# quickwit-oss/tantivy

Measured on AMD Instinct MI355X. Metric: queries_per_sec_2term_AND_bm25_top10, higher is better.
Workload: dtype u32+f32; 1 GPU; and2: 10000 queries/batch, k=10, one 10M-doc Zipf segment per GPU (256 terms, df_r=0.5N/r, WithFreqs); term ranks ~ Zipf(1); distinct_queries=3877, mode=block-max pruned (block_wand_intersection semantics), exchange=single rank: no exchange, segments_per_gpu=1, index_bytes=40381332

## Files before the change

include/tantivy_amd.h:

```cpp
#ifndef TANTIVY_AMD_H
#define TANTIVY_AMD_H

#include <stddef.h>
#include <stdint.h>

#ifdef __cplusplus
extern "C" {
#endif

#define TQ_TERMINATED 0x7FFFFFFFu
#define TQ_MAX_TERMS 16u
#define TQ_MAX_K 1024u

enum tq_status {
  TQ_OK = 0,
  TQ_ERR_INVALID = 1,
  TQ_ERR_HIP = 2,
  TQ_ERR_FORMAT = 3,
  TQ_ERR_UNSUPPORTED = 4,
  TQ_ERR_NO_DEVICE = 5
};

enum tq_record_option { TQ_BASIC = 0, TQ_WITH_FREQS = 1, TQ_WITH_FREQS_AND_POSITIONS = 2 };

// ... 34 lines not shown
int tq_all_query_form(const tq_query *q, tq_all_form *out);

int tq_init(const int *device_ids, int n_devices, tq_ctx **out);
void tq_shutdown(tq_ctx *ctx);
const char *tq_last_error(void);

int tq_segment_upload(tq_ctx *ctx, int device, uint32_t max_doc, const uint8_t *idx,
                      size_t idx_len, const uint8_t *pos, size_t pos_len,
                      const uint8_t *fieldnorm, size_t fn_len, uint8_t record_option,
                      tq_segment **out);
int tq_segment_upload_device(tq_ctx *ctx, int device, uint32_t max_doc, const uint8_t *d_idx,
                             size_t idx_len, const uint8_t *d_pos, size_t pos_len,
                             const uint8_t *d_fieldnorm, size_t fn_len, uint8_t record_option,
                             tq_segment **out);
void tq_segment_free(tq_segment *seg);

int tq_term_prepare(tq_segment *seg, uint64_t postings_off, uint32_t postings_len,
                    uint64_t positions_off, uint32_t positions_len, uint32_t doc_freq,
                    tq_term_handle *out);
typedef struct tq_term_info {
  uint64_t postings_off;
  uint64_t positions_off;
  uint32_t postings_len, positions_len;
  uint32_t doc_freq;
  uint32_t pad_;
} tq_term_info;
int tq_term_prepare_batch(tq_segment *seg, const tq_term_info *infos, uint32_t n, tq_term_handle *out);
int tq_segment_reserve_columns(tq_segment *seg, const uint64_t *postings_offs, uint32_t n);

int tq_term_set_prepare(tq_segment *seg, const tq_term_handle *members, uint32_t n, tq_term_handle *out);
int tq_term_set_info(tq_segment *seg, tq_term_handle set, uint32_t *n_docs, uint64_t *bytes);
int tq_term_set_release(tq_segment *seg, tq_term_handle set);

int tq_search_batch(tq_segment *seg, const tq_query *queries, uint32_t n_queries,
                    uint32_t out_stride, float *out_scores, uint32_t *out_docs,
                    uint32_t *out_counts);

int tq_search_batch_device(tq_segment *seg, const tq_query *queries, uint32_t n_queries,
                           uint32_t out_stride, float *d_out_scores, uint32_t *d_out_docs,
                           uint32_t *d_out_counts, void *hip_stream);

#define TQ_OPT_DEFAULT 0xFFFFFFFFu
typedef struct tq_search_opts {
  int32_t exhaustive;
  uint32_t bound_slack_ppm;
} tq_search_opts;
int tq_search_batch_opts(tq_segment *seg, const tq_query *queries, uint32_t n_queries,
                         uint32_t out_stride, float *out_scores, uint32_t *out_docs,
                         uint32_t *out_counts, const tq_search_opts *opts);
int tq_search_batch_device_opts(tq_segment *seg, const tq_query *queries, uint32_t n_queries,
                                uint32_t out_stride, float *d_out_scores, uint32_t *d_out_docs,
                                uint32_t *d_out_counts, const tq_search_opts *opts,
                                void *hip_stream);

typedef struct tq_ticket tq_ticket;
int tq_submit(tq_segment *seg, const tq_query *query, const tq_search_opts *opts, float *out_scores,
              uint32_t *out_docs, uint32_t *out_count, tq_ticket **out);
int tq_wait(tq_ticket *ticket);
int tq_search_one(tq_segment *seg, const tq_query *query, const tq_search_opts *opts,
                  float *out_scores, uint32_t *out_docs, uint32_t *out_count);
typedef struct tq_submit_stats {
  uint64_t batches;
  uint64_t queries;
  uint64_t max_batch;
} tq_submit_stats;
int tq_get_submit_stats(tq_segment *seg, tq_submit_stats *out, int reset);

int tq_merge_topk(const float *scores, const uint32_t *docs, const uint32_t *counts,
                  uint32_t n_segments, uint32_t n_queries, uint32_t stride, uint32_t offset,
                  uint32_t limit, float *out_scores, uint32_t *out_segment_ords,
                  uint32_t *out_docs, uint32_t *out_counts);
int tq_merge_topk_device(tq_ctx *ctx, int device, const float *d_scores, const uint32_t *d_docs,
                         const uint32_t *d_counts, const uint32_t *segment_ords,
                         uint32_t n_segments, uint32_t n_queries, uint32_t stride,
                         uint32_t offset, uint32_t limit, float *d_out_scores,
                         uint32_t *d_out_segment_ords, uint32_t *d_out_docs,
                         uint32_t *d_out_counts, void *hip_stream);
int tq_copy_to_host_async(tq_ctx *ctx, int device, void *dst_pinned_host, const void *src_device, size_t bytes,
                          void *hip_stream);

#define TQ_COMM_ID_BYTES 128
typedef struct tq_comm tq_comm;
int tq_comm_unique_id(uint8_t *id_out );
int tq_comm_init(tq_ctx *ctx, int device, const uint8_t *id, int rank, int world, tq_comm **out);
void tq_comm_free(tq_comm *comm);
int tq_comm_info(const tq_comm *comm, int *rank, int *world, const char **library);
int tq_allgather_topk(tq_comm *comm, const float *d_scores, const uint32_t *d_docs,
                      const uint32_t *d_counts, uint32_t n_rows, uint32_t stride,
                      float *d_all_scores, uint32_t *d_all_docs, uint32_t *d_all_counts,
                      void *hip_stream);

int tq_decode_postings(tq_segment *seg, tq_term_handle term, uint32_t *docs, uint32_t *tfs);
int tq_decode_position_deltas(tq_segment *seg, tq_term_handle term, uint32_t *out, uint64_t cap,
                              uint64_t *n_out);

typedef struct tq_encoder tq_encoder;
int tq_encoder_create(tq_ctx *ctx, int device, tq_encoder **out);
void tq_encoder_free(tq_encoder *enc);
int tq_encode_postings(tq_encoder *enc, uint32_t n_terms, const uint64_t *term_starts,
                       const uint32_t *docs, const uint32_t *tfs, const uint8_t *fieldnorm_ids,
                       uint32_t num_docs, float avg_fieldnorm, uint8_t record_option, uint8_t *out,
                       uint64_t out_cap, uint64_t *out_term_starts, uint64_t *out_len);
int tq_encode_positions(tq_encoder *enc, uint32_t n_terms, const uint64_t *term_starts,
                        const uint32_t *position_deltas, uint8_t *out, uint64_t out_cap,
                        uint64_t *out_term_starts, uint64_t *out_len);
int tq_encode_postings_device(tq_encoder *enc, uint32_t n_terms, const uint64_t *term_starts,
// ... 76 lines not shown
```

include/tantivy_amd_host.h:

```cpp
#ifndef TANTIVY_AMD_HOST_H
#define TANTIVY_AMD_HOST_H
#include "tantivy_amd.h"
#ifdef __cplusplus
extern "C" {
#endif

typedef struct tqh_searcher tqh_searcher;

typedef struct tqh_term_info {
  uint32_t term_id;
  uint32_t doc_freq;
  uint64_t postings_start, postings_end, positions_start, positions_end;
} tqh_term_info;

#define TQH_MODE_TERM 4
typedef struct tqh_query {
  uint8_t mode;
  uint32_t n_terms;
  const uint32_t *terms;
  const uint32_t *phrase_offsets;
  const uint8_t *occurs;
  const uint8_t *clause_of;
  uint32_t min_should_match;
  const float *boosts;
  const uint8_t *nested_occurs;
  const uint8_t *clause_min_should;
  const uint8_t *atom_of;
  const uint32_t *set_terms;
  const uint32_t *set_starts;
} tqh_query;
#define TQH_TERM_SET_BASE 0xFFFFFF00u

const char *tqh_last_error(void);
int tqh_searcher_new(tq_ctx *ctx, tqh_searcher **out);
void tqh_searcher_free(tqh_searcher *s);
int tqh_searcher_add_segment(tqh_searcher *s, int device, uint32_t max_doc, uint8_t record_option,
                             const uint8_t *idx, size_t idx_len, const uint8_t *pos,
                             size_t pos_len, const uint8_t *fieldnorm, size_t fn_len,
                             const tqh_term_info *terms, uint32_t n_terms);
int tqh_searcher_add_remote_stats(tqh_searcher *s, uint64_t max_doc, uint64_t total_num_tokens,
                                  const uint32_t *term_ids, const uint32_t *doc_freqs,
                                  uint32_t n_terms);
int tqh_prepare_batch(tqh_searcher *s, const tqh_query *queries, uint32_t n);
int tqh_prepare_batch_next(tqh_searcher *s, const tqh_query *queries, uint32_t n);
int tqh_commit_next(tqh_searcher *s);
int tqh_search_prepared(tqh_searcher *s, uint32_t offset, uint32_t limit, float *scores,
                        uint32_t *segment_ords, uint32_t *docs, uint32_t *counts);
int tqh_search_concurrent(tqh_searcher *s, const tqh_query *queries, uint32_t n, uint32_t offset,
                          uint32_t limit, uint32_t n_threads, float *scores, uint32_t *segment_ords,
                          uint32_t *docs, uint32_t *counts, float *latency_ms, double *wall_ms);
int tqh_count_prepared(tqh_searcher *s, uint64_t *counts);
int tqh_docset_prepared(tqh_searcher *s, uint32_t *out_segment_ords, uint32_t *out_docs, uint64_t out_cap,
                        uint64_t *out_starts);
int tqh_docset_scored_prepared(tqh_searcher *s, uint32_t *out_segment_ords, uint32_t *out_docs, float *out_scores,
                               uint64_t out_cap, uint64_t *out_starts);
int tqh_collect_segment_prepared(tqh_searcher *s, uint32_t segment_ord, uint32_t k, float *scores,
                                 uint32_t *docs, uint32_t *counts);
int tqh_collect_segment_prepared_device(tqh_searcher *s, uint32_t segment_ord, uint32_t k,
                                        float *d_scores, uint32_t *d_docs, uint32_t *d_counts,
                                        void *hip_stream);
int tqh_bm25_for_terms(const uint64_t *term_doc_freqs, uint32_t n_terms, uint64_t total_num_docs,
                       uint64_t total_num_tokens, float boost, float *weight_out,
                       float *cache_out);
tq_segment *tqh_segment_raw(tqh_searcher *s, uint32_t segment_ord);
uint32_t tqh_term_handle(tqh_searcher *s, uint32_t segment_ord, uint32_t term_id);

typedef struct tqh_term_info_store tqh_term_info_store;
int tqh_term_dictionary_values(const uint8_t *file, size_t len, uint64_t *store_off,
                               uint64_t *store_len);
int tqh_term_info_store_open(const uint8_t *bytes, size_t len, tqh_term_info_store **out);
void tqh_term_info_store_free(tqh_term_info_store *s);
uint64_t tqh_term_info_store_num_terms(const tqh_term_info_store *s);
int tqh_term_info_store_get(const tqh_term_info_store *s, const uint64_t *term_ords, uint32_t n,
                            tqh_term_info *out);
int tqh_term_info_store_write(const tqh_term_info *infos, uint32_t n, uint8_t *out,
                              uint64_t out_cap, uint64_t *out_len);
int tqh_searcher_add_segment_with_store(tqh_searcher *s, int device, uint32_t max_doc,
                                        uint8_t record_option, const uint8_t *idx, size_t idx_len,
                                        const uint8_t *pos, size_t pos_len,
                                        const uint8_t *fieldnorm, size_t fn_len,
                                        const uint8_t *store, size_t store_len);

int tqh_searcher_add_segment_device_with_store(tqh_searcher *s, int device, uint32_t max_doc,
                                               uint8_t record_option, const uint8_t *d_idx,
                                               size_t idx_len, const uint8_t *d_pos, size_t pos_len,
                                               const uint8_t *d_fieldnorm, size_t fn_len,
                                               uint64_t total_num_tokens, const uint8_t *store,
                                               size_t store_len);

#ifdef __cplusplus
}
#endif
#endif
```

tantivy_amd/binding.py:

```python
import ctypes as C
import os

import numpy as np

_HERE = os.path.dirname(os.path.abspath(__file__))
LIB_PATH = os.path.join(_HERE, "lib", "libtantivy_amd.so")
if os.environ.get("TQ_LIB_PATH"):
    LIB_PATH = os.environ["TQ_LIB_PATH"]

TERMINATED = 0x7FFFFFFF
TERM_ABSENT = 0xFFFFFFFF
TERM_ALL = 0xFFFFFFFE
ALL_EMPTY, ALL_PLAIN, ALL_BASED = 0, 1, 2
MODE_AND, MODE_OR, MODE_PHRASE, MODE_BOOL, MODE_TERM = 0, 1, 2, 3, 4
SHOULD, MUST, MUST_NOT = 0, 1, 2
BASIC, WITH_FREQS, WITH_FREQS_AND_POSITIONS = 0, 1, 2


class TantivyAmdError(RuntimeError):
    def __init__(self, code, msg):
        super().__init__("tantivy_amd error %d: %s" % (code, msg))
        self.code = code


# ... 42 lines not shown
    return [n for b, n in sorted(KERNEL_NAMES.items()) if mask & b]


class TqAllForm(C.Structure):
    _fields_ = [("kind", C.c_uint32), ("base", C.c_float), ("min_should", C.c_uint32), ("keep_mask", C.c_uint32)]


class TqSubmitStats(C.Structure):
    _fields_ = [("batches", C.c_uint64), ("queries", C.c_uint64), ("max_batch", C.c_uint64)]


class TqSegmentStats(C.Structure):
    _fields_ = [(n, C.c_uint64) for n in (
        "index_bytes", "positions_bytes", "fieldnorm_bytes", "alive_bytes", "term_table_bytes",
        "bitmap_bytes", "docmat_bytes", "posdir_bytes", "scratch_bytes", "dense_budget_bytes")] + [
        (n, C.c_uint32) for n in ("n_terms", "n_dense_lists", "n_docmat_columns", "probe_evictions")] + [
        ("device_scratch_bytes", C.c_uint64)]


class TqTermInfo(C.Structure):
    _fields_ = [("postings_off", C.c_uint64), ("positions_off", C.c_uint64), ("postings_len", C.c_uint32),
                ("positions_len", C.c_uint32), ("doc_freq", C.c_uint32), ("pad_", C.c_uint32)]


class TqhTermInfo(C.Structure):
    _fields_ = [("term_id", C.c_uint32), ("doc_freq", C.c_uint32), ("postings_start", C.c_uint64),
                ("postings_end", C.c_uint64), ("positions_start", C.c_uint64),
                ("positions_end", C.c_uint64)]


class TqhQuery(C.Structure):
    _fields_ = [("mode", C.c_uint8), ("n_terms", C.c_uint32), ("terms", C.POINTER(C.c_uint32)),
                ("phrase_offsets", C.POINTER(C.c_uint32)), ("occurs", C.POINTER(C.c_uint8)),
                ("clause_of", C.POINTER(C.c_uint8)), ("min_should_match", C.c_uint32),
                ("boosts", C.POINTER(C.c_float)), ("nested_occurs", C.POINTER(C.c_uint8)),
                ("clause_min_should", C.POINTER(C.c_uint8)), ("atom_of", C.POINTER(C.c_uint8)),
                ("set_terms", C.POINTER(C.c_uint32)), ("set_starts", C.POINTER(C.c_uint32))]


TERM_SET_BASE = 0xFFFFFF00


class RawHandle(int):
    """A tq_term_handle as the C ABI returned it (DeviceIndex.term_set_prepare): DeviceIndex.term_handle passes it
    through untouched where a plain int is a term id of the dictionary."""


_lib = None

EXPORTS = [
    "tq_init", "tq_shutdown", "tq_last_error", "tq_segment_upload", "tq_segment_upload_device",
    "tq_segment_free",
    "tq_term_prepare", "tq_term_prepare_batch", "tq_search_batch", "tq_search_batch_device", "tq_search_batch_opts",
    "tq_search_batch_device_opts", "tq_merge_topk",
    "tq_merge_topk_device", "tq_copy_to_host_async", "tq_decode_postings", "tq_decode_position_deltas",
    "tq_last_batch_stats", "tq_segment_get_stats", "tq_segment_reserve_columns", "tq_set_option", "tq_segment_set_alive_bitset", "tq_count_batch",
    "tq_last_batch_match_counts", "tq_last_batch_query_kernels", "tq_encoder_create", "tq_encoder_free", "tq_encode_postings",
    "tq_encode_positions", "tq_encode_postings_device", "tq_encode_positions_device",
    "tq_encoder_last_kernel_ms", "tq_comm_unique_id", "tq_comm_init", "tq_comm_free",
    "tq_comm_info", "tq_allgather_topk",
    "tqh_last_error", "tqh_searcher_new", "tqh_searcher_free", "tqh_searcher_add_segment",
    "tqh_prepare_batch", "tqh_prepare_batch_next", "tqh_commit_next", "tqh_search_prepared", "tqh_collect_segment_prepared",
    "tqh_collect_segment_prepared_device", "tqh_searcher_add_remote_stats",
    "tqh_bm25_for_terms", "tqh_segment_raw", "tqh_term_handle", "tqh_term_dictionary_values",
    "tqh_term_info_store_open", "tqh_term_info_store_free", "tqh_term_info_store_num_terms",
    "tqh_term_info_store_get", "tqh_term_info_store_write", "tqh_searcher_add_segment_with_store",
    "tqh_count_prepared", "tqh_searcher_add_segment_device_with_store",
    "tq_docset_batch", "tq_docset_batch_device", "tqh_docset_prepared",
    "tq_docset_scored_batch", "tq_docset_scored_batch_device", "tqh_docset_scored_prepared",
    "tq_all_query_form",
    "tq_term_set_prepare", "tq_term_set_info", "tq_term_set_release",
]


def lib():
    global _lib
    if _lib is not None:
        return _lib
    if not os.path.exists(LIB_PATH):
        raise TantivyAmdError(-1, "%s not built (run `python -m tantivy_amd.build` or "
                                  "__graft_entry__.build())" % LIB_PATH)
    L = C.CDLL(LIB_PATH)
    vp, u8p, u32p, f32p = C.c_void_p, C.POINTER(C.c_uint8), C.POINTER(C.c_uint32), C.POINTER(C.c_float)
    L.tq_last_error.restype = C.c_char_p
    L.tqh_last_error.restype = C.c_char_p
    L.tq_init.argtypes = [C.POINTER(C.c_int), C.c_int, C.POINTER(vp)]
    L.tq_shutdown.argtypes = [vp]
    L.tq_segment_upload.argtypes = [vp, C.c_int, C.c_uint32, vp, C.c_size_t, vp, C.c_size_t, vp,
                                    C.c_size_t, C.c_uint8, C.POINTER(vp)]
    L.tq_segment_upload_device.argtypes = [vp, C.c_int, C.c_uint32, vp, C.c_size_t, vp, C.c_size_t, vp,
                                           C.c_size_t, C.c_uint8, C.POINTER(vp)]
    L.tq_segment_free.argtypes = [vp]
    L.tq_term_prepare.argtypes = [vp, C.c_uint64, C.c_uint32, C.c_uint64, C.c_uint32, C.c_uint32,
                                  u32p]
    L.tq_term_prepare_batch.argtypes = [vp, C.POINTER(TqTermInfo), C.c_uint32, u32p]
    L.tq_search_batch.argtypes = [vp, C.POINTER(TqQuery), C.c_uint32, C.c_uint32, f32p, u32p, u32p]
    L.tq_search_batch_device.argtypes = [vp, C.POINTER(TqQuery), C.c_uint32, C.c_uint32, vp, vp,
                                         vp, vp]
    L.tq_search_batch_opts.argtypes = [vp, C.POINTER(TqQuery), C.c_uint32, C.c_uint32, f32p, u32p,
                                       u32p, C.POINTER(TqSearchOpts)]
    L.tq_search_batch_device_opts.argtypes = [vp, C.POINTER(TqQuery), C.c_uint32, C.c_uint32, vp,
                                              vp, vp, C.POINTER(TqSearchOpts), vp]
    L.tq_merge_topk.argtypes = [f32p, u32p, u32p, C.c_uint32, C.c_uint32, C.c_uint32, C.c_uint32,
                                C.c_uint32, f32p, u32p, u32p, u32p]
    L.tq_copy_to_host_async.argtypes = [vp, C.c_int, vp, vp, C.c_size_t, vp]
    L.tq_merge_topk_device.argtypes = [vp, C.c_int, vp, vp, vp, vp, C.c_uint32, C.c_uint32,
                                       C.c_uint32, C.c_uint32, C.c_uint32, vp, vp, vp, vp, vp]
    L.tq_decode_postings.argtypes = [vp, C.c_uint32, u32p, u32p]
    L.tq_decode_position_deltas.argtypes = [vp, C.c_uint32, u32p, C.c_uint64,
                                            C.POINTER(C.c_uint64)]
    L.tq_last_batch_stats.argtypes = [vp, C.POINTER(TqBatchStats)]
    L.tq_segment_get_stats.argtypes = [vp, C.POINTER(TqSegmentStats)]
    L.tq_segment_reserve_columns.argtypes = [vp, C.POINTER(C.c_uint64), C.c_uint32]
    L.tq_set_option.argtypes = [vp, C.c_char_p, C.c_int64]
    L.tq_segment_set_alive_bitset.argtypes = [vp, vp, C.c_size_t]
    L.tq_count_batch.argtypes = [vp, C.POINTER(TqQuery), C.c_uint32, u32p]
    L.tq_last_batch_match_counts.argtypes = [vp, u32p, C.c_uint32]
    L.tq_docset_batch.argtypes = [vp, C.POINTER(TqQuery), C.c_uint32, u32p, C.c_uint64, C.POINTER(C.c_uint64)]
    L.tq_docset_batch_device.argtypes = [vp, C.POINTER(TqQuery), C.c_uint32, vp, C.c_uint64, vp, vp]
    L.tqh_docset_prepared.argtypes = [vp, u32p, u32p, C.c_uint64, C.POINTER(C.c_uint64)]
    L.tq_docset_scored_batch.argtypes = [vp, C.POINTER(TqQuery), C.c_uint32, u32p, f32p, C.c_uint64, C.POINTER(C.c_uint64)]
    L.tq_docset_scored_batch_device.argtypes = [vp, C.POINTER(TqQuery), C.c_uint32, vp, vp, C.c_uint64, vp, vp]
    L.tqh_docset_scored_prepared.argtypes = [vp, u32p, u32p, f32p, C.c_uint64, C.POINTER(C.c_uint64)]
    L.tq_last_batch_query_kernels.argtypes = [vp, u32p, C.c_uint32]
    L.tq_all_query_form.argtypes = [C.POINTER(TqQuery), C.POINTER(TqAllForm)]
    L.tq_term_set_prepare.argtypes = [vp, u32p, C.c_uint32, u32p]
    L.tq_term_set_info.argtypes = [vp, C.c_uint32, u32p, C.POINTER(C.c_uint64)]
    L.tq_term_set_release.argtypes = [vp, C.c_uint32]
    u64p = C.POINTER(C.c_uint64)
    L.tq_encoder_create.argtypes = [vp, C.c_int, C.POINTER(vp)]
    L.tq_encoder_free.argtypes = [vp]
    L.tq_encoder_free.restype = None
    L.tq_encode_postings.argtypes = [vp, C.c_uint32, vp, vp, vp, vp, C.c_uint32, C.c_float,
                                     C.c_uint8, vp, C.c_uint64, vp, u64p]
    L.tq_encode_positions.argtypes = [vp, C.c_uint32, vp, vp, vp, C.c_uint64, vp, u64p]
    L.tq_encode_postings_device.argtypes = [vp, C.c_uint32, vp, vp, vp, vp, vp, C.c_uint32,
                                            C.c_float, C.c_uint8, vp, C.c_uint64, vp, u64p, vp]
    L.tq_encode_positions_device.argtypes = [vp, C.c_uint32, vp, vp, vp, vp, C.c_uint64, vp, u64p,
                                             vp]
    L.tq_encoder_last_kernel_ms.argtypes = [vp, C.POINTER(C.c_float)]
    L.tq_comm_unique_id.argtypes = [vp]
    L.tq_comm_init.argtypes = [vp, C.c_int, vp, C.c_int, C.c_int, C.POINTER(vp)]
    L.tq_comm_free.argtypes = [vp]
    L.tq_comm_free.restype = None
    L.tq_comm_info.argtypes = [vp, C.POINTER(C.c_int), C.POINTER(C.c_int), C.POINTER(C.c_char_p)]
    L.tq_allgather_topk.argtypes = [vp, vp, vp, vp, C.c_uint32, C.c_uint32, vp, vp, vp, vp]
    L.tqh_searcher_new.argtypes = [vp, C.POINTER(vp)]
    L.tqh_searcher_free.argtypes = [vp]
    L.tqh_searcher_add_segment.argtypes = [vp, C.c_int, C.c_uint32, C.c_uint8, vp, C.c_size_t, vp,
                                           C.c_size_t, vp, C.c_size_t, C.POINTER(TqhTermInfo),
                                           C.c_uint32]
    L.tqh_prepare_batch.argtypes = [vp, C.POINTER(TqhQuery), C.c_uint32]
    L.tqh_prepare_batch_next.argtypes = [vp, C.POINTER(TqhQuery), C.c_uint32]
    L.tqh_commit_next.argtypes = [vp]
    L.tqh_search_prepared.argtypes = [vp, C.c_uint32, C.c_uint32, f32p, u32p, u32p, u32p]
    L.tqh_search_concurrent.argtypes = [vp, C.POINTER(TqhQuery), C.c_uint32, C.c_uint32, C.c_uint32, C.c_uint32,
                                        f32p, u32p, u32p, u32p, f32p, C.POINTER(C.c_double)]
    L.tq_get_submit_stats.argtypes = [vp, C.POINTER(TqSubmitStats), C.c_int]
    L.tq_search_one.argtypes = [vp, C.POINTER(TqQuery), C.POINTER(TqSearchOpts), f32p, u32p, u32p]
    L.tq_submit.argtypes = [vp, C.POINTER(TqQuery), C.POINTER(TqSearchOpts), f32p, u32p, u32p, C.POINTER(vp)]
    L.tq_wait.argtypes = [vp]
    L.tqh_collect_segment_prepared.argtypes = [vp, C.c_uint32, C.c_uint32, f32p, u32p, u32p]
    L.tqh_collect_segment_prepared_device.argtypes = [vp, C.c_uint32, C.c_uint32, vp, vp, vp, vp]
    L.tqh_searcher_add_remote_stats.argtypes = [vp, C.c_uint64, C.c_uint64, u32p, u32p, C.c_uint32]
    L.tqh_bm25_for_terms.argtypes = [C.POINTER(C.c_uint64), C.c_uint32, C.c_uint64, C.c_uint64,
                                     C.c_float, f32p, f32p]
    L.tqh_segment_raw.restype = vp
    L.tqh_segment_raw.argtypes = [vp, C.c_uint32]
    L.tqh_term_handle.restype = C.c_uint32
    L.tqh_term_handle.argtypes = [vp, C.c_uint32, C.c_uint32]
    L.tqh_term_dictionary_values.argtypes = [vp, C.c_size_t, u64p, u64p]
    L.tqh_count_prepared.argtypes = [vp, u64p]
    L.tqh_term_info_store_open.argtypes = [vp, C.c_size_t, C.POINTER(vp)]
    L.tqh_term_info_store_free.argtypes = [vp]
    L.tqh_term_info_store_free.restype = None
    L.tqh_term_info_store_num_terms.argtypes = [vp]
    L.tqh_term_info_store_num_terms.restype = C.c_uint64
    L.tqh_term_info_store_get.argtypes = [vp, vp, C.c_uint32, C.POINTER(TqhTermInfo)]
    L.tqh_term_info_store_write.argtypes = [C.POINTER(TqhTermInfo), C.c_uint32, vp, C.c_uint64, u64p]
    L.tqh_searcher_add_segment_with_store.argtypes = [vp, C.c_int, C.c_uint32, C.c_uint8, vp,
                                                      C.c_size_t, vp, C.c_size_t, vp, C.c_size_t,
                                                      vp, C.c_size_t]
    L.tqh_searcher_add_segment_device_with_store.argtypes = [
        vp, C.c_int, C.c_uint32, C.c_uint8, vp, C.c_size_t, vp, C.c_size_t, vp, C.c_size_t,
        C.c_uint64, vp, C.c_size_t]
    _lib = L
    return L


def _check(rc, host=False):
    if rc != 0:
        L = lib()
        msg = (L.tqh_last_error() if host else L.tq_last_error()) or b""
        if host and not msg:
            msg = L.tq_last_error() or b""
        raise TantivyAmdError(rc, msg.decode("utf-8", "replace"))


def _f32(a):
    return a.ctypes.data_as(C.POINTER(C.c_float))


def _u32(a):
    return a.ctypes.data_as(C.POINTER(C.c_uint32))


def bm25_for_terms(doc_freqs, total_num_docs, total_num_tokens, boost=1.0):
    dfs = (C.c_uint64 * len(doc_freqs))(*[int(d) for d in doc_freqs])
    w = C.c_float()
    cache = np.zeros(256, np.float32)
    _check(lib().tqh_bm25_for_terms(dfs, len(doc_freqs), int(total_num_docs), int(total_num_tokens),
                                    C.c_float(boost), C.byref(w), _f32(cache)), host=True)
    return float(w.value), cache


def all_query_form(handles, weights=None, mode=MODE_BOOL, occurs=None, clause_of=None, min_should_match=0):
# ... 328 lines not shown

    def commit_next(self):
        fut, n, _ = self._prep_next
        secs = fut.result()
        self._prep_next = None
        _check(lib().tqh_commit_next(self._s), host=True)
        self._n_prepared = n
        return secs

    def search_concurrent(self, queries, limit, n_threads, offset=0):
        qs, keep = self._host_queries(queries)
        n = len(queries)
        scores = np.zeros((n, limit), np.float32)
        ords = np.zeros((n, limit), np.uint32)
        docs = np.zeros((n, limit), np.uint32)
        counts = np.zeros(n, np.uint32)
        lat = np.zeros(max(1, n), np.float32)
        wall = C.c_double()
        _check(lib().tqh_search_concurrent(self._s, qs, n, int(offset), int(limit), int(n_threads),
                                           _f32(scores), _u32(ords), _u32(docs), _u32(counts), _f32(lat),
                                           C.byref(wall)), host=True)
        return scores, ords, docs, counts, lat[:n], float(wall.value)

    def submit_stats(self, segment_ord=0, reset=False):
        st = TqSubmitStats()
        _check(lib().tq_get_submit_stats(self.segment_raw(segment_ord), C.byref(st), 1 if reset else 0))
        return {"batches": int(st.batches), "queries": int(st.queries), "max_batch": int(st.max_batch)}

    def search_prepared(self, limit, offset=0):
        n = self._n_prepared
        scores = np.zeros((n, limit), np.float32)
        ords = np.zeros((n, limit), np.uint32)
        docs = np.zeros((n, limit), np.uint32)
        counts = np.zeros(n, np.uint32)
        _check(lib().tqh_search_prepared(self._s, int(offset), int(limit), _f32(scores),
                                         _u32(ords), _u32(docs), _u32(counts)), host=True)
        return scores, ords, docs, counts

    def collect_segment_prepared(self, segment_ord, k):
        n = self._n_prepared
        scores = np.zeros((n, k), np.float32)
        docs = np.zeros((n, k), np.uint32)
        counts = np.zeros(n, np.uint32)
        _check(lib().tqh_collect_segment_prepared(self._s, int(segment_ord), int(k), _f32(scores),
                                                  _u32(docs), _u32(counts)), host=True)
        return scores, docs, counts

    def collect_segment_prepared_device(self, segment_ord, k, d_scores, d_docs, d_counts,
                                        stream=None):
        _check(lib().tqh_collect_segment_prepared_device(
            self._s, int(segment_ord), int(k), d_scores.data_ptr(), d_docs.data_ptr(),
            d_counts.data_ptr(), C.c_void_p(stream) if stream else None), host=True)

    @property
    def ctx(self):
        return self._ctx

    def search(self, queries, limit, offset=0):
        self.prepare(queries)
        return self.search_prepared(limit, offset)

    def count(self, queries):
        self.prepare(queries)
        out = np.zeros(max(1, len(queries)), np.uint64)
        _check(lib().tqh_count_prepared(self._s, out.ctypes.data_as(C.POINTER(C.c_uint64))), host=True)
        return out[: len(queries)]

    def docset(self, queries):
        self.prepare(queries)
        n = len(queries)
        starts = np.zeros(n + 1, np.uint64)
        ords = np.zeros(1, np.uint32)
        docs = np.zeros(1, np.uint32)
        u64p = C.POINTER(C.c_uint64)
        rc = lib().tqh_docset_prepared(self._s, _u32(ords), _u32(docs), 0, starts.ctypes.data_as(u64p))
        if rc != 0 and int(starts[n]) > 0:
            ords = np.zeros(int(starts[n]), np.uint32)
            docs = np.zeros(int(starts[n]), np.uint32)
            rc = lib().tqh_docset_prepared(self._s, _u32(ords), _u32(docs), docs.size, starts.ctypes.data_as(u64p))
        _check(rc, host=True)
        pairs = np.stack([ords, docs], axis=1)
        return [pairs[int(starts[q]): int(starts[q + 1])] for q in range(n)]

    def docset_scored(self, queries):
        self.prepare(queries)
        n = len(queries)
        starts = np.zeros(n + 1, np.uint64)
        ords = np.zeros(1, np.uint32)
        docs = np.zeros(1, np.uint32)
        scores = np.zeros(1, np.float32)
        u64p = C.POINTER(C.c_uint64)
        rc = lib().tqh_docset_scored_prepared(self._s, _u32(ords), _u32(docs), _f32(scores), 0, starts.ctypes.data_as(u64p))
        if rc != 0 and int(starts[n]) > 0:
            ords = np.zeros(int(starts[n]), np.uint32)
            docs = np.zeros(int(starts[n]), np.uint32)
            scores = np.zeros(int(starts[n]), np.float32)
            rc = lib().tqh_docset_scored_prepared(self._s, _u32(ords), _u32(docs), _f32(scores), docs.size,
                                                  starts.ctypes.data_as(u64p))
        _check(rc, host=True)
        pairs = np.stack([ords, docs], axis=1)
        return [(pairs[int(starts[q]): int(starts[q + 1])], scores[int(starts[q]): int(starts[q + 1])]) for q in range(n)]

    def segment_raw(self, segment_ord=0):
        return C.c_void_p(lib().tqh_segment_raw(self._s, segment_ord))

    def term_handle(self, term_id, segment_ord=0):
# ... 279 lines not shown
```

tantivy_amd/csrc/tq_api.cpp:

```cpp
#include "tq_internal.hpp"
#include "../host/bm25.hpp"

namespace tqi {

thread_local std::string g_last_error;

int fail(int code, const char *fmt, ...) {
  char buf[512];
  va_list ap;
  va_start(ap, fmt);
  vsnprintf(buf, sizeof buf, fmt, ap);
  va_end(ap);
  g_last_error = buf;
  return code;
}
}

int tq_internal_fail(int code, const char *where, const char *what) {
  return fail(code, "%s: %s", where, what);
}
bool tq_internal_ctx_has_device(const tq_ctx *ctx, int device) {
  return std::find(ctx->devices.begin(), ctx->devices.end(), device) != ctx->devices.end();
}

// ... 409 lines not shown
    r.device_scratch_bytes = s->dscratch->partials.cap + s->dscratch->share_stage.cap + s->dscratch->ashare_stage.cap +
                             s->dscratch->bshare_stage.cap;
  }
  r.n_terms = (uint32_t)s->terms.size();
  r.n_dense_lists = s->n_dense_lists;
  r.n_docmat_columns = s->n_mat_slots;
  r.probe_evictions = (uint32_t)std::min<uint64_t>(s->probe_evictions, 0xFFFFFFFFull);
  r.dense_budget_bytes = s->dense_budget();
  *out = r;
  return TQ_OK;
}

int tq_set_option(tq_segment *s, const char *name, int64_t value) {
  if (!s || !name) return fail(TQ_ERR_INVALID, "tq_set_option: null argument");
  TQ_SEGMENT_LOCK(s);
  if (!strcmp(name, "exhaustive"))
    __atomic_store_n(&s->opt.exhaustive, value != 0 ? 1 : 0, __ATOMIC_RELAXED);
  else if (!strcmp(name, "timing"))
    s->opt.timing = value != 0;
  else if (!strcmp(name, "use_dpp"))
    s->opt.use_dpp = value != 0;
  else if (!strcmp(name, "use_dense"))
    s->opt.use_dense = value != 0;
  else if (!strcmp(name, "or_windows"))
    s->opt.or_windows = value < 0 ? -1 : (value != 0);
  else if (!strcmp(name, "dense_ratio") && value >= 1)
    s->opt.dense_ratio = (int)value;
  else if (!strcmp(name, "rdir_budget_x") && value >= 0 && value <= 0x7FFFFFFF)
    s->opt.rdir_budget_x = (int)value;
  else if (!strcmp(name, "probe_budget_x") && value >= 0 && value <= 0x7FFFFFFF)
    s->opt.probe_budget_x = (int)value, s->probe_full = false;
  else if (!strcmp(name, "dense_budget_x") && value >= 0)
    s->opt.dense_budget_x = (int)value;
  else if (!strcmp(name, "bound_slack_ppm") && value >= 0 && value <= 1000000000)
    __atomic_store_n(&s->opt.bound_slack_ppm, (int)value, __ATOMIC_RELAXED);
  else if (!strcmp(name, "dense"))
    s->opt.dense = value != 0;
  else if (!strcmp(name, "docmat"))
    s->opt.docmat = value != 0;
  else if (!strcmp(name, "docsig"))
    s->opt.docsig = value != 0;
  else if (!strcmp(name, "device_prepare"))
    s->opt.device_prepare = value != 0;
  else if (!strcmp(name, "xunion_ratio") && value >= 0 && value <= 0x7FFFFFFF)
    s->opt.xunion_ratio = (int)value;
  else if (!strcmp(name, "count_bitmap_ratio") && value >= 0 && value <= 0x7FFFFFFF)
    s->opt.count_bitmap_ratio = (int)value;
  else if (!strcmp(name, "docset_temp_lists") && value >= 0 && value <= 0x7FFFFFFF)
    s->opt.docset_temp_lists = (int)value;
  else if (!strcmp(name, "docset_trees") && (value == 0 || value == 1))
    s->opt.docset_trees = (int)value;
  else if (!strcmp(name, "docset_score_trees") && (value == 0 || value == 1))
    s->opt.docset_score_trees = (int)value;
  else if (!strcmp(name, "ashare_min_batch") && value >= 0 && value <= 0x7FFFFFFF)
    s->opt.ashare_min_batch = (int)value;
  else if (!strcmp(name, "xunion_min_queries") && value >= 1 && value <= 0x7FFFFFFF)
    s->opt.xunion_min_queries = (int)value;
  else if (!strcmp(name, "record_query_kernels"))
    s->opt.record_query_kernels = value != 0;
  else if (!strcmp(name, "debug") && value >= -1 && value <= 0x7FFFFFFF)
    s->opt.debug = (int)value;
  else if (!strcmp(name, "submit_window_us") && value >= 0 && value <= 1000000)
    s->opt.submit_window_us = (int)value;
  else
    return fail(TQ_ERR_INVALID, "unknown option '%s'", name);
  return TQ_OK;
}

int tq_decode_postings(tq_segment *s, tq_term_handle term, uint32_t *docs, uint32_t *tfs) {
  if (!s || !docs || !tfs) return fail(TQ_ERR_INVALID, "tq_decode_postings: null argument");
  TQ_SEGMENT_LOCK(s);
  if (term >= s->terms.size()) return fail(TQ_ERR_INVALID, "unknown term handle %u", term);
  if (s->terms[term].set_kind != TermHost::kNoSet) return fail(TQ_ERR_INVALID, "tq_decode_postings: handle %u is a term set: it has no postings", term);
  HIP_TRY(hipSetDevice(s->device));
  int rc = sync_terms(s, s->stream);
  if (rc != TQ_OK) return rc;
  const TermHost &t = s->terms[term];
  const size_t bytes = (size_t)t.doc_freq * sizeof(uint32_t);
  rc = s->d_misc.ensure(2 * bytes + 64);
  if (rc != TQ_OK) return rc;
  uint32_t *dd = (uint32_t *)s->d_misc.p, *dt = dd + t.doc_freq;
  hipError_t e = tqk_launch_decode_list(s->dseg, s->d_terms, term, t.n_blocks, dd, dt,
                                        s->opt.use_dpp != 0, s->stream);
  if (e != hipSuccess) return fail(TQ_ERR_HIP, "decode launch: %s", hipGetErrorString(e));
  HIP_TRY(hipMemcpyAsync(docs, dd, bytes, hipMemcpyDeviceToHost, s->stream));
  HIP_TRY(hipMemcpyAsync(tfs, dt, bytes, hipMemcpyDeviceToHost, s->stream));
  HIP_TRY(hipStreamSynchronize(s->stream));
  return TQ_OK;
}

int tq_decode_position_deltas(tq_segment *s, tq_term_handle term, uint32_t *out, uint64_t cap,
                              uint64_t *n_out) {
  if (!s || !n_out) return fail(TQ_ERR_INVALID, "tq_decode_position_deltas: null argument");
  TQ_SEGMENT_LOCK(s);
  if (term >= s->terms.size()) return fail(TQ_ERR_INVALID, "unknown term handle %u", term);
  const TermHost &t = s->terms[term];
  if (t.set_kind != TermHost::kNoSet) return fail(TQ_ERR_INVALID, "tq_decode_position_deltas: handle %u is a term set: it has no positions", term);
  if (t.positions_len == 0) return fail(TQ_ERR_UNSUPPORTED, "term has no positions on the device");
  *n_out = t.n_positions;
  const uint64_t n = std::min<uint64_t>(cap, t.n_positions);
  if (n == 0 || !out) return TQ_OK;
  HIP_TRY(hipSetDevice(s->device));
  int rc = sync_terms(s, s->stream);
  if (rc != TQ_OK) return rc;
  rc = s->d_misc.ensure(n * sizeof(uint32_t));
  if (rc != TQ_OK) return rc;
// ... 98 lines not shown
```

tantivy_amd/csrc/tq_common.hpp:

```cpp
#pragma once
#include <hip/hip_runtime.h>
#include <stdint.h>

#include "tq_device.h"
#include "tq_launch.h"

namespace {

constexpr int WAVE = 64;

__device__ __forceinline__ uint32_t uni(uint32_t x) {
  return (uint32_t)__builtin_amdgcn_readfirstlane((int)x);
}
__device__ __forceinline__ float uni_f(float x) { return __uint_as_float(uni(__float_as_uint(x))); }
__device__ uint32_t uni(float) = delete;
__device__ uint32_t uni(double) = delete;
__device__ __forceinline__ uint64_t uni64(uint64_t x) {
  uint32_t lo = uni((uint32_t)x), hi = uni((uint32_t)(x >> 32));
  return ((uint64_t)hi << 32) | lo;
}
template <typename T>
__device__ __forceinline__ const T *uni_ptr(const T *p) {
  return (const T *)uni64((uint64_t)p);
}
// ... 328 lines not shown
      m &= m - 1;
      const uint64_t nk = readlane64(key, src);
      if (nk <= thr) continue;
      uint32_t pos = 0;
#pragma unroll
      for (int r = 0; r < KPL; ++r) pos += (uint32_t)__popcll(__ballot(v[r] > nk));
#pragma unroll
      for (int r = KPL - 1; r >= 0; --r) {
        uint64_t up = __shfl_up(v[r], 1, WAVE);
        if (r > 0) {
          const uint64_t carry = readlane64(v[r - 1], 63);
          if (lane == 0) up = carry;
        }
        const uint32_t rank = (uint32_t)r * 64u + (uint32_t)lane;
        if (rank > pos)
          v[r] = up;
        else if (rank == pos)
          v[r] = nk;
      }
      refresh_thr();
    }
  }
};

__device__ __forceinline__ void wave_mem_fence() {
  __builtin_amdgcn_fence(__ATOMIC_ACQ_REL, "wavefront");
  __builtin_amdgcn_wave_barrier();
}

__device__ __forceinline__ uint32_t find_query(const uint32_t *tile_starts, uint32_t n_queries,
                                               uint32_t t) {
  uint32_t lo = 0, hi = n_queries;
  while (hi - lo > 1u) {
    const uint32_t mid = (lo + hi) >> 1;
    if (sload(tile_starts + mid) <= t)
      lo = mid;
    else
      hi = mid;
  }
  return lo;
}

template <int KPL>
__device__ __forceinline__ void flush_partial(const TopK<KPL> &tk, uint64_t *partials,
                                              uint32_t part, int lane) {
  uint64_t *dst = partials + (uint64_t)part * (uint64_t)(KPL * 64);
#pragma unroll
  for (int r = 0; r < KPL; ++r) {
    const uint32_t rank = (uint32_t)r * 64u + (uint32_t)lane;
    dst[rank] = rank < tk.k ? tk.v[r] : 0ull;
  }
}

__device__ __forceinline__ uint32_t sortable(float x) {
  uint32_t fb = __float_as_uint(x);
  return fb ^ ((uint32_t)((int32_t)fb >> 31) | 0x80000000u);
}
__device__ __forceinline__ float block_max_score(uint32_t meta, float w, const float *cache,
                                                 uint32_t has_freq, float slack) {
  const uint32_t tfc = meta >> 24;
  if (meta == META_TAIL || !has_freq || tfc == 0u) return w;
  const uint32_t tf = tfc == 255u ? 0xFFFFFFFFu : tfc;
  return bm25(w, cache[(meta >> 16) & 0xFFu], tf) * slack;
}
__device__ __forceinline__ float block_max_bound(uint32_t meta, float w, const float *cache,
                                                 uint32_t has_freq, float slack) {
  const uint32_t tfc = meta >> 24;
  if (meta == META_TAIL || !has_freq || tfc == 0u) return w;
  const uint32_t tf = tfc == 255u ? 0xFFFFFFFFu : tfc;
  return bm25_bound(w, cache[(meta >> 16) & 0xFFu], tf) * slack;
}
template <int S>
__device__ __forceinline__ uint32_t kth_largest_multi(const uint32_t (&v)[S], uint32_t k) {
  uint32_t ans = 0;
  for (int bit = 31; bit >= 0; --bit) {
    const uint32_t trial = ans | (1u << bit);
    uint32_t c = 0;
#pragma unroll
    for (int r = 0; r < S; ++r) c += (uint32_t)__popcll(__ballot(v[r] >= trial));
    if (c >= k) ans = trial;
  }
  return ans;
}
#ifndef TQ_KTH_LOW_BIT
#define TQ_KTH_LOW_BIT 8
#endif
template <int S>
__device__ __forceinline__ uint32_t kth_largest_hi16(const uint32_t (&v)[4], uint32_t k) {
  uint32_t ans = 0;
  for (int bit = 31; bit >= TQ_KTH_LOW_BIT; --bit) {
    const uint32_t trial = ans | (1u << bit);
    uint32_t c = 0;
#pragma unroll
    for (int r = 0; r < S; ++r) c += (uint32_t)__popcll(__ballot(v[r] >= trial));
    if (c >= k) ans = trial;
  }
  return ans;
}
__device__ __forceinline__ uint32_t kth_largest64(uint32_t v, uint32_t k) {
  const uint32_t a[1] = {v};
  return kth_largest_multi<1>(a, k);
}
__device__ __forceinline__ uint32_t mbcnt64(uint64_t m) {
  return __builtin_amdgcn_mbcnt_hi((uint32_t)(m >> 32), __builtin_amdgcn_mbcnt_lo((uint32_t)m, 0u));
}
constexpr uint32_t NOT_FOUND = 0xFFFFFFFFu;
// ... 199 lines not shown
```

tantivy_amd/csrc/tq_internal.hpp:

```cpp
#pragma once
#include <hip/hip_runtime.h>

#include <algorithm>
#include <array>
#include <atomic>
#include <chrono>
#include <condition_variable>
#include <deque>
#include <map>
#include <mutex>
#include <new>
#include <cstdlib>
#include <cmath>
#include <cstdarg>
#include <cstdio>
#include <cstring>
#include <string>
#include <unordered_map>
#include <unordered_set>
#include <thread>
#include <vector>

#include "../../include/tantivy_amd.h"
#include "tq_device.h"
// ... 87 lines not shown
inline uint32_t rd32(const uint8_t *p) {
  return (uint32_t)p[0] | ((uint32_t)p[1] << 8) | ((uint32_t)p[2] << 16) | ((uint32_t)p[3] << 24);
}
inline bool read_vint(const uint8_t *d, size_t len, size_t &at, uint64_t &out) {
  uint64_t r = 0;
  unsigned shift = 0;
  while (at < len) {
    uint8_t b = d[at++];
    r |= (uint64_t)(b & 127u) << shift;
    if (b & 128u) {
      out = r;
      return true;
    }
    shift += 7;
    if (shift > 63) return false;
  }
  return false;
}
inline bool read_vint32_block(const uint8_t *d, size_t len, size_t &at, uint32_t &out) {
  uint32_t r = 0, shift = 0;
  while (at < len) {
    uint8_t b = d[at++];
    r += (uint32_t)(b & 127u) << shift;
    if (b & 128u) {
      out = r;
      return true;
    }
    shift += 7;
  }
  return false;
}

struct Options {
  int exhaustive = 0;
  int timing = 0;
  int use_dpp = 1;
  int dense = 1;
  int dense_ratio = TQD_DENSE_RATIO;
  int dense_budget_x = 8;
  int use_dense = 1;
  int docmat = 1;
  int docsig = 1;
  int device_prepare = 0;
  int or_windows = -1;
  int bound_slack_ppm = 0;
  int xunion_ratio = 64;
  int xunion_min_queries = 64;
  int rdir_budget_x = 4;
  int probe_budget_x = 16;
  int count_bitmap_ratio = 128;
  int docset_temp_lists = 0;
  int docset_trees = 0;
  int docset_score_trees = 0;
  int ashare_min_batch = 16;
  int submit_window_us = 100;
  int record_query_kernels = 0;
  int debug = -1;
};


inline uint32_t tune_u32(const char *name, uint32_t dflt) {
  const char *v = getenv(name);
  return v && *v ? (uint32_t)strtoul(v, nullptr, 10) : dflt;
}

}
using namespace tqi;

struct DeviceScratch {
  std::mutex m;
  DevBuf partials, share_stage, ashare_stage, bshare_stage;
  hipEvent_t ev_last = nullptr;
  hipStream_t last_stream = nullptr;
  bool in_flight = false;
};
struct tq_ctx {
  std::vector<int> devices;
  std::mutex m;
  std::map<int, DeviceScratch *> scratch;
  DeviceScratch *scratch_for(int device) {
    std::lock_guard<std::mutex> lk(m);
    DeviceScratch *&p = scratch[device];
    if (!p) p = new DeviceScratch();
    return p;
  }
  ~tq_ctx() {
    for (auto &kv : scratch) {
      (void)hipSetDevice(kv.first);
      if (kv.second->ev_last) (void)hipEventDestroy(kv.second->ev_last);
      kv.second->partials.release();
      kv.second->share_stage.release();
      kv.second->ashare_stage.release();
      kv.second->bshare_stage.release();
      delete kv.second;
    }
  }
};

struct tq_segment {
  tq_ctx *ctx = nullptr;
  int device = 0;
  hipStream_t stream = nullptr;
  uint32_t max_doc = 0;
  uint8_t record_option = 0;
  std::vector<uint8_t> h_idx, h_pos;
  size_t idx_len = 0, pos_len = 0;
// ... 253 lines not shown
    {TQ_MODE_OR, false, TQ_KERNEL_ALL}};
inline uint32_t group_kernel_bit(int gi, bool or_windows) {
  return gi == kGUnion && or_windows ? TQ_KERNEL_OR_WINDOWS : kGroupTraits[gi].kernel;
}
struct RouteTotals {
  uint32_t n_thr_rows = 0;
  uint32_t n_ashare_ext = 0;
  uint64_t algo_bytes = 0;
  bool phrase_all_dense = true;
};
struct QuerySlab {
  Group groups[kNGroups];
  RouteTotals t;
  int rc = 0;
  std::string err;
};
struct PlanScratch {
  Group groups[kNGroups];
  std::vector<uint32_t> q_cache;
  std::vector<QuerySlab> q_slabs;
  std::vector<TqkDenseRow> xrows;
  std::vector<TqkDenseQuery> xqueries;
  std::vector<uint64_t> xrow_term;
  std::unordered_map<uint64_t, uint32_t> xrow_of;
  uint32_t xcache = 0xFFFFFFFFu;
  uint32_t xgrid = 0, x_bitmap_rows = 0, x_tiles_per_task = 1, x_list_stride = 0, x_max_terms = 1;
  std::vector<ShareKey> share_keys, share_keys2;
  std::vector<uint64_t> sort_keys, sort_keys2;
  std::vector<uint32_t> term_rank, term_distinct;
  std::vector<TqdLead> leads;
  std::vector<uint4> tasks;
  std::vector<uint32_t> share_pairs;
  struct ASharePlan {
    std::vector<TqdALead> aleads, aleads_unsorted;
    std::vector<ALeadKey> alead_keys, alead_keys2;
    std::vector<uint32_t> alead_first, alead_bucket, alead_bucket_at, alead_bucket_starts;
    std::vector<uint8_t> alead_same;
    std::vector<uint64_t> aq_sig;
    std::vector<uint64_t> aq_slot;
    struct QKey {
      uint32_t t0, t1, w0, w1, k, shape;
    };
    std::vector<QKey> aq_key;
    std::vector<uint32_t> aowner;
    std::vector<uint4> atasks;
    std::vector<uint2> alists;
    std::vector<uint32_t> apairs, atask_hist, atask_slab_run;
    struct ARun {
      uint32_t r0, r1, term, cache, n_blocks, n_groups, per_group, bpt, nb_warm, n_runs;
      size_t task0;
    };
    std::vector<ARun> aruns;
    uint32_t a_warm_tasks = 0;
    bool over_budget = false;
    bool any_rdir = false;
  };
  ASharePlan ap[2];
  std::vector<uint32_t> q_leader;
  std::vector<uint32_t> and_lead_count;
  std::vector<uint32_t> term_stamp;
  uint32_t batch_stamp = 0;
  uint32_t share_phase_first[TQD_US_MAX_TERMS + 1];
  uint64_t share_table_base = 0;
  std::vector<uint32_t> lead_cost, sort_start;
  std::vector<PlanSlab> slabs;
  std::vector<std::pair<uint64_t, uint32_t>> keyed;
  PodVec<TqdQuery> q_tmp;
  std::vector<uint32_t> o_tmp, c_tmp, hist;
  std::vector<uint4> sorted_recs;
};

namespace tqi {

uint32_t plan_threads();
class PlanPool {
 public:
  static PlanPool &get() {
    static PlanPool *pool = new PlanPool();
    return *pool;
  }
  void run(uint32_t n, void (*fn)(void *, uint32_t), void *ctx) {
    std::unique_lock<std::mutex> job_lock(job_mutex_, std::try_to_lock);
    if (!job_lock.owns_lock() || !ensure_workers(std::min<uint32_t>(n, plan_threads()) - 1u)) {
      for (uint32_t i = 0; i < n; ++i) fn(ctx, i);
      return;
    }
    uint64_t gen;
    {
      std::lock_guard<std::mutex> lk(m_);
      fn_ = fn;
      ctx_ = ctx;
      n_ = n;
      gen = generation_.load(std::memory_order_relaxed) + 1;
      done_.store(0, std::memory_order_relaxed);
      ticket_.store(gen << 32, std::memory_order_release);
      generation_.store(gen, std::memory_order_release);
    }
    cv_.notify_all();
    work(gen, fn, ctx, n);
    while (done_.load(std::memory_order_acquire) < n) std::this_thread::yield();
  }

 private:
  void work(uint64_t gen, void (*fn)(void *, uint32_t), void *ctx, uint32_t n) {
    for (;;) {
      uint64_t cur = ticket_.load(std::memory_order_acquire);
// ... 167 lines not shown
  uint32_t min_should = 0, keep_mask = 0;
  bool boost_mixed = false;
};
int all_query_form(const tq_query &q, AllForm &f, const char **why);
struct AllView {
  tq_query q;
  tq_term_handle terms[TQ_MAX_TERMS];
  float weights[TQ_MAX_TERMS];
  uint8_t occurs[TQ_MAX_TERMS], clause_of[TQ_MAX_TERMS];
  uint32_t pos[TQ_MAX_TERMS];
};
void all_strip_view(const tq_query &q, const AllForm &f, AllView &v);
inline bool is_term_set(const tq_segment *s, uint32_t h) { return h < s->terms.size() && s->terms[h].set_kind == TermHost::kSet; }
inline const void *expression_bitmap(const tq_segment *s, const TermHost &th) {
  return th.dense_blob && (s->opt.use_dense || th.set_kind == TermHost::kSet) ? th.dense_blob : nullptr;
}
inline bool query_names_set(const tq_segment *s, const tq_query &q) {
  if (!q.terms || q.n_terms > TQ_MAX_TERMS) return false;
  for (uint32_t i = 0; i < q.n_terms; ++i)
    if (is_term_set(s, q.terms[i])) return true;
  return false;
}
int check_set_query(const tq_segment *s, const tq_query &q, uint32_t qi, const char *fn, bool *has);
int count_batch(tq_segment *s, const tq_query *queries, uint32_t n_queries, uint32_t *out_counts);
bool count_expression(tq_segment *s, const tq_query &q, TqkCountQuery &cq, bool &known, uint64_t &driver_postings,
                      std::unordered_map<uint32_t, uint32_t> &temp_slot, uint32_t max_temp);
struct FlatClauses {
  struct Clause {
    uint32_t id, occur, n = 0, terms[TQ_MAX_TERMS];
    uint32_t pos[TQ_MAX_TERMS];
    uint64_t cost = 0;
  };
  Clause cl[TQ_MAX_TERMS];
  uint32_t n_cl = 0, n_must = 0, n_should = 0;
  bool empty = false;
  uint32_t msm = 0;
  bool all_based = false, all_boost_mixed = false;
  float all_base = 0.0f;
};
enum { FLAT_OK = 0, FLAT_UNSUPPORTED, FLAT_INVALID };
int parse_flat_clauses(tq_segment *s, const tq_query &q, FlatClauses &fc, const char **why);
int docset_expression(tq_segment *s, const tq_query &q, TqkDocsetQuery &dq, const char **why, FlatClauses *fc_out = nullptr);
void score_expression(tq_segment *s, const tq_query &q, const FlatClauses &fc, TqkScoreQuery &sq);
int docset_batch(tq_segment *s, const tq_query *queries, uint32_t n_queries, uint32_t *out_docs, float *out_scores,
                 uint64_t out_cap, uint64_t *out_starts, bool scored, bool device_out, void *hip_stream, bool count_only = false);
struct TreeView {
  tq_query q;
  uint8_t occurs[TQ_MAX_TERMS], clause_of[TQ_MAX_TERMS], atom_of[TQ_MAX_TERMS], nested_occurs[TQ_MAX_TERMS];
  float weights[TQ_MAX_TERMS];
};
void docset_tree_view(const tq_query &q, TreeView &v, bool scored = false);
int build_group_chunks(Group &g, bool or_windows, PlanScratch &ps, bool boolean_group = false);
int build_share_plan(tq_segment *s, Group &g, PlanScratch &ps);
int build_ashare_plan(tq_segment *s, Group &g, PlanScratch &ps, bool boolean = false);
int build_dense_plan(tq_segment *s, Group &g, PlanScratch &ps, uint32_t cus);
int plan_bool_query(tq_segment *s, const tq_query &q, uint32_t qi, TqdQuery &dq, uint64_t &qbytes,
                    uint32_t &n_tiles, uint32_t &tile_cost, uint32_t &n_thr_rows, bool exhaustive);
bool bool_query_is_tree(const tq_query &q);
int plan_tree_query(tq_segment *s, const tq_query &q, uint32_t qi, TqdTreeQuery &tq, uint64_t &qbytes, uint64_t table_base);
int resolve_opts(const tq_segment *s, const tq_search_opts *o, CallOpts &co);
void update_table_span(tq_segment *s);
int build_tree_query_probe_tables(tq_segment *s, const tq_query &q, bool *built, bool flat_too = false);
int fail_tree_tables(const tq_segment *s, uint32_t qi);
int search_batch_impl(tq_segment *s, const tq_query *queries, uint32_t n_queries, uint32_t out_stride,
                      float *d_out_scores, uint32_t *d_out_docs, uint32_t *d_out_counts, void *hip_stream,
                      const CallOpts &co);
int search_batch_host(tq_segment *s, const tq_query *queries, uint32_t n_queries, uint32_t out_stride,
                      float *out_scores, uint32_t *out_docs, uint32_t *out_counts, const CallOpts &co);
struct HostBatchSlot {
  PinnedBuf out;
  hipEvent_t done = nullptr, done_blocking = nullptr;
  bool blocking = false;
  size_t o_docs = 0, o_counts = 0;
  uint32_t n = 0, stride = 0;
};
int search_batch_host_begin(tq_segment *s, const tq_query *queries, uint32_t n_queries, uint32_t out_stride,
                            const CallOpts &co, HostBatchSlot &slot);
int search_batch_host_end(tq_segment *s, HostBatchSlot &slot);

}
```

tantivy_amd/csrc/tq_launch.h:

```cpp
#pragma once
#include <hip/hip_runtime.h>
#include <stdint.h>

#include "tq_device.h"

struct TqkSinks {
  uint64_t *partials;
  unsigned long long *match_counter;
  uint32_t *query_matches;
  const uint32_t *out_index;
};

struct TqkScanParams {
  TqdSegment seg;
  const TqdTerm *terms;
  const TqdQuery *queries;
  const uint32_t *tile_starts;
  const uint4 *chunk_recs;
  const float *caches;
  const TqkSinks *sinks;
  uint32_t *thr_slots;
  uint32_t n_queries;
  uint32_t total_tiles;
  uint32_t n_chunks;
// ... 62 lines not shown
constexpr uint32_t TQK_XU_TILE = 128;
constexpr uint32_t TQK_XU_MAX_ROWS = 256;
constexpr uint32_t TQK_XU_MAX_QUERIES = 8192;
#ifndef TQK_XU_WAVES_N
#define TQK_XU_WAVES_N 16
#endif
constexpr uint32_t TQK_XU_WAVES = TQK_XU_WAVES_N;
struct TqkDenseRow {
  const uint2 *dense;
  const uint8_t *tf8;
  const uint32_t *flat_docs;
  uint32_t handle;
  uint32_t doc_freq;
  float w;
  uint32_t pad;
};
struct TqkDenseQuery {
  uint32_t rows_lo, rows_hi;
  uint32_t nt_k;
  uint32_t thr_row;
};
struct TqkDenseParams {
  TqdSegment seg;
  const TqdTerm *terms;
  const TqkDenseRow *rows;
  const TqkDenseQuery *queries;
  const float *cache;
  const TqkSinks *sinks;
  uint32_t *thr_slots;
  uint32_t *thr_val;
  uint32_t *list_count;
  uint32_t *task_counter;
  uint64_t *stage;
  uint64_t *lists;
  uint32_t n_rows, n_bitmap_rows;
  uint32_t n_queries;
  uint32_t max_terms;
  uint32_t n_tasks, tiles_per_task;
  uint32_t list_stride;
  uint32_t grid;
  uint32_t debug;
};

struct TqkMergeParams {
  const TqdQuery *queries;
  const uint64_t *partials;
  const uint32_t *out_index;
  float *out_scores;
  uint32_t *out_docs;
  uint32_t *out_counts;
  uint32_t n_queries;
  uint32_t out_stride;
  uint32_t pre_slices;
};
constexpr uint32_t TQK_MERGE_PRE_MIN = 96;
inline __host__ __device__ uint32_t tqk_merge_slice_lists(uint32_t n_parts, uint32_t pre_slices) {
  return (pre_slices == 0u || n_parts < TQK_MERGE_PRE_MIN) ? 1u : (n_parts + pre_slices - 1u) / pre_slices;
}

struct TqkSegMergeParams {
  const float *scores;
  const uint32_t *docs;
  const uint32_t *counts;
  const uint32_t *segment_ords;
  float *out_scores;
  uint32_t *out_segment_ords;
  uint32_t *out_docs;
  uint32_t *out_counts;
  uint32_t n_segments, n_queries, stride, offset, limit;
};

constexpr uint32_t TQK_TREE_TILE_WORDS = 4096;
constexpr uint32_t TQK_TREE_MAX_TERMS = 16;
constexpr uint32_t TQK_TREE_PHRASE_TERMS = 8;
struct TqdTreeQuery {
  uint32_t n_terms, n_clauses;
  uint32_t k, cache_idx;
  uint32_t part_start;
  uint32_t top_has_must;
  uint32_t top_need;
  uint32_t has_phrase;
  uint32_t dense_off[TQK_TREE_MAX_TERMS];
  uint32_t tf8_off[TQK_TREE_MAX_TERMS];
  uint32_t weight_bits[TQK_TREE_MAX_TERMS];
  uint32_t handle[TQK_TREE_MAX_TERMS];
  uint32_t inner[TQK_TREE_MAX_TERMS];
  uint32_t atom_end[TQK_TREE_MAX_TERMS];
  uint32_t dir_off[TQK_TREE_MAX_TERMS];
  uint32_t phrase_off[TQK_TREE_MAX_TERMS];
  uint32_t outer[TQK_TREE_MAX_TERMS];
  uint32_t inner_need[TQK_TREE_MAX_TERMS];
  uint32_t first_term[TQK_TREE_MAX_TERMS + 1];
};
struct TqkTreeParams {
  TqdSegment seg;
  const TqdTerm *terms;
  const TqdTreeQuery *queries;
  const float *caches;
  const TqkSinks *sinks;
  const uint8_t *table_base;
  uint32_t n_queries, n_words;
  uint32_t any_phrase;
};
hipError_t tqk_launch_tree(const TqkTreeParams &p, int kpl, hipStream_t st);
uint32_t tqk_tree_tiles(uint32_t n_words);
struct TqkDocsetTreeParams {
// ... 190 lines not shown
```

tantivy_amd/csrc/tq_misc.hip:

```cpp
#include "tq_common.hpp"

namespace {

template <int KPL, bool PRE>
__global__ __launch_bounds__(64) void merge_kernel(TqkMergeParams p) {
  const int lane = (int)__lane_id();
  const uint32_t q = PRE ? blockIdx.x % p.n_queries : blockIdx.x;
  if (q >= p.n_queries) return;
  const TqdQuery *Q = uni_ptr(p.queries + q);
  const uint32_t k = uni(Q->k);
  uint32_t part_start = uni(Q->part_start), n_parts = uni(Q->n_parts);
  const uint32_t per = tqk_merge_slice_lists(n_parts, p.pre_slices);
  uint32_t stride = 1u;
  if constexpr (PRE) {
    if (per == 1u) return;
    const uint32_t sl = blockIdx.x / p.n_queries;
    if (sl * per >= n_parts) return;
    part_start += sl * per;
    n_parts = n_parts - sl * per < per ? n_parts - sl * per : per;
    if (n_parts == 1u) return;
  } else {
    stride = per;
    n_parts = (n_parts + per - 1u) / per;
  }
  TopK<KPL> tk;
  tk.reset(k);
  uint64_t floor_key = 0;
  for (uint32_t pi = (uint32_t)lane; pi < n_parts; pi += WAVE) {
    const uint64_t kth = p.partials[(uint64_t)(part_start + pi * stride) * (uint64_t)(KPL * 64) + (k - 1u)];
    floor_key = kth > floor_key ? kth : floor_key;
  }
  for (int o = 32; o; o >>= 1) {
    const uint64_t other = ((uint64_t)(uint32_t)__shfl_xor((int)(floor_key >> 32), o, WAVE) << 32) |
                           (uint32_t)__shfl_xor((int)(uint32_t)floor_key, o, WAVE);
    floor_key = other > floor_key ? other : floor_key;
  }
  constexpr uint32_t GROUP = KPL <= 2 ? 8u : (KPL <= 4 ? 4u : 1u);
  for (uint32_t pi0 = 0; pi0 < n_parts; pi0 += GROUP) {
    uint64_t keys[GROUP][KPL];
#pragma unroll
    for (uint32_t g = 0; g < GROUP; ++g) {
      const uint32_t pi = pi0 + g < n_parts ? pi0 + g : n_parts - 1u;
      const uint64_t *src = p.partials + (uint64_t)(part_start + pi * stride) * (uint64_t)(KPL * 64);
#pragma unroll
      for (int r = 0; r < KPL; ++r) keys[g][r] = src[(uint32_t)r * 64u + (uint32_t)lane];
    }
#pragma unroll
    for (uint32_t g = 0; g < GROUP; ++g) {
      if (pi0 + g >= n_parts) break;
#pragma unroll
      for (int r = 0; r < KPL; ++r)
        tk.offer(keys[g][r] != 0ull && keys[g][r] >= floor_key, keys[g][r], lane);
    }
  }
  if constexpr (PRE) {
    flush_partial<KPL>(tk, const_cast<uint64_t *>(p.partials), part_start, lane);
    return;
  }
  const uint32_t out_q = p.out_index ? p.out_index[q] : q;
  uint32_t count = 0;
#pragma unroll
  for (int r = 0; r < KPL; ++r) {
    const uint32_t rank = (uint32_t)r * 64u + (uint32_t)lane;
    const bool real = rank < k && tk.v[r] != 0ull;
    count += (uint32_t)__popcll(__ballot(real));
    if (rank < p.out_stride) {
      p.out_scores[(uint64_t)out_q * p.out_stride + rank] = real ? key_score(tk.v[r]) : 0.0f;
      p.out_docs[(uint64_t)out_q * p.out_stride + rank] = real ? key_doc(tk.v[r]) : TQD_TERMINATED;
    }
  }
  for (uint32_t rank = (uint32_t)(KPL * 64) + (uint32_t)lane; rank < p.out_stride; rank += 64u) {
    p.out_scores[(uint64_t)out_q * p.out_stride + rank] = 0.0f;
    p.out_docs[(uint64_t)out_q * p.out_stride + rank] = TQD_TERMINATED;
  }
  if (lane == 0) p.out_counts[out_q] = count;
}

__global__ __launch_bounds__(256) void zero_regions_kernel(TqkZeroParams p) {
  const uint32_t r = blockIdx.y;
  uint32_t *dst = p.ptr[r];
  const uint32_t n = p.words[r];
  const uint32_t head = (uint32_t)((16u - ((uintptr_t)dst & 15u)) & 15u) >> 2;
  const uint32_t h = head < n ? head : n;
  const uint32_t tid = blockIdx.x * 256u + threadIdx.x, stride = gridDim.x * 256u;
  if (tid < h) dst[tid] = 0u;
  const uint32_t n4 = (n - h) >> 2;
  uint4 *d4 = reinterpret_cast<uint4 *>(dst + h);
  for (uint32_t i = tid; i < n4; i += stride) d4[i] = make_uint4(0u, 0u, 0u, 0u);
  const uint32_t tail0 = h + (n4 << 2);
  if (tid < n - tail0) dst[tail0 + tid] = 0u;
}

template <bool USE_DPP>
__global__ __launch_bounds__(256) void decode_list_kernel(TqdSegment seg, const TqdTerm *terms,
                                                          uint32_t handle, uint32_t *docs,
                                                          uint32_t *tfs) {
  const int lane = (int)__lane_id();
  const uint32_t wave = uni(threadIdx.x >> 6);
  const TermRef t = load_term(terms, handle);
  const uint32_t j = blockIdx.x * 4u + wave;
  if (j >= t.n_blocks) return;
  const Dec d = decode_block<USE_DPP, false>(uni_ptr(seg.idx), t, j, lane);
  const uint32_t i0 = j * 128u + 2u * (uint32_t)lane;
  const uint32_t df = uni(terms[handle].doc_freq);
  if (i0 < df) {
    docs[i0] = d.d0;
    tfs[i0] = d.t0;
  }
  if (i0 + 1u < df) {
    docs[i0 + 1u] = d.d1;
    tfs[i0 + 1u] = d.t1;
  }
}

__global__ void decode_positions_kernel(TqdSegment seg, const TqdTerm *terms, uint32_t handle,
                                        uint32_t *out, uint64_t n) {
  const uint64_t i = (uint64_t)blockIdx.x * blockDim.x + threadIdx.x;
  if (i >= n) return;
  out[i] = position_delta(seg.pos, terms + handle, i);
}

__global__ __launch_bounds__(64) void merge_segments_kernel(TqkSegMergeParams p) {
  const int lane = (int)__lane_id();
  const uint32_t q = blockIdx.x;
  if (q >= p.n_queries) return;
  const uint32_t total = p.n_segments * p.stride;
  const uint32_t want = p.offset + p.limit;
  uint32_t n_valid = 0;
// ... 248 lines not shown
```

tantivy_amd/csrc/tq_plan_share.cpp:

```cpp
#include "tq_internal.hpp"

namespace tqi {

int build_share_plan(tq_segment *s, Group &g, PlanScratch &ps) {
  static const uint32_t kTaskCost = std::max<uint32_t>(64u, tune_u32("TQ_US_TASK_COST", 2048));
  static const uint32_t kTaskBlocksMax = std::max<uint32_t>(1u, tune_u32("TQ_US_TASK_BLOCKS", 64));
  static const uint32_t kGroupMax = std::min<uint32_t>(TQD_US_GROUP, std::max<uint32_t>(1u, tune_u32("TQ_US_GROUP", TQD_US_GROUP)));
  const size_t nq = g.queries.size();
  g.kpl = kpl_for(g.max_k);
  static const bool ptrace = getenv("TQ_PLAN_TRACE") != nullptr;
  auto pt_last = std::chrono::steady_clock::now();
  auto pt = [&](const char *what) {
    if (!ptrace) return;
    const auto now = std::chrono::steady_clock::now();
    fprintf(stderr, "[tq share plan] %-12s %7.2f ms\n", what, std::chrono::duration<double, std::milli>(now - pt_last).count());
    pt_last = now;
  };
  std::vector<ShareKey> &keys = ps.share_keys;
  {
    std::vector<uint32_t> &rank = ps.term_rank, &distinct = ps.term_distinct;
    if (rank.size() < s->terms.size()) rank.resize(s->terms.size(), 0u);
    distinct.clear();
    size_t n_pairs = 0;
    for (size_t q = 0; q < nq; ++q) {
// ... 132 lines not shown
  for (size_t r0 = 0; r0 < keys.size();) {
    size_t r1 = r0;
    while (r1 < keys.size() && keys[r1].key == keys[r0].key && keys[r1].term == keys[r0].term) ++r1;
    const uint32_t li = (uint32_t)(keys[r0].key >> 56);
    const uint32_t task_cost = (uint32_t)std::min<uint64_t>(kTaskCost, std::max<uint64_t>(36u, phase_cost[li] / kPhaseTasks));
    while (phase < li) ps.share_phase_first[++phase] = (uint32_t)tasks.size();
    const uint32_t term = keys[r0].term, cache = (uint32_t)keys[r0].key & 0xFFu;
    const uint32_t n_blocks = s->terms[term].n_blocks;
    const uint32_t n_run = (uint32_t)(r1 - r0);
    const uint32_t n_groups = (n_run + kGroupMax - 1) / kGroupMax;
    const uint32_t per_group = (n_run + n_groups - 1) / n_groups;
    uint32_t bpt = task_cost / (4u + per_group);
    bpt = std::min<uint32_t>(kTaskBlocksMax, std::max<uint32_t>(1u, bpt));
    bpt = (uint32_t)std::min<uint64_t>(0xFFFFu, (uint64_t)bpt * stretch);
    for (uint32_t j0 = 0; j0 < n_blocks; j0 += bpt) {
      const uint32_t nb = std::min<uint32_t>(bpt, n_blocks - j0);
      for (uint32_t gr = 0; gr < n_groups; ++gr) {
        const uint32_t l0 = gr * per_group, l1 = std::min<uint32_t>(n_run, l0 + per_group);
        if (l0 >= l1) continue;
        tasks.push_back(make_uint4(term, j0, nb | ((l1 - l0) << 16) | (cache << 24), (uint32_t)r0 + l0));
      }
    }
    const uint32_t n_runs = (n_blocks + bpt - 1) / bpt;
    for (size_t a = r0; a < r1; ++a) pairs[keys[a].q] += n_runs;
    r0 = r1;
  }
  while (phase < TQD_US_MAX_TERMS) ps.share_phase_first[++phase] = (uint32_t)tasks.size();
  pt("tasks");
  if (tasks.size() > 0x7FFFFFFFull) return fail(TQ_ERR_UNSUPPORTED, "batch too large (tasks)");
  {
    uint64_t total = 0;
    for (size_t q = 0; q < nq; ++q) total += (uint64_t)pairs[q] * g.queries[q].k;
    if ((total * sizeof(uint64_t) > kListBudget || total > 0xFFFFFFFFull) && stretch < 65536u) {
      stretch *= 2u;
      goto retry_tasks;
    }
  }
  uint64_t entries = 0;
  for (size_t q = 0; q < nq; ++q) {
    TqdQuery &dq = g.queries[q];
    const uint64_t cap = (uint64_t)pairs[q] * dq.k;
    if (entries + cap > 0xFFFFFFFFull) return fail(TQ_ERR_UNSUPPORTED, "batch too large (result lists)");
    dq.part_start = (uint32_t)entries;
    dq.n_parts = (uint32_t)cap;
    dq.chunk_first = (uint32_t)q;
    entries += cap;
  }
  g.list_entries = entries;
  g.total_tiles = (uint32_t)tasks.size();
  g.n_chunks = (uint32_t)tasks.size();
  return TQ_OK;
}

int build_ashare_plan(tq_segment *s, Group &g, PlanScratch &ps, bool boolean) {
  PlanScratch::ASharePlan &A = ps.ap[boolean ? 1 : 0];
  static const uint32_t kTaskPairsEnv = tune_u32("TQ_AS_TASK_PAIRS", 0);
  static const uint32_t kTargetTasks = std::max<uint32_t>(1u, tune_u32("TQ_AS_TARGET_TASKS", 24576));
  static const uint32_t kTaskBlocksMax = std::min<uint32_t>(0xFFFFu, std::max<uint32_t>(1u, tune_u32("TQ_AS_TASK_BLOCKS", 64)));
  static const uint32_t kGroupMax = std::min<uint32_t>(TQD_AS_GROUP, std::max<uint32_t>(1u, tune_u32("TQ_AS_GROUP", TQD_AS_GROUP)));
  static const uint64_t kListBudget = (uint64_t)std::max<uint32_t>(1u, tune_u32("TQ_AS_LIST_MB", 1024)) << 20;
  static const bool ptrace = getenv("TQ_PLAN_TRACE") != nullptr;
  auto pt_last = std::chrono::steady_clock::now();
  auto pt = [&](const char *what) {
    if (!ptrace) return;
    const auto now = std::chrono::steady_clock::now();
    fprintf(stderr, "[tq ashare plan] %-12s %7.2f ms\n", what, std::chrono::duration<double, std::milli>(now - pt_last).count());
    pt_last = now;
  };
  static const bool kUseRanges = tune_u32("TQ_AS_BOUND", 3) != 0;
  const size_t nq = g.queries.size();
  A.over_budget = false;
  g.kpl = g.max_k <= 64 ? 1 : 2;
  auto column_of = [&](uint32_t handle) -> uint32_t {
    const uint32_t slot1 = (s->h_dterms[handle].has_freq >> 8) & 0xFFu;
    return slot1 ? 8u + (slot1 - 1u) : 0u;
  };
  ps.share_table_base = s->share_table_lo;
  auto off_of = [&](const void *ptr) -> uint32_t {
    return ptr ? (uint32_t)(((uint64_t)ptr - ps.share_table_base) >> 3) : 0u;
  };
  std::vector<TqdALead> &leads = A.aleads, &unsorted = A.aleads_unsorted;
  std::vector<ALeadKey> &keys = A.alead_keys;
  std::vector<uint32_t> &lead0 = A.alead_first;
  static const bool kDedupe = tune_u32("TQ_AS_DEDUPE", 1) != 0;
  std::vector<uint32_t> &owner = A.aowner;
  std::vector<uint64_t> &sigs = A.aq_sig;
  owner.resize(nq);
  sigs.resize(nq);
  std::vector<PlanScratch::ASharePlan::QKey> &qk = A.aq_key;
  qk.resize(nq);
  for (size_t q = 0; q < nq; ++q) {
    const TqdQuery &dq = g.queries[q];
    uint64_t sig = 0x9E3779B97F4A7C15ull * (uint64_t)(dq.n_terms | (dq.k << 8));
    for (uint32_t m = 0; m < dq.n_terms; ++m) {
      uint32_t wb;
      memcpy(&wb, &dq.weight[m], sizeof wb);
      sig = (sig ^ (((uint64_t)dq.term[m] << 32) | wb)) * 0xFF51AFD7ED558CCDull;
      sig ^= sig >> 29;
    }
    if (boolean) {
      sig = (sig ^ (((uint64_t)dq.roles << 32) | dq.clause_end)) * 0xFF51AFD7ED558CCDull;
      sig = (sig ^ (((uint64_t)dq.n_lead << 40) | ((uint64_t)dq.n_opt_lead << 20) | dq.min_should)) * 0xFF51AFD7ED558CCDull;
    }
    sigs[q] = sig;
    owner[q] = (uint32_t)q;
    PlanScratch::ASharePlan::QKey &key = qk[q];
    key.t0 = dq.term[0];
// ... 289 lines not shown
    uint64_t total_pairs = 0;
    for (size_t r0 = 0; r0 < nl;) {
      size_t r1 = r0;
      while (r1 < nl && keys[r1].k1 == keys[r0].k1) ++r1;
      total_pairs += (uint64_t)(r1 - r0) * s->terms[(size_t)(keys[r0].k1 >> 8)].n_blocks;
      r0 = r1;
    }
    static const uint32_t kTaskPairsMin = std::max<uint32_t>(4u, tune_u32("TQ_AS_TASK_PAIRS_MIN", 64));
    task_pairs = (uint32_t)std::min<uint64_t>(512u, std::max<uint64_t>(kTaskPairsMin, total_pairs / kTargetTasks));
  }
  task_pairs = std::max<uint32_t>(4u, task_pairs);
  const uint32_t kStretchedBlocksMax = std::max<uint32_t>(kTaskBlocksMax, 511u);
  uint32_t stretch = 1;
  size_t n_tasks = 0;
  for (;;) {
    runs.clear();
    n_tasks = 0;
    uint64_t entries = 0;
    bool can_stretch = false;
    for (size_t r0 = 0; r0 < nl;) {
      size_t r1 = r0;
      uint64_t k_sum = 0;
      while (r1 < nl && keys[r1].k1 == keys[r0].k1) k_sum += leads[r1++].k;
      PlanScratch::ASharePlan::ARun R;
      R.r0 = (uint32_t)r0;
      R.r1 = (uint32_t)r1;
      R.term = (uint32_t)(keys[r0].k1 >> 8);
      R.cache = (uint32_t)keys[r0].k1 & 0xFFu;
      R.n_blocks = s->terms[R.term].n_blocks;
      const uint32_t n_run = (uint32_t)(r1 - r0);
      const uint32_t n_groups = (n_run + kGroupMax - 1) / kGroupMax;
      R.per_group = (n_run + n_groups - 1) / n_groups;
      R.n_groups = (n_run + R.per_group - 1) / R.per_group;
      R.bpt = (uint32_t)std::min<uint64_t>(kStretchedBlocksMax, (uint64_t)std::min<uint32_t>(kTaskBlocksMax, std::max<uint32_t>(1u, task_pairs / R.per_group)) * stretch);
      R.nb_warm = (uint32_t)((uint64_t)R.n_blocks * kWarmPermille / 1000u);
      R.n_runs = (R.nb_warm + kWarmBlocks - 1) / kWarmBlocks + (R.n_blocks - R.nb_warm + R.bpt - 1) / R.bpt;
      can_stretch = can_stretch || (R.bpt < kStretchedBlocksMax && R.bpt < R.n_blocks);
      R.task0 = n_tasks;
      n_tasks += (size_t)R.n_runs * R.n_groups;
      entries += (uint64_t)R.n_runs * k_sum;
      runs.push_back(R);
      r0 = r1;
    }
    if (entries * sizeof(uint64_t) <= kListBudget && entries <= 0xFFFFFFFFull) break;
    if (!can_stretch) {
      A.over_budget = true;
      return fail(TQ_ERR_UNSUPPORTED, "batch too large (result lists of the shared launch: %llu entries over the %llu MB budget)",
                  (unsigned long long)entries, (unsigned long long)(kListBudget >> 20));
    }
    stretch *= 2u;
  }
  if (n_tasks > 0x7FFFFFFFull) return fail(TQ_ERR_UNSUPPORTED, "batch too large (tasks)");
  tasks.resize(n_tasks);
  constexpr uint32_t kSl = 4098;
  const uint32_t t_slabs = n_tasks >= 16384 ? std::min<uint32_t>(plan_threads(), (uint32_t)runs.size()) : 1u;
  std::vector<uint32_t> &hist = A.atask_hist;
  hist.assign((size_t)t_slabs * kSl, 0u);
  std::vector<uint32_t> &slab_run = A.atask_slab_run;
  slab_run.assign(t_slabs + 1, (uint32_t)runs.size());
  {
    uint32_t sb = 0;
    slab_run[0] = 0;
    for (uint32_t r = 0; r < runs.size() && sb + 1 < t_slabs; ++r)
      if (runs[r].task0 >= n_tasks * (sb + 1) / t_slabs) slab_run[++sb] = r;
    for (uint32_t x = sb + 1; x < t_slabs; ++x) slab_run[x] = (uint32_t)runs.size();
  }
  auto walk_run = [&](const PlanScratch::ASharePlan::ARun &R, auto &&emit) {
    const uint64_t slice_mul = ((uint64_t)1 << 44) / R.n_blocks;
    for (uint32_t j0 = 0; j0 < R.n_blocks;) {
      const bool warm = j0 < R.nb_warm;
      const uint32_t nb = warm ? std::min<uint32_t>(kWarmBlocks, R.nb_warm - j0) : std::min<uint32_t>(R.bpt, R.n_blocks - j0);
      emit(j0, nb, warm ? 0u : 1u + std::min<uint32_t>(4095u, (uint32_t)((j0 * slice_mul) >> 32)));
      j0 += nb;
    }
  };
  parallel_slabs(t_slabs, [&](uint32_t sb) {
    uint32_t *h = hist.data() + (size_t)sb * kSl;
    for (uint32_t r = slab_run[sb]; r < slab_run[sb + 1]; ++r) {
      const PlanScratch::ASharePlan::ARun &R = runs[r];
      for (uint32_t a = R.r0; a < R.r1; ++a) {
        const bool twin = (a - R.r0) % R.per_group != 0 && same_as_prev[a];
        leads[a].info = (leads[a].info & ~0x200u) | (twin ? 0x200u : 0u);
      }
      walk_run(R, [&](uint32_t, uint32_t, uint32_t slice) { h[slice] += R.n_groups; });
    }
  });
  {
    uint32_t run = 0;
    for (uint32_t sl = 0; sl < kSl; ++sl)
      for (uint32_t sb = 0; sb < t_slabs; ++sb) {
        const uint32_t n = hist[(size_t)sb * kSl + sl];
        hist[(size_t)sb * kSl + sl] = run;
        run += n;
        if (sl == 0 && sb + 1 == t_slabs) A.a_warm_tasks = run;
      }
  }
  parallel_slabs(t_slabs, [&](uint32_t sb) {
    uint32_t *h = hist.data() + (size_t)sb * kSl;
    for (uint32_t r = slab_run[sb]; r < slab_run[sb + 1]; ++r) {
      const PlanScratch::ASharePlan::ARun &R = runs[r];
      const uint32_t n_run = R.r1 - R.r0;
      walk_run(R, [&](uint32_t j0, uint32_t nb, uint32_t slice) {
        uint4 *out = tasks.data() + h[slice];
        h[slice] += R.n_groups;
        for (uint32_t gr = 0; gr < R.n_groups; ++gr) {
          const uint32_t l0 = gr * R.per_group, l1 = std::min<uint32_t>(n_run, l0 + R.per_group);
          out[gr] = make_uint4(R.term, j0, nb | ((l1 - l0) << 16) | (R.cache << 24), R.r0 + l0);
        }
      });
    }
  });
  pt("tasks");
  std::fill(pairs.begin(), pairs.end(), 0u);
  for (const PlanScratch::ASharePlan::ARun &R : runs)
    for (uint32_t a = R.r0; a < R.r1; ++a) pairs[leads[a].query] += R.n_runs;
  uint64_t entries = 0;
  for (size_t q = 0; q < nq; ++q) {
    TqdQuery &dq = g.queries[q];
    if (owner[q] != q) {
      dq.part_start = g.queries[owner[q]].part_start;
      dq.n_parts = g.queries[owner[q]].n_parts;
      dq.chunk_first = owner[q];
      continue;
    }
    const uint64_t cap = (uint64_t)pairs[q] * dq.k;
    if (entries + cap > 0xFFFFFFFFull) return fail(TQ_ERR_UNSUPPORTED, "batch too large (result lists)");
    dq.part_start = (uint32_t)entries;
    dq.n_parts = (uint32_t)cap;
    dq.chunk_first = (uint32_t)q;
    entries += cap;
  }
  g.list_entries = entries;
  g.total_tiles = (uint32_t)tasks.size();
  g.n_chunks = (uint32_t)tasks.size();
  return TQ_OK;
}

}
```

tantivy_amd/csrc/tq_search.cpp:

```cpp
#include "tq_internal.hpp"

namespace tqi {
namespace {

using Clock = std::chrono::steady_clock;

struct Knobs {
  bool use_bshare = tune_u32("TQ_BSHARE", 1) != 0, bs_rdir = tune_u32("TQ_BS_RDIR", 1) != 0;
  bool use_ashare = tune_u32("TQ_ASHARE", 1) != 0;
  uint32_t ashare_min = std::max<uint32_t>(1u, tune_u32("TQ_AS_MIN_LEADS", 1));
  bool use_ushare = tune_u32("TQ_USHARE", 1) != 0;
  uint32_t debug = tune_u32("TQ_DEBUG", 0);
};
const Knobs &knobs() {
  static const Knobs k;
  return k;
}

struct Batch {
  tq_segment *s;
  const tq_query *queries;
  uint32_t n_queries, out_stride;
  float *out_scores;
  uint32_t *out_docs, *out_counts;
  void *hip_stream;
  CallOpts co;
  bool replan = false;
  hipStream_t st = nullptr;
  bool exhaustive = false, or_windows = false;
  Clock::time_point t0, t_route, t_routed, t_laid, t_waited, t_filled;
  size_t terms_from = 0, terms_to = 0;
  std::vector<const float *> caches;
  uint32_t n_union_queries = 0, n_bool_queries = 0, n_sparse2 = 0;
  uint32_t n_all_queries = 0;
  const uint8_t *set_q = nullptr;
  bool and_probe = false, ashare_on = false, ashare_and = false;
  uint32_t and_tile_cap = TQD_AND_TILE, dense_min_queries = 1;
  uint64_t unique_bytes = 0, dense_ratio = 0;
  PlanScratch *ps = nullptr;
  Group *groups = nullptr;
  RouteTotals t;
  int cus = 256;
  size_t part_off_bytes[kNGroups] = {}, partial_bytes = 0;
  struct Copy { size_t off; const void *src; size_t bytes; };
  std::vector<Copy> copies;
  size_t stage = 0, o_caches = 0, o_terms = 0;
  int bx = 0;
  const uint8_t *ds = nullptr;
  DeviceScratch *sc = nullptr;
  int slot = 0;
  uint32_t grid[kNGroups] = {};
};

}

void update_table_span(tq_segment *s) {
  if (s->share_span_terms == s->terms.size()) return;
  uint64_t lo = ~0ull, hi = 0;
  for (const TermHost &th : s->terms)
    for (const void *ptr : {th.dense_blob, th.tf8_blob, th.probe_dense_blob, th.probe_tf8_blob, th.rmax_blob, th.posdir_blob, th.probe_posdir_blob, th.lnorm_blob})
      if (ptr) {
        lo = std::min<uint64_t>(lo, (uint64_t)ptr);
        hi = std::max<uint64_t>(hi, (uint64_t)ptr);
      }
  if (lo == ~0ull) lo = hi = 8;
  {
    uint64_t lo2 = lo, hi2 = hi;
    for (const auto &ch : s->rdir_chunks) {
      lo2 = std::min<uint64_t>(lo2, (uint64_t)ch.first);
      hi2 = std::max<uint64_t>(hi2, (uint64_t)ch.first + ch.second);
    }
    s->rdir_span_ok = !s->rdir_chunks.empty() && hi2 - (lo2 - 8) < (8ull << 32);
    if (s->rdir_span_ok) {
      lo = lo2;
      hi = hi2;
    }
  }
  s->share_table_lo = (lo - 8) & ~255ull;
  s->share_span_ok = hi - s->share_table_lo < (8ull << 32);
// ... 653 lines not shown
      const size_t at = g_base[gi][sb], n = src.queries.size();
      for (size_t i = 0; i < n; ++i) {
        g.queries[at + i] = src.queries[i];
        if (g.queries[at + i].thr_index != 0xFFFFFFFFu) g.queries[at + i].thr_index += thr_base[sb];
      }
      if (n) {
        memcpy(g.tile_cost.data() + at, src.tile_cost.data(), n * sizeof(uint32_t));
        memcpy(g.out_index.data() + at, src.out_index.data(), n * sizeof(uint32_t));
      }
    }
  });
  return TQ_OK;
}

int route_queries(Batch &b) {
  PlanScratch &ps = *b.ps;
  static const uint32_t kDenseRatioEnv = tune_u32("TQ_XU_RATIO", 0xFFFFFFFFu);
  static const uint32_t kDenseMinEnv = tune_u32("TQ_XU_MIN_QUERIES", 0xFFFFFFFFu);
  b.dense_ratio = kDenseRatioEnv != 0xFFFFFFFFu ? kDenseRatioEnv : (uint32_t)b.s->opt.xunion_ratio;
  b.dense_min_queries = std::max<uint32_t>(1u, kDenseMinEnv != 0xFFFFFFFFu ? kDenseMinEnv : (uint32_t)b.s->opt.xunion_min_queries);
  b.groups = ps.groups;
  for (int gi = 0; gi < kNGroups; ++gi) {
    b.groups[gi].reset();
    b.groups[gi].mode = kGroupTraits[gi].mode;
  }
  ps.xrow_term.clear();
  ps.xrow_of.clear();
  ps.xcache = 0xFFFFFFFFu;
  b.t_route = Clock::now();
  static const uint32_t kQuerySlabMin = tune_u32("TQ_PLAN_QUERY_PAR_MIN", 4096);
  const uint32_t q_slabs = (!b.exhaustive && b.n_queries >= kQuerySlabMin) ? std::min<uint32_t>(plan_threads(), 8u) : 1u;
  if (q_slabs > 1) {
    const int rc = route_in_slabs(b, q_slabs);
    if (rc != TQ_OK) return rc;
  } else {
    for (uint32_t qi = 0; qi < b.n_queries; ++qi) {
      const int rc = plan_query(b, qi, b.groups, b.t);
      if (rc != TQ_OK) return rc;
    }
  }
  b.t_routed = Clock::now();
  Group &d = b.groups[kGXUnion], &o = b.groups[kGUnion];
  if (!d.queries.empty() && d.queries.size() < b.dense_min_queries) {
    o.queries.append(d.queries.begin(), d.queries.end());
    o.tile_cost.insert(o.tile_cost.end(), d.tile_cost.begin(), d.tile_cost.end());
    o.out_index.insert(o.out_index.end(), d.out_index.begin(), d.out_index.end());
    o.max_k = std::max(o.max_k, d.max_k);
    d.reset();
    d.mode = kGroupTraits[kGXUnion].mode;
  }
  return TQ_OK;
}

int plan_group_tasks(Batch &b) {
  PlanScratch &ps = *b.ps;
  (void)hipDeviceGetAttribute(&b.cus, hipDeviceAttributeMultiprocessorCount, b.s->device);
  for (int gi = 0; gi < kNGroups; ++gi) {
    Group &g = b.groups[gi];
    if (g.queries.empty()) continue;
    if (gi == kGTree) {
      const uint32_t tiles = tqk_tree_tiles((b.s->max_doc + 31u) / 32u);
      g.kpl = kpl_for(g.max_k);
      for (TqdQuery &dq : g.queries) dq.n_parts = tiles;
      g.n_chunks = g.total_tiles = (uint32_t)g.queries.size() * tiles;
      continue;
    }
    if (gi == kGAll) {
      g.kpl = kpl_for(g.max_k);
      for (const TqdQuery &dq : g.queries) g.total_tiles += dq.n_parts;
      g.n_chunks = g.total_tiles;
      continue;
    }
    const int rc = gi == kGUShare   ? build_share_plan(b.s, g, ps)
                   : gi == kGAShare ? build_ashare_plan(b.s, g, ps, false)
                   : gi == kGBShare ? build_ashare_plan(b.s, g, ps, true)
                   : gi == kGXUnion ? build_dense_plan(b.s, g, ps, (uint32_t)std::max(1, b.cus))
                                    : build_group_chunks(g, b.or_windows && gi != kGBool, ps, gi == kGBool);
    if (rc == TQ_ERR_UNSUPPORTED && (gi == kGAShare || gi == kGBShare) && ps.ap[gi == kGBShare ? 1 : 0].over_budget) {
      (gi == kGBShare ? b.co.no_bshare : b.co.no_ashare) = true;
      b.replan = true;
    }
    if (rc != TQ_OK) return rc;
  }
  for (int gi = 0; gi < kNGroups; ++gi) {
    Group &g = b.groups[gi];
    b.part_off_bytes[gi] = b.partial_bytes;
    if (kGroupTraits[gi].result_lists) {
      if (!g.queries.empty())
        b.partial_bytes += std::max<size_t>((size_t)g.list_entries, (size_t)g.queries.back().part_start + g.queries.back().n_parts) * sizeof(uint64_t);
      continue;
    }
    uint32_t parts = 0;
    for (TqdQuery &dq : g.queries) {
      dq.part_start = parts;
      parts += dq.n_parts;
    }
    b.partial_bytes += (size_t)parts * (size_t)g.kpl * 64u * sizeof(uint64_t);
  }
  Group &tree = b.groups[kGTree];
  for (size_t i = 0; i < tree.tree.size(); ++i) tree.tree[i].part_start = tree.queries[i].part_start;
  Group &all = b.groups[kGAll];
  for (size_t i = 0; i < all.all.size(); ++i) all.all[i].part_start = all.queries[i].part_start;
  return TQ_OK;
}

int plan_batch(Batch &b) {
  b.t0 = Clock::now();
  b.exhaustive = b.co.exhaustive;
  int rc = sync_term_records(b);
  if (rc != TQ_OK) return rc;
  look_at_queries(b);
  b.or_windows = b.s->opt.or_windows < 0 ? b.exhaustive : b.s->opt.or_windows != 0;
  if ((rc = build_flat_probe_tables(b)) != TQ_OK || (rc = build_tree_probe_tables(b)) != TQ_OK || (rc = build_all_probe_tables(b)) != TQ_OK) return rc;
  count_leaders(b);
  build_leader_norms(b);
  if ((rc = route_queries(b)) != TQ_OK) return rc;
  return plan_group_tasks(b);
}

int lay_out_stage(Batch &b) {
  if (!b.sc->ev_last) HIP_TRY(hipEventCreateWithFlags(&b.sc->ev_last, hipEventDisableTiming));
  int rc = b.sc->partials.ensure(b.partial_bytes + 256);
  if (rc == TQ_OK) rc = b.s->d_qmatches.ensure((size_t)b.n_queries * sizeof(uint32_t));
  if (rc != TQ_OK) return rc;
  const PlanScratch &ps = *b.ps;
  b.copies.reserve(8 * kNGroups + b.caches.size());
  auto put = [&](size_t align, const void *src, size_t bytes) {
// ... 160 lines not shown
    const Group &g = b.groups[gi];
    const size_t n = g.queries.size();
    if (!n) continue;
    const uint32_t per_cu = gi == kGXUnion ? 0u : gi == kGUShare ? kGridMul : kAGridMul ? kAGridMul
                            : gi == kGBShare ? tqk_bshare_waves_per_cu() : tqk_ashare_waves_per_cu();
    b.grid[gi] = gi == kGXUnion ? b.ps->xgrid : (uint32_t)std::min<uint64_t>(g.n_chunks, cus * per_cu);
    const size_t stage_lists = (size_t)b.grid[gi] * (gi == kGXUnion ? n : gi == kGUShare ? TQD_US_GROUP : TQD_AS_GROUP);
    const size_t words = 2 * n + 16;
    rc = list_words(b.s, gi).ensure(words * sizeof(uint32_t));
    if (rc == TQ_OK) rc = list_stage(*b.sc, gi).ensure(stage_lists * tqk_share_capl(g.kpl) * sizeof(uint64_t));
    if (rc == TQ_OK) rc = zero_later(list_words(b.s, gi).p, words * sizeof(uint32_t));
    if (rc != TQ_OK) return rc;
  }
  return launched(tqk_launch_zero(zp, b.st), "zero");
}

template <typename P>
void common_params(P &p, const Batch &b, const Group &g) {
  p.seg = b.s->dseg;
  p.terms = b.s->d_terms;
  p.queries = (const TqdQuery *)(b.ds + g.o_queries);
  p.caches = (const float *)(b.ds + b.o_caches);
  p.sinks = (const TqkSinks *)(b.ds + g.o_sinks);
  p.thr_slots = (uint32_t *)b.s->d_thr.p;
  p.debug = b.s->opt.debug >= 0 ? (uint32_t)b.s->opt.debug : knobs().debug;
  p.bound_slack = b.co.bound_slack;
}

int launch_ashare(const Batch &b, int gi, hipStream_t gst) {
  const Group &g = b.groups[gi];
  const int ai = gi == kGBShare ? 1 : 0;
  const size_t n_a = g.queries.size();
  TqkAShareParams ap{};
  common_params(ap, b, g);
  if (gi == kGAShare) {
    ap.queries = nullptr;
    ap.aqueries = (const TqdAQuery *)(b.ds + g.o_queries);
    ap.xqueries = (const TqdQuery *)(b.ds + g.o_xqueries);
  }
  ap.leads = (const TqdALead *)(b.ds + g.o_leads);
  ap.tasks = (const uint4 *)(b.ds + g.o_tasks);
  ap.qlists = (const uint2 *)(b.ds + g.o_lists);
  ap.thr_val = (uint32_t *)list_words(b.s, gi).p;
  ap.list_count = ap.thr_val + n_a;
  ap.table_base = (const uint8_t *)b.ps->share_table_base;
  ap.stage = (uint64_t *)list_stage(*b.sc, gi).p;
  ap.lists = (uint64_t *)((uint8_t *)b.sc->partials.p + b.part_off_bytes[gi]);
  ap.n_queries = (uint32_t)n_a;
  ap.boolean = (uint32_t)ai;
  ap.rdir_lists = ai && b.ps->ap[ai].any_rdir ? 1u : 0u;
  static const uint32_t kBoundMode = tune_u32("TQ_AS_BOUND", 3);
  ap.bound_mode = kBoundMode;
  ap.n_queues = 1;
  const uint32_t bounds[3] = {0u, b.ps->ap[ai].a_warm_tasks, g.n_chunks};
  for (int ph = 0; ph < 2; ++ph) {
    ap.task_begin = bounds[ph];
    ap.n_tasks = bounds[ph + 1];
    if (ap.n_tasks <= ap.task_begin) continue;
    ap.task_counter = ap.thr_val + 2 * n_a + 8 * ph;
    ap.grid = std::min<uint32_t>(b.grid[gi], ap.n_tasks - ap.task_begin);
    const int rc = launched(tqk_launch_ashare(ap, g.kpl, gst), "shared-intersection");
    if (rc != TQ_OK) return rc;
  }
  return TQ_OK;
}

int launch_ushare(const Batch &b, hipStream_t gst) {
  const Group &g = b.groups[kGUShare];
  const size_t n_share = g.queries.size();
  TqkShareParams sp{};
  common_params(sp, b, g);
  sp.leads = (const TqdLead *)(b.ds + g.o_leads);
  sp.tasks = (const uint4 *)(b.ds + g.o_tasks);
  sp.thr_val = (uint32_t *)b.s->d_share_words.p;
  sp.list_count = sp.thr_val + n_share;
  uint32_t *const counters = sp.thr_val + 2 * n_share;
  sp.stage = (uint64_t *)b.sc->share_stage.p;
  sp.lists = (uint64_t *)((uint8_t *)b.sc->partials.p + b.part_off_bytes[kGUShare]);
  sp.n_queries = (uint32_t)n_share;
  sp.table_base = (const uint8_t *)b.ps->share_table_base;
  static const uint32_t kPhases = tune_u32("TQ_US_PHASES", 0);
  for (uint32_t ph = 0; ph < TQD_US_MAX_TERMS; ++ph) {
    sp.task_begin = b.ps->share_phase_first[ph];
    sp.n_tasks = b.ps->share_phase_first[ph + 1];
    if (!kPhases) {
      if (ph) break;
      sp.n_tasks = g.n_chunks;
    }
    if (sp.n_tasks <= sp.task_begin) continue;
    sp.task_counter = counters + ph;
    sp.grid = std::min<uint32_t>(b.grid[kGUShare], sp.n_tasks - sp.task_begin);
    const int rc = launched(tqk_launch_share(sp, g.kpl, gst), "shared-union");
    if (rc != TQ_OK) return rc;
  }
  return TQ_OK;
}

int launch_tree(const Batch &b, hipStream_t gst) {
  const Group &g = b.groups[kGTree];
  TqkTreeParams tp{};
  tp.seg = b.s->dseg;
  tp.terms = b.s->d_terms;
  tp.queries = (const TqdTreeQuery *)(b.ds + g.o_leads);
  tp.caches = (const float *)(b.ds + b.o_caches);
  tp.sinks = (const TqkSinks *)(b.ds + g.o_sinks);
  tp.table_base = (const uint8_t *)b.s->share_table_lo;
  tp.n_queries = (uint32_t)g.queries.size();
// ... 64 lines not shown
  p.small_k = g.max_k <= 16u ? 1u : 0u;
  p.max_terms = 0;
  for (const TqdQuery &dq : g.queries) p.max_terms = std::max(p.max_terms, dq.n_terms);
  const bool dpp = b.s->opt.use_dpp != 0;
  return launched(g.mode == TQ_MODE_AND  ? tqk_launch_and(p, g.kpl, dpp, gst)
                  : g.mode == TQ_MODE_OR ? tqk_launch_or(p, g.kpl, dpp, gst)
                                         : tqk_launch_phrase(p, g.kpl, dpp, gst),
                  "scan kernel");
}

int launch_groups(Batch &b) {
  const Group *groups = b.groups;
  if (b.s->opt.timing) HIP_TRY(hipEventRecord(b.s->ev_k0[b.slot], b.st));
  const bool fork = std::count_if(groups, groups + kNGroups, [](const Group &g) { return !g.queries.empty(); }) > 1;
  if (fork) {
    HIP_TRY(hipEventRecord(b.s->ev_fork, b.st));
    HIP_TRY(hipStreamWaitEvent(b.s->side_stream, b.s->ev_fork, 0));
  }
  int main_group = -1;
  for (int gi : {kGAShare, kGAndDense, kGPhSweep})
    if (main_group < 0 && !groups[gi].queries.empty()) main_group = gi;
  for (int gi = 0; main_group < 0 && gi < kNGroups; ++gi)
    if (!groups[gi].queries.empty()) main_group = gi;
  for (const int gi : {kGAnd, kGBool, kGBShare, kGUShare, kGXUnion, kGTree, kGAll, kGUnion, kGPhrase, kGPhSweep, kGAndDense, kGAShare}) {
    if (groups[gi].queries.empty()) continue;
    const hipStream_t gst = (fork && gi != main_group) ? b.s->side_stream : b.st;
    const int rc = gi == kGAShare || gi == kGBShare ? launch_ashare(b, gi, gst)
                   : gi == kGUShare                ? launch_ushare(b, gst)
                   : gi == kGTree                  ? launch_tree(b, gst)
                   : gi == kGAll                   ? launch_all(b, gst)
                   : gi == kGXUnion                ? launch_xunion(b, gst)
                                                   : launch_scan(b, gi, gst);
    if (rc != TQ_OK) return rc;
  }
  if (fork) {
    HIP_TRY(hipEventRecord(b.s->ev_join, b.s->side_stream));
    HIP_TRY(hipStreamWaitEvent(b.st, b.s->ev_join, 0));
  }
  if (b.s->opt.timing) HIP_TRY(hipEventRecord(b.s->ev_k1[b.slot], b.st));
  return TQ_OK;
}

int launch_merges(const Batch &b) {
  for (int gi = 0; gi < kNGroups; ++gi) {
    const Group &g = b.groups[gi];
    if (g.queries.empty()) continue;
    TqkMergeParams m{};
    m.queries = (const TqdQuery *)(b.ds + g.o_queries);
    m.partials = (const uint64_t *)((const uint8_t *)b.sc->partials.p + b.part_off_bytes[gi]);
    m.out_index = (const uint32_t *)(b.ds + g.o_outidx);
    m.out_scores = b.out_scores;
    m.out_docs = b.out_docs;
    m.out_counts = b.out_counts;
    m.n_queries = (uint32_t)g.queries.size();
    m.out_stride = b.out_stride;
    if (!kGroupTraits[gi].result_lists) {
      uint32_t max_parts = 0;
      for (const TqdQuery &dq : g.queries) max_parts = std::max(max_parts, dq.n_parts);
      if (max_parts >= TQK_MERGE_PRE_MIN && m.n_queries <= 4096u)
        m.pre_slices = std::min<uint32_t>(32u, std::max<uint32_t>(2u, (uint32_t)std::sqrt((double)max_parts)));
    }
    const int rc = launched(kGroupTraits[gi].result_lists
                                ? tqk_launch_merge_lists(m, (const uint32_t *)list_words(b.s, gi).p + g.queries.size(), g.kpl, gi == kGAShare, b.st)
                                : tqk_launch_merge(m, g.kpl, b.st),
                            "merge kernel");
    if (rc != TQ_OK) return rc;
  }
  return TQ_OK;
}

int finish_batch(const Batch &b) {
  DeviceScratch &sc = *b.sc;
  if (b.s->opt.timing) {
    HIP_TRY(hipEventRecord(b.s->ev_t1[b.slot], b.st));
    ++b.s->batches_timed;
  }
  HIP_TRY(hipEventRecord(b.s->ev_batch_done, b.st));
  HIP_TRY(hipEventRecord(sc.ev_last, b.st));
  sc.last_stream = b.st;
  sc.in_flight = true;
  HIP_TRY(hipEventRecord(b.s->ev_buf_free[b.bx], b.st));
  b.s->buf_used[b.bx] = true;
  ++b.s->batches_enqueued;
  b.s->last_stream = b.st;
  b.s->batch_in_flight = true;
  uint32_t kernel_mask = 0, tiles_total = 0, chunks_total = 0;
  if (b.s->opt.record_query_kernels) b.s->last_query_kernel.assign(b.n_queries, 0u);
  for (int gi = 0; gi < kNGroups; ++gi) {
    const Group &g = b.groups[gi];
    if (g.queries.empty()) continue;
    const uint32_t bit = group_kernel_bit(gi, b.or_windows);
    kernel_mask |= bit;
    tiles_total += g.total_tiles;
    chunks_total += g.n_chunks;
    if (b.s->opt.record_query_kernels)
      for (uint32_t qi : g.out_index) b.s->last_query_kernel[qi] = bit;
  }
  static const bool trace = getenv("TQ_TRACE") != nullptr;
  if (trace) {
    const auto t_enqueued = Clock::now();
    auto us = [](auto x, auto y) { return (long)std::chrono::duration_cast<std::chrono::microseconds>(y - x).count(); };
    for (int gi = 0; gi < kNGroups; ++gi)
      if (!b.groups[gi].queries.empty())
        fprintf(stderr, "[tq] group %d: %zu queries, %u tasks\n", gi, b.groups[gi].queries.size(), b.groups[gi].n_chunks);
    fprintf(stderr, "[tq] plan %ld us (pre-pass %ld us, queries %ld us, chunks %ld us), wait for the staging buffer %ld us, stage fill %ld us, enqueue %ld us, stage bytes %zu\n",
            us(b.t0, b.t_laid), us(b.t0, b.t_route), us(b.t_route, b.t_routed), us(b.t_routed, b.t_laid), us(b.t_laid, b.t_waited),
// ... 44 lines not shown
    if (query_has_all(queries[qi])) {
      AllForm f;
      const char *why = "";
      const int rc = all_query_form(queries[qi], f, &why);
      if (rc != TQ_OK) return fail(rc, "query %u: %s", qi, why);
      if (f.boost_mixed)
        return fail(TQ_ERR_UNSUPPORTED, "query %u has a boosted match-all clause beside another scoring clause or a second match-all clause: its scores stay on the CPU", qi);
      all_based = f.kind == TQ_ALL_BASED;
      if (all_based) {
        ++st.n_all_based;
      } else {
        if (st.eff.empty()) st.eff.assign(queries, queries + n_queries);
        st.views.emplace_back();
        all_strip_view(queries[qi], f, st.views.back());
        st.eff[qi] = st.views.back().q;
      }
    }
    if (!names_set) continue;
    const tq_query &q = st.eff.empty() ? queries[qi] : st.eff[qi];
    if (all_based) {
      for (uint32_t i = 0; i < q.n_terms; ++i)
        if (is_term_set(s, q.terms[i]) && !(q.mode == TQ_MODE_BOOL && q.occurs && q.occurs[i] == TQ_MUST_NOT))
          return fail(TQ_ERR_UNSUPPORTED, "tq_search_batch: query %u: a term set as a Should clause beside a match-all clause stays on the CPU (its counts and doc sets are taken)", qi);
      continue;
    }
    if (!query_names_set(s, q)) continue;
    if (st.set_q.empty()) st.set_q.assign(n_queries, 0);
    st.set_q[qi] = 1;
    ++st.n_set;
    if (q.mode == TQ_MODE_BOOL) continue;
    if (st.eff.empty()) st.eff.assign(queries, queries + n_queries);
    st.set_occurs.emplace_back();
    st.set_occurs.back().fill(q.mode == TQ_MODE_AND ? (uint8_t)TQ_MUST : (uint8_t)TQ_SHOULD);
    tq_query &v = st.eff[qi];
    v.mode = TQ_MODE_BOOL;
    v.occurs = st.set_occurs.back().data();
    v.clause_of = v.nested_occurs = v.clause_min_should = v.atom_of = nullptr;
    v.min_should_match = 0;
  }
  return TQ_OK;
}

size_t host_rows_layout(uint32_t n_queries, uint32_t out_stride, size_t &o_docs, size_t &o_counts) {
  const size_t n = (size_t)n_queries * out_stride;
  o_docs = (n * sizeof(float) + 255) & ~(size_t)255;
  o_counts = (o_docs + n * sizeof(uint32_t) + 255) & ~(size_t)255;
  return o_counts + (size_t)n_queries * sizeof(uint32_t);
}

}

int search_batch_impl(tq_segment *s, const tq_query *queries, uint32_t n_queries,
                      uint32_t out_stride, float *d_out_scores, uint32_t *d_out_docs,
                      uint32_t *d_out_counts, void *hip_stream, const CallOpts &co) {
  if (!s || (!queries && n_queries) || !d_out_scores || !d_out_docs || !d_out_counts)
    return fail(TQ_ERR_INVALID, "tq_search_batch: null argument");
  if (n_queries == 0) return TQ_OK;
  AllStrip strip;
  int rc = strip_all_clauses(s, queries, n_queries, strip);
  if (rc != TQ_OK) return rc;
  if (!strip.eff.empty()) queries = strip.eff.data();
  Batch b{s, queries, n_queries, out_stride, d_out_scores, d_out_docs, d_out_counts, hip_stream, co};
  b.n_all_queries = strip.n_all_based;
  b.set_q = strip.n_set ? strip.set_q.data() : nullptr;
  rc = plan_batch(b);
  while (rc != TQ_OK && b.replan) {
    b = Batch{s, queries, n_queries, out_stride, d_out_scores, d_out_docs, d_out_counts, hip_stream, b.co};
    b.n_all_queries = strip.n_all_based;
    b.set_q = strip.n_set ? strip.set_q.data() : nullptr;
    rc = plan_batch(b);
  }
  if (rc != TQ_OK) return rc;
  b.sc = s->dscratch;
  std::unique_lock<std::mutex> scratch_lock(b.sc->m);
  if ((rc = lay_out_stage(b)) != TQ_OK || (rc = fill_stage(b)) != TQ_OK || (rc = order_batch(b)) != TQ_OK) return rc;
  DrainOnError drain_on_error{s, b.st};
  if ((rc = enqueue_copy(b)) != TQ_OK || (rc = zero_batch_buffers(b)) != TQ_OK || (rc = launch_groups(b)) != TQ_OK ||
      (rc = launch_merges(b)) != TQ_OK || (rc = finish_batch(b)) != TQ_OK)
    return rc;
  drain_on_error.armed = false;
  s->host_ms_sum += std::chrono::duration<double, std::milli>((Clock::now() - b.t0) - (b.t_waited - b.t_laid)).count();
  ++s->host_ms_n;
  return TQ_OK;
}

int resolve_opts(const tq_segment *s, const tq_search_opts *o, CallOpts &co) {
  co.exhaustive = __atomic_load_n(&s->opt.exhaustive, __ATOMIC_RELAXED) != 0;
  uint32_t ppm = (uint32_t)__atomic_load_n(&s->opt.bound_slack_ppm, __ATOMIC_RELAXED);
  if (o) {
    if (o->exhaustive == 0 || o->exhaustive == 1)
      co.exhaustive = o->exhaustive != 0;
    else if (o->exhaustive != -1)
      return fail(TQ_ERR_INVALID, "tq_search_opts.exhaustive must be -1, 0 or 1");
    if (o->bound_slack_ppm != TQ_OPT_DEFAULT) ppm = o->bound_slack_ppm;
    if (ppm > 1000000000u) return fail(TQ_ERR_INVALID, "bound_slack_ppm above 1e9");
  }
  co.bound_slack = 1.0f + (float)ppm * 1e-6f;
  return TQ_OK;
}

int search_batch_host(tq_segment *s, const tq_query *queries, uint32_t n_queries,
                      uint32_t out_stride, float *out_scores, uint32_t *out_docs,
                      uint32_t *out_counts, const CallOpts &co) {
  if (!s || !out_scores || !out_docs || !out_counts)
    return fail(TQ_ERR_INVALID, "tq_search_batch: null argument");
  if (n_queries == 0) return TQ_OK;
  HIP_TRY(hipSetDevice(s->device));
  const size_t n = (size_t)n_queries * out_stride;
  size_t o_docs, o_counts;
  int rc = s->h_out.ensure(host_rows_layout(n_queries, out_stride, o_docs, o_counts));
  if (rc != TQ_OK) return rc;
  uint8_t *h = (uint8_t *)s->h_out.p;
  rc = search_batch_impl(s, queries, n_queries, out_stride, (float *)h, (uint32_t *)(h + o_docs),
                         (uint32_t *)(h + o_counts), nullptr, co);
  if (rc != TQ_OK) return rc;
  HIP_TRY(hipStreamSynchronize(s->stream));
  memcpy(out_scores, h, n * sizeof(float));
  memcpy(out_docs, h + o_docs, n * sizeof(uint32_t));
  memcpy(out_counts, h + o_counts, (size_t)n_queries * sizeof(uint32_t));
  return TQ_OK;
// ... 2 lines not shown
                            const CallOpts &co, HostBatchSlot &slot) {
  if (!s || !n_queries) return fail(TQ_ERR_INVALID, "tq_submit: empty batch");
  HIP_TRY(hipSetDevice(s->device));
  slot.n = n_queries;
  slot.stride = out_stride;
  int rc = slot.out.ensure(host_rows_layout(n_queries, out_stride, slot.o_docs, slot.o_counts));
  if (rc != TQ_OK) return rc;
  if (!slot.done) HIP_TRY(hipEventCreateWithFlags(&slot.done, hipEventDisableTiming));
  if (!slot.done_blocking) HIP_TRY(hipEventCreateWithFlags(&slot.done_blocking, hipEventDisableTiming | hipEventBlockingSync));
  uint8_t *h = (uint8_t *)slot.out.p;
  rc = search_batch_impl(s, queries, n_queries, out_stride, (float *)h, (uint32_t *)(h + slot.o_docs),
                         (uint32_t *)(h + slot.o_counts), nullptr, co);
  if (rc != TQ_OK) return rc;
  static const uint32_t kBlockMin = tune_u32("TQ_SUBMIT_BLOCK_MIN", 128);
  slot.blocking = n_queries >= kBlockMin;
  HIP_TRY(hipEventRecord(slot.blocking ? slot.done_blocking : slot.done, s->stream));
  return TQ_OK;
}
int search_batch_host_end(tq_segment *s, HostBatchSlot &slot) {
  (void)s;
  HIP_TRY(hipEventSynchronize(slot.blocking ? slot.done_blocking : slot.done));
  return TQ_OK;
}
}

extern "C" {

int tq_search_batch_device(tq_segment *s, const tq_query *queries, uint32_t n_queries,
                           uint32_t out_stride, float *d_out_scores, uint32_t *d_out_docs,
                           uint32_t *d_out_counts, void *hip_stream) {
  return tq_search_batch_device_opts(s, queries, n_queries, out_stride, d_out_scores, d_out_docs,
                                     d_out_counts, nullptr, hip_stream);
}

int tq_search_batch_device_opts(tq_segment *s, const tq_query *queries, uint32_t n_queries,
                                uint32_t out_stride, float *d_out_scores, uint32_t *d_out_docs,
                                uint32_t *d_out_counts, const tq_search_opts *opts,
                                void *hip_stream) {
  if (!s) return fail(TQ_ERR_INVALID, "tq_search_batch: null segment");
  try {
    TQ_SEGMENT_LOCK(s);
    CallOpts co;
    const int rc = resolve_opts(s, opts, co);
    if (rc != TQ_OK) return rc;
    return search_batch_impl(s, queries, n_queries, out_stride, d_out_scores, d_out_docs,
                             d_out_counts, hip_stream, co);
  } catch (const std::exception &e) {
    return fail(TQ_ERR_HIP, "tq_search_batch_device: %s", e.what());
  } catch (...) {
    return fail(TQ_ERR_HIP, "tq_search_batch_device: unknown exception");
  }
}

int tq_search_batch(tq_segment *s, const tq_query *queries, uint32_t n_queries,
                    uint32_t out_stride, float *out_scores, uint32_t *out_docs,
                    uint32_t *out_counts) {
  return tq_search_batch_opts(s, queries, n_queries, out_stride, out_scores, out_docs, out_counts,
                              nullptr);
}

int tq_search_batch_opts(tq_segment *s, const tq_query *queries, uint32_t n_queries,
                         uint32_t out_stride, float *out_scores, uint32_t *out_docs,
                         uint32_t *out_counts, const tq_search_opts *opts) {
  if (!s) return fail(TQ_ERR_INVALID, "tq_search_batch: null segment");
  try {
    TQ_SEGMENT_LOCK(s);
    CallOpts co;
    const int rc = resolve_opts(s, opts, co);
    if (rc != TQ_OK) return rc;
    return search_batch_host(s, queries, n_queries, out_stride, out_scores, out_docs, out_counts, co);
  } catch (const std::exception &e) {
    return fail(TQ_ERR_HIP, "tq_search_batch: %s", e.what());
  } catch (...) {
    return fail(TQ_ERR_HIP, "tq_search_batch: unknown exception");
  }
}

}
```

tantivy_amd/csrc/tq_ushare.hip:

```cpp
#include "tq_common.hpp"

#ifndef TQ_US_REFRESH
#define TQ_US_REFRESH 8u
#endif
#ifndef TQ_US_TIMERS
#define TQ_US_TIMERS 0
#endif
#ifndef TQ_US_CHUNK
#define TQ_US_CHUNK 2
#endif
#ifndef TQ_US_WAVES
#define TQ_US_WAVES 4
#endif
#ifndef TQ_US_FWIDE
#define TQ_US_FWIDE 1
#endif

namespace {

constexpr uint32_t US_GROUP = TQD_US_GROUP;
constexpr uint32_t CH = TQ_US_CHUNK;

struct alignas(16) ShareLds {
  TqdLead lead[US_GROUP];
// ... 695 lines not shown
      }
    }
    tb(5u);
    while (qn) stageC(qn < 64u ? qn : 64u);
    te(5u);
    tb(11u);

    wave_mem_fence();
    const uint32_t cw = (uint32_t)lane < US_GROUP ? L.cnt[lane] : 0u;
    const uint32_t cn = cw & 0xFFFFu, sc = cw >> 16;
    if (sc) atomicAdd(sload(&p.sinks->query_matches) + sload(&p.sinks->out_index)[L.lead[lane].query], sc);
    uint64_t have = __ballot(cn != 0u);
    while (have) {
      const uint32_t gs = (uint32_t)__builtin_ctzll(have);
      have &= have - 1ull;
      uint32_t ns = (uint32_t)__builtin_amdgcn_readlane((int)cn, (int)gs);
      const uint32_t ks = uni(L.lk[gs]) & 0xFFu;
      const uint32_t qs = uni(L.lead[gs].query);
      if (ns > ks) {
        (void)compact_slot(gs, ns, ks);
        ns = ks;
      }
      const uint32_t thr_now = __hip_atomic_load(p.thr_val + qs, __ATOMIC_RELAXED, __HIP_MEMORY_SCOPE_AGENT);
      const uint64_t *sl = my_stage + (size_t)gs * CAPL;
      uint64_t v[R];
      uint32_t keep_n = 0;
#pragma unroll
      for (int r = 0; r < R; ++r) {
        const uint32_t i = (uint32_t)r * 64u + (uint32_t)lane;
        v[r] = i < ns ? sl[i] : 0ull;
        if ((uint32_t)(v[r] >> 32) < thr_now) v[r] = 0ull;
        keep_n += (uint32_t)__popcll(__ballot(v[r] != 0ull));
      }
      if (!keep_n) continue;
      uint32_t at = 0;
      if (lane == 0) at = atomicAdd(p.list_count + qs, keep_n);
      at = uni(at);
      uint64_t *dst = p.lists + (size_t)sload(&p.queries[qs].part_start) + at;
      uint32_t base = 0;
#pragma unroll
      for (int r = 0; r < R; ++r) {
        const uint64_t m = __ballot(v[r] != 0ull);
        if (v[r] != 0ull) dst[base + mbcnt64(m)] = v[r];
        base += (uint32_t)__popcll(m);
      }
    }
    te(11u);
  }
  te(1u);
  if (tphase) n_scored = (uint32_t)(tacc >> 6);
  if (lane == 0 && n_scored) atomicAdd(sload(&p.sinks->match_counter), (unsigned long long)n_scored);
}

template <int KPL, typename QT>
__global__ __launch_bounds__(64) void merge_lists_kernel(TqkMergeParams p, const uint32_t *list_count) {
  const int lane = (int)__lane_id();
  const uint32_t q = blockIdx.x;
  if (q >= p.n_queries) return;
  const QT *Q = uni_ptr(reinterpret_cast<const QT *>(p.queries) + q);
  const uint32_t k = uni(Q->k);
  const uint32_t n = uni(list_count[uni(Q->chunk_first)]);
  const uint64_t *src = p.partials + (size_t)uni(Q->part_start);
  TopK<KPL> tk;
  tk.reset(k);
  for (uint32_t i0 = 0; i0 < n; i0 += 256u) {
    uint64_t keys[4];
#pragma unroll
    for (uint32_t u = 0; u < 4u; ++u) {
      const uint32_t i = i0 + 64u * u + (uint32_t)lane;
      keys[u] = i < n ? src[i] : 0ull;
    }
#pragma unroll
    for (uint32_t u = 0; u < 4u; ++u) tk.offer(keys[u] != 0ull, keys[u], lane);
  }
  const uint32_t out_q = p.out_index ? p.out_index[q] : q;
  uint32_t count = 0;
#pragma unroll
  for (int r = 0; r < KPL; ++r) {
    const uint32_t rank = (uint32_t)r * 64u + (uint32_t)lane;
    const bool real = rank < k && tk.v[r] != 0ull;
    count += (uint32_t)__popcll(__ballot(real));
    if (rank < p.out_stride) {
      p.out_scores[(uint64_t)out_q * p.out_stride + rank] = real ? key_score(tk.v[r]) : 0.0f;
      p.out_docs[(uint64_t)out_q * p.out_stride + rank] = real ? key_doc(tk.v[r]) : TQD_TERMINATED;
    }
  }
  for (uint32_t rank = (uint32_t)(KPL * 64) + (uint32_t)lane; rank < p.out_stride; rank += 64u) {
    p.out_scores[(uint64_t)out_q * p.out_stride + rank] = 0.0f;
    p.out_docs[(uint64_t)out_q * p.out_stride + rank] = TQD_TERMINATED;
  }
  if (lane == 0) p.out_counts[out_q] = count;
}

}

uint32_t tqk_share_capl(int kpl) { return (uint32_t)(kpl + 1) * 64u; }

hipError_t tqk_launch_share(const TqkShareParams &p, int kpl, hipStream_t st) {
  if (p.n_tasks <= p.task_begin || p.grid == 0) return hipSuccess;
  const dim3 grid(p.grid), block(64);
  switch (kpl) {
    case 1: ushare_kernel<1><<<grid, block, 0, st>>>(p); break;
    default: ushare_kernel<2><<<grid, block, 0, st>>>(p); break;
  }
  return hipGetLastError();
}

hipError_t tqk_launch_merge_lists(const TqkMergeParams &m, const uint32_t *list_count, int kpl, bool compact,
                                  hipStream_t st) {
  if (m.n_queries == 0) return hipSuccess;
  const dim3 grid(m.n_queries), block(64);
  if (compact) {
    switch (kpl) {
      case 1: merge_lists_kernel<1, TqdAQuery><<<grid, block, 0, st>>>(m, list_count); break;
      default: merge_lists_kernel<2, TqdAQuery><<<grid, block, 0, st>>>(m, list_count); break;
    }
    return hipGetLastError();
  }
  switch (kpl) {
    case 1: merge_lists_kernel<1, TqdQuery><<<grid, block, 0, st>>>(m, list_count); break;
    default: merge_lists_kernel<2, TqdQuery><<<grid, block, 0, st>>>(m, list_count); break;
  }
  return hipGetLastError();
}
```

tantivy_amd/distributed.py:

```python
import ctypes as C
import os
import sys
import time

import numpy as np

from . import binding as B


def allgather_topk(scores, docs, counts, group=None):
    import torch
    import torch.distributed as dist

    world = dist.get_world_size(group)
    n, k = scores.shape
    packed = torch.empty(n * (2 * k + 1), dtype=torch.int32, device=scores.device)
    packed[: n * k] = scores.contiguous().view(torch.int32).reshape(-1)
    packed[n * k: 2 * n * k] = docs.contiguous().view(torch.int32).reshape(-1)
    packed[2 * n * k:] = counts.contiguous().view(torch.int32).reshape(-1)
    out = torch.empty(world * packed.numel(), dtype=torch.int32, device=scores.device)
    dist.all_gather_into_tensor(out, packed, group=group)
    out = out.view(world, -1)
    g_scores = out[:, : n * k].contiguous().view(torch.float32).view(world, n, k)
    g_docs = out[:, n * k: 2 * n * k].contiguous().view(world, n, k)
# ... 50 lines not shown
        lib_name = C.c_char_p()
        B._check(L.tq_comm_info(self._c, None, None, C.byref(lib_name)))
        self.library = (lib_name.value or b"").decode()

    def allgather_topk(self, scores, docs, counts, out, stream):
        rows, k = scores.shape
        B._check(B.lib().tq_allgather_topk(
            self._c, scores.data_ptr(), docs.data_ptr(), counts.data_ptr(), rows, k,
            out[0].data_ptr(), out[1].data_ptr(), out[2].data_ptr(), C.c_void_p(stream)))

    def close(self):
        if self._c:
            B.lib().tq_comm_free(self._c)
            self._c = C.c_void_p()


def exchange_topk(local, n, k, n_local, world, comm=None, torch_group=None, gathered=None, stream=None,
                  force=False):
    sc, dc, ct = local
    S, W = n_local, world
    if W > 1 or force:
        if comm is not None:
            comm.allgather_topk(sc, dc, ct, gathered, stream)
            g = gathered
        else:
            g = allgather_topk(sc, dc, ct, group=torch_group)
    else:
        g = (sc.unsqueeze(0), dc.unsqueeze(0), ct.unsqueeze(0))
    return g[0].reshape(W * S, n, k), g[1].reshape(W * S, n, k), g[2].reshape(W * S, n)


class ShardRunner:

    def __init__(self, segments, device, rank=0, world=1, remote_stats=(), comm=None,
                 torch_group=None, force_exchange=False):
        import torch

        from . import DeviceIndex

        self.torch = torch
        self.dev = DeviceIndex(segments, devices=[device] * max(1, len(segments)))
        self.n_local = len(segments)
        self.device, self.rank, self.world = device, rank, world
        for st in remote_stats:
            self.dev.add_remote_stats(*st)
        self.comm, self.torch_group = comm, torch_group
        self.force_exchange = force_exchange
        self.stream_obj = torch.cuda.Stream(device=device)
        self.stream = self.stream_obj.cuda_stream
        self._ev_ring = [(torch.cuda.Event(enable_timing=True), torch.cuda.Event(enable_timing=True)) for _ in range(16)]
        self._ev_at = 0
        self._trace = bool(os.environ.get("TQ_RUNNER_TRACE"))
        self.n = self.k = 0
        self._ex_events = []
        self._agree("local segments per rank", self.n_local)

    def _agree(self, what, value):
        if self.world <= 1:
            return
        import torch.distributed as dist

        if not (dist.is_available() and dist.is_initialized()):
            return
        seen = [None] * dist.get_world_size()
        dist.all_gather_object(seen, value)
        if any(v != value for v in seen):
            raise ValueError("ShardRunner: ranks disagree on %s: %r" % (what, seen))

    def _any_rank(self, flag):
        if self.world <= 1:
            return bool(flag)
        import torch.distributed as dist

        if not (dist.is_available() and dist.is_initialized()):
            return bool(flag)
        dev = self.torch.device("cuda", self.device) if dist.get_backend() == "nccl" else "cpu"
        t = self.torch.tensor([1 if flag else 0], dtype=self.torch.int32, device=dev)
        dist.all_reduce(t, op=dist.ReduceOp.MAX)
        return bool(int(t.item()))

    def set_option(self, name, value):
        self.dev.set_option(name, value)

    def prepare(self, queries, k, marshalled=None):
        torch = self.torch
        if marshalled is not None:
            self.dev.prepare_marshalled(marshalled)
        else:
            self.dev.prepare(queries)
        n, S, W = len(queries), self.n_local, self.world
        changed = (n, k) != (self.n, self.k)
        if self._any_rank(changed):
            self._agree("(queries per batch, k)", (n, k))
        if not changed:
            return
        self.n, self.k = n, k
        cuda = torch.device("cuda", self.device)
        self.local = (torch.empty((S * n, k), dtype=torch.float32, device=cuda),
                      torch.empty((S * n, k), dtype=torch.int32, device=cuda),
                      torch.empty(S * n, dtype=torch.int32, device=cuda))
        if W > 1 or self.force_exchange:
            self.gathered = (torch.empty((W, S * n, k), dtype=torch.float32, device=cuda),
                             torch.empty((W, S * n, k), dtype=torch.int32, device=cuda),
                             torch.empty((W, S * n), dtype=torch.int32, device=cuda))
        self._merged_all = torch.empty(n * (3 * k + 1), dtype=torch.int32, device=cuda)
        self._host_all = torch.empty(n * (3 * k + 1), dtype=torch.int32).pin_memory()

        def views(buf):
            return (buf[0:n * k].view(torch.float32).view(n, k), buf[n * k:2 * n * k].view(n, k),
                    buf[2 * n * k:3 * n * k].view(n, k), buf[3 * n * k:3 * n * k + n])

        self._zero_copy = os.environ.get("TQ_RUNNER_D2H_COPY", "0") != "1"
        self.host = list(views(self._host_all))
        self.merged = tuple(self.host) if self._zero_copy else views(self._merged_all)

    def prepare_next(self, queries, k, marshalled):
        if (len(queries), k) != (self.n, self.k):
            raise ValueError("prepare_next: the next batch must have the shape of the current one")
        self.dev.prepare_next_async(marshalled)

    def commit_next(self):
        return self.dev.commit_next()

    def enqueue(self):
        torch = self.torch
        n, k, S, W = self.n, self.k, self.n_local, self.world
        sc, dc, ct = self.local
        tr = self._trace
        t0 = time.perf_counter() if tr else 0.0
        with torch.cuda.stream(self.stream_obj):
            t0b = time.perf_counter() if tr else 0.0
            for s in range(S):
                self.dev.collect_segment_prepared_device(
                    s, k, sc[s * n:(s + 1) * n], dc[s * n:(s + 1) * n], ct[s * n:(s + 1) * n],
                    self.stream)
            t1 = time.perf_counter() if tr else 0.0
            ev = self._ev_ring[self._ev_at % 16]
            self._ev_at += 1
            ev[0].record(self.stream_obj)
            t2 = time.perf_counter() if tr else 0.0
            g = exchange_topk((sc, dc, ct), n, k, S, W, self.comm, self.torch_group,
                              getattr(self, "gathered", None), self.stream, self.force_exchange)
            merge_gathered_device(self.dev.ctx, self.device, g[0], g[1], g[2], 0, k, self.stream,
                                  out=self.merged)
            t3 = time.perf_counter() if tr else 0.0
            ev[1].record(self.stream_obj)
            self._ex_events = [e for e in self._ex_events if e is not ev][-15:] + [ev]
            t4 = time.perf_counter() if tr else 0.0
            if not self._zero_copy:
                B._check(B.lib().tq_copy_to_host_async(
                    self.dev.ctx, int(self.device), self._host_all.data_ptr(), self._merged_all.data_ptr(),
                    self._merged_all.numel() * 4, C.c_void_p(self.stream)))
            t5 = time.perf_counter() if tr else 0.0
        if tr and time.perf_counter() - t0 > 0.003:
            t6 = time.perf_counter()
            print("[runner] enter-stream %.2f collect %.2f ev0 %.2f exchange+merge %.2f ev1 %.2f copy %.2f exit-stream %.2f ms" %
                  tuple((b - a) * 1e3 for a, b in ((t0, t0b), (t0b, t1), (t1, t2), (t2, t3), (t3, t4), (t4, t5), (t5, t6))),
                  file=sys.stderr)

    def synchronize(self):
        self.stream_obj.synchronize()

    def results(self):
        return [h.clone().numpy() for h in self.host]

    def batch_stats(self):
        out = None
        for s in range(self.n_local):
            st = self.dev.last_batch_stats(s)
            if out is None:
                out = dict(st)
            else:
                for key in ("algorithmic_bytes", "matches", "kernel_ms", "total_ms", "tiles", "chunks",
                            "host_plan_ms", "unique_bytes"):
                    out[key] += st[key]
                out["kernel_mask"] |= st["kernel_mask"]
                out["kernels"] = sorted(set(out["kernels"]) | set(st["kernels"]))
        return out

    def exchange_ms(self):
        if not self._ex_events:
            return 0.0
        self.stream_obj.synchronize()
        ms = [a.elapsed_time(b) for a, b in self._ex_events]
        self._ex_events = []
        return float(sum(ms) / len(ms))

    def close(self):
        self.dev.close()
```

tantivy_amd/host/host_capi.cpp:

```cpp
#include <atomic>
#include <chrono>
#include <condition_variable>
#include <mutex>
#include <cstring>
#include <ctime>
#include <cstdio>
#include <cstdlib>
#include <memory>
#include <string>
#include <thread>
#include <vector>

#include "searcher.hpp"
#include "term_info_store.hpp"

using namespace tantivy_amd;

namespace {
thread_local std::string g_err;
template <typename F>
int guard(F &&f) {
  try {
    f();
    return TQ_OK;
  } catch (const TantivyError &e) {
    g_err = e.what();
    switch (e.kind) {
      case TantivyError::InvalidArgument: return TQ_ERR_INVALID;
      case TantivyError::DataCorruption: return TQ_ERR_FORMAT;
      case TantivyError::Unsupported: return TQ_ERR_UNSUPPORTED;
      default: return TQ_ERR_HIP;
    }
  } catch (const std::exception &e) {
    g_err = e.what();
    return TQ_ERR_INVALID;
  }
}
}

struct tqh_searcher {
  tq_ctx *ctx = nullptr;
  std::vector<std::shared_ptr<SegmentReader>> segments;
  std::unique_ptr<Searcher> searcher;
  std::vector<Weight> prepared;
  std::vector<Weight> prepared_next;
};

extern "C" {

struct tqh_term_info {
  uint32_t term_id;
  uint32_t doc_freq;
  uint64_t postings_start, postings_end, positions_start, positions_end;
};
#define TQH_MODE_TERM 4
struct tqh_query {
  uint8_t mode;
  uint32_t n_terms;
  const uint32_t *terms;
  const uint32_t *phrase_offsets;
  const uint8_t *occurs;
  const uint8_t *clause_of;
  uint32_t min_should_match;
  const float *boosts;
  const uint8_t *nested_occurs;
  const uint8_t *clause_min_should;
  const uint8_t *atom_of;
  const uint32_t *set_terms;
  const uint32_t *set_starts;
};
#define TQH_TERM_SET_BASE 0xFFFFFF00u

const char *tqh_last_error(void) { return g_err.c_str(); }

int tqh_searcher_new(tq_ctx *ctx, tqh_searcher **out) {
  return guard([&] {
    if (!ctx || !out) throw TantivyError(TantivyError::InvalidArgument, "null argument");
    auto *s = new tqh_searcher();
    s->ctx = ctx;
    *out = s;
  });
}
void tqh_searcher_free(tqh_searcher *s) { delete s; }

static void reserve_densest_columns(SegmentReader &seg, std::vector<std::pair<uint32_t, uint64_t>> &by_df) {
  const size_t keep = std::min<size_t>(by_df.size(), 40);
  std::partial_sort(by_df.begin(), by_df.begin() + keep, by_df.end(),
                    [](const std::pair<uint32_t, uint64_t> &a, const std::pair<uint32_t, uint64_t> &b) {
                      return a.first != b.first ? a.first > b.first : a.second < b.second;
                    });
  std::vector<uint64_t> offs;
  for (size_t i = 0; i < keep; ++i) offs.push_back(by_df[i].second);
  if (tq_segment_reserve_columns(seg.raw(), offs.data(), (uint32_t)offs.size()) != TQ_OK)
    throw TantivyError(TantivyError::SystemError, tq_last_error());
}
static void reserve_densest_columns(SegmentReader &seg, const TermInfoStore &st) {
  std::vector<std::pair<uint32_t, uint64_t>> by_df;
  by_df.reserve(st.num_terms());
  for (uint64_t o = 0; o < st.num_terms(); ++o) {
    const TermInfo ti = st.get(o);
    by_df.emplace_back(ti.doc_freq, ti.postings_start);
  }
  reserve_densest_columns(seg, by_df);
}

int tqh_searcher_add_segment(tqh_searcher *s, int device, uint32_t max_doc, uint8_t record_option,
                             const uint8_t *idx, size_t idx_len, const uint8_t *pos,
                             size_t pos_len, const uint8_t *fieldnorm, size_t fn_len,
                             const tqh_term_info *terms, uint32_t n_terms) {
  return guard([&] {
    if (!s) throw TantivyError(TantivyError::InvalidArgument, "null searcher");
    auto seg = std::make_shared<SegmentReader>(s->ctx, device, (uint32_t)s->segments.size(),
                                               max_doc, record_option, idx, idx_len, pos, pos_len,
                                               fieldnorm, fn_len);
    for (uint32_t i = 0; i < n_terms; ++i) {
      TermInfo ti;
      ti.doc_freq = terms[i].doc_freq;
      ti.postings_start = terms[i].postings_start;
      ti.postings_end = terms[i].postings_end;
      ti.positions_start = terms[i].positions_start;
      ti.positions_end = terms[i].positions_end;
      seg->add_term(terms[i].term_id, ti);
    }
    {
      std::vector<std::pair<uint32_t, uint64_t>> by_df;
      by_df.reserve(n_terms);
      for (uint32_t i = 0; i < n_terms; ++i) by_df.emplace_back(terms[i].doc_freq, terms[i].postings_start);
      reserve_densest_columns(*seg, by_df);
    }
    s->segments.push_back(seg);
    s->searcher.reset(new Searcher(s->segments));
  });
}

int tqh_searcher_add_segment_with_store(tqh_searcher *s, int device, uint32_t max_doc,
                                        uint8_t record_option, const uint8_t *idx, size_t idx_len,
                                        const uint8_t *pos, size_t pos_len,
                                        const uint8_t *fieldnorm, size_t fn_len,
                                        const uint8_t *store, size_t store_len) {
  return guard([&] {
    if (!s) throw TantivyError(TantivyError::InvalidArgument, "null searcher");
    auto st = std::make_shared<TermInfoStore>(TermInfoStore::open(store, store_len));
    auto seg = std::make_shared<SegmentReader>(s->ctx, device, (uint32_t)s->segments.size(),
                                               max_doc, record_option, idx, idx_len, pos, pos_len,
                                               fieldnorm, fn_len);
    seg->set_term_info_store(st);
    reserve_densest_columns(*seg, *st);
    s->segments.push_back(seg);
    s->searcher.reset(new Searcher(s->segments));
  });
}

int tqh_searcher_add_segment_device_with_store(tqh_searcher *s, int device, uint32_t max_doc,
                                               uint8_t record_option, const uint8_t *d_idx,
                                               size_t idx_len, const uint8_t *d_pos, size_t pos_len,
                                               const uint8_t *d_fieldnorm, size_t fn_len,
                                               uint64_t total_num_tokens, const uint8_t *store,
                                               size_t store_len) {
  return guard([&] {
    if (!s) throw TantivyError(TantivyError::InvalidArgument, "null searcher");
    auto st = std::make_shared<TermInfoStore>(TermInfoStore::open(store, store_len));
    auto seg = std::make_shared<SegmentReader>(SegmentReader::DeviceResident{}, s->ctx, device,
                                               (uint32_t)s->segments.size(), max_doc, record_option,
                                               d_idx, idx_len, d_pos, pos_len, d_fieldnorm, fn_len,
                                               total_num_tokens);
    seg->set_term_info_store(st);
    reserve_densest_columns(*seg, *st);
    s->segments.push_back(seg);
    s->searcher.reset(new Searcher(s->segments));
  });
}

int tqh_searcher_add_remote_stats(tqh_searcher *s, uint64_t max_doc, uint64_t total_num_tokens,
                                  const uint32_t *term_ids, const uint32_t *doc_freqs,
                                  uint32_t n_terms) {
  return guard([&] {
    if (!s || !s->searcher) throw TantivyError(TantivyError::InvalidArgument, "no segments");
    std::vector<std::pair<uint32_t, uint32_t>> v;
    for (uint32_t i = 0; i < n_terms; ++i) v.emplace_back(term_ids[i], doc_freqs[i]);
    s->searcher->add_remote_statistics(max_doc, total_num_tokens, v);
  });
}

static bool is_set_entry(const tqh_query &q, uint32_t t) {
  return q.set_terms && q.set_starts && q.terms[t] >= TQH_TERM_SET_BASE && q.terms[t] < TQH_TERM_SET_BASE + TQ_MAX_TERMS;
}
static Query set_query_of(const tqh_query &q, uint32_t t) {
  const uint32_t j = q.terms[t] - TQH_TERM_SET_BASE;
  if (q.set_starts[j + 1] < q.set_starts[j]) throw TantivyError(TantivyError::InvalidArgument, "set_starts must ascend");
  return Query::term_set(std::vector<uint32_t>(q.set_terms + q.set_starts[j], q.set_terms + q.set_starts[j + 1])).boosted(q.boosts ? q.boosts[t] : 1.0f);
}

static Query build_query(const tqh_query &q) {
  Query query;
  if (q.mode > TQH_MODE_TERM)
    throw TantivyError(TantivyError::InvalidArgument, "unknown query mode");
  if (q.n_terms == 0) throw TantivyError(TantivyError::InvalidArgument, "query without terms");
  if (q.mode == TQ_MODE_BOOL) {
    if (!q.occurs) throw TantivyError(TantivyError::InvalidArgument, "TQ_MODE_BOOL needs occurs");
    std::vector<std::pair<Occur, Query>> clauses;
    std::vector<int> ids;
    std::vector<uint32_t> first_term_of;
    std::vector<std::vector<int>> atom_ids(TQ_MAX_TERMS + 1);
    std::vector<char> nested_built(TQ_MAX_TERMS + 1, 0);
    auto in_phrase = [&](uint32_t tt) {
      return q.nested_occurs && q.nested_occurs[tt] != 255 && (q.nested_occurs[tt] & TQ_NESTED_PHRASE) != 0;
    };
    auto leaf_of = [&](uint32_t tt) {
      if (is_set_entry(q, tt)) return set_query_of(q, tt);
      if (q.terms[tt] == TQ_TERM_ALL) return Query::all().boosted(q.boosts ? q.boosts[tt] : 1.0f);
      if (in_phrase(tt))
        return Query::phrase_with_offsets({{q.phrase_offsets ? q.phrase_offsets[tt] : 0u, q.terms[tt]}}).boosted(q.boosts ? q.boosts[tt] : 1.0f);
      return Query::term_query(q.terms[tt]).boosted(q.boosts ? q.boosts[tt] : 1.0f);
    };
    for (uint32_t t = 0; t < q.n_terms; ++t) {
      if (q.occurs[t] > 2) throw TantivyError(TantivyError::InvalidArgument, "bad occur");
      const Occur oc = q.occurs[t] == 1 ? Occur::Must
                                        : (q.occurs[t] == 2 ? Occur::MustNot : Occur::Should);
      const int id = q.clause_of ? (int)q.clause_of[t] : -1;
      size_t c = ids.size();
// ... 188 lines not shown
            segment_ords[(size_t)qi * limit + i] = real ? res[i].second.segment_ord : 0xFFFFFFFFu;
            docs[(size_t)qi * limit + i] = real ? res[i].second.doc_id : TERMINATED;
          }
        }
      } catch (const TantivyError &e) {
        errors[t] = e.what();
        kinds[t] = e.kind;
      } catch (const std::exception &e) {
        errors[t] = e.what();
      }
      if (conc_trace) {
        clock_gettime(CLOCK_THREAD_CPUTIME_ID, &c1);
        callers_cpu_ns.fetch_add((uint64_t)((c1.tv_sec - c0.tv_sec) * 1000000000ll + (c1.tv_nsec - c0.tv_nsec)), std::memory_order_relaxed);
      }
    };
    std::vector<std::thread> threads;
    for (uint32_t t = 1; t < n_threads; ++t) threads.emplace_back(work, t);
    work(0);
    for (std::thread &th : threads) th.join();
    if (wall_ms) *wall_ms = std::chrono::duration<double, std::milli>(std::chrono::steady_clock::now() - t0).count();
    if (conc_trace)
      fprintf(stderr, "[tqh] %u threads, %u queries: %.1f us of CPU per query inside the calling threads (from the starting line on)\n", n_threads, n,
              (double)callers_cpu_ns.load() / 1e3 / (double)std::max<uint32_t>(1u, n));
    for (uint32_t t = 0; t < n_threads; ++t)
      if (!errors[t].empty()) throw TantivyError(kinds[t], errors[t]);
  });
}

int tqh_collect_segment_prepared(tqh_searcher *s, uint32_t segment_ord, uint32_t k, float *scores,
                                 uint32_t *docs, uint32_t *counts) {
  return guard([&] {
    if (!s || !s->searcher || segment_ord >= s->segments.size())
      throw TantivyError(TantivyError::InvalidArgument, "bad segment");
    std::vector<float> sc;
    std::vector<uint32_t> dc, ct;
    s->searcher->collect_segment_batch(segment_ord, s->prepared, k, sc, dc, ct);
    std::memcpy(scores, sc.data(), sc.size() * sizeof(float));
    std::memcpy(docs, dc.data(), dc.size() * sizeof(uint32_t));
    std::memcpy(counts, ct.data(), ct.size() * sizeof(uint32_t));
  });
}

int tqh_collect_segment_prepared_device(tqh_searcher *s, uint32_t segment_ord, uint32_t k,
                                        float *d_scores, uint32_t *d_docs, uint32_t *d_counts,
                                        void *hip_stream) {
  return guard([&] {
    if (!s || !s->searcher || segment_ord >= s->segments.size())
      throw TantivyError(TantivyError::InvalidArgument, "bad segment");
    s->searcher->collect_segment_batch_device(segment_ord, s->prepared, k, d_scores, d_docs,
                                              d_counts, hip_stream);
  });
}

int tqh_bm25_for_terms(const uint64_t *term_doc_freqs, uint32_t n_terms, uint64_t total_num_docs,
                       uint64_t total_num_tokens, float boost, float *weight_out,
                       float *cache_out ) {
  return guard([&] {
    if (!term_doc_freqs || !n_terms || !weight_out)
      throw TantivyError(TantivyError::InvalidArgument, "null argument");
    std::vector<uint64_t> dfs(term_doc_freqs, term_doc_freqs + n_terms);
    Bm25Weight w = Bm25Weight::for_terms(dfs, total_num_docs, total_num_tokens).boost_by(boost);
    *weight_out = w.weight;
    if (cache_out) std::memcpy(cache_out, w.cache, sizeof w.cache);
  });
}

tq_segment *tqh_segment_raw(tqh_searcher *s, uint32_t segment_ord) {
  if (!s || segment_ord >= s->segments.size()) return nullptr;
  return s->segments[segment_ord]->raw();
}
uint32_t tqh_term_handle(tqh_searcher *s, uint32_t segment_ord, uint32_t term_id) {
  if (!s || segment_ord >= s->segments.size()) return TQ_TERM_ABSENT;
  uint32_t h = TQ_TERM_ABSENT;
  guard([&] { h = s->segments[segment_ord]->term_handle(term_id); });
  return h;
}

int tqh_count_prepared(tqh_searcher *s, uint64_t *counts) {
  return guard([&] {
    if (!s || !s->searcher || !counts) throw TantivyError(TantivyError::InvalidArgument, "null argument");
    const std::vector<uint64_t> c = s->searcher->count_batch(s->prepared);
    if (!c.empty()) std::memcpy(counts, c.data(), c.size() * sizeof(uint64_t));
  });
}

int tqh_docset_prepared(tqh_searcher *s, uint32_t *out_segment_ords, uint32_t *out_docs, uint64_t out_cap,
                        uint64_t *out_starts) {
  return guard([&] {
    if (!s || !s->searcher || !out_starts || (out_cap && (!out_segment_ords || !out_docs)))
      throw TantivyError(TantivyError::InvalidArgument, "null argument");
    const std::vector<std::vector<DocAddress>> rows = s->searcher->docset_batch(s->prepared);
    uint64_t at = 0;
    for (size_t q = 0; q < rows.size(); ++q) {
      out_starts[q] = at;
      at += rows[q].size();
    }
    out_starts[rows.size()] = at;
    if (at > out_cap) throw TantivyError(TantivyError::InvalidArgument, "output buffer too small");
    for (size_t q = 0; q < rows.size(); ++q)
      for (size_t i = 0; i < rows[q].size(); ++i) {
        out_segment_ords[out_starts[q] + i] = rows[q][i].segment_ord;
        out_docs[out_starts[q] + i] = rows[q][i].doc_id;
      }
  });
}

// ... 86 lines not shown
```

tantivy_amd/host/searcher.cpp:

```cpp
#include "searcher.hpp"

#include "term_info_store.hpp"

#include <algorithm>
#include <cmath>
#include <cstring>

namespace tantivy_amd {

namespace {
[[noreturn]] void throw_tq(int code) {
  const std::string msg = tq_last_error();
  switch (code) {
    case TQ_ERR_INVALID: throw TantivyError(TantivyError::InvalidArgument, msg);
    case TQ_ERR_FORMAT: throw TantivyError(TantivyError::DataCorruption, msg);
    case TQ_ERR_UNSUPPORTED: throw TantivyError(TantivyError::Unsupported, msg);
    default: throw TantivyError(TantivyError::SystemError, msg);
  }
}
}

SegmentReader::SegmentReader(tq_ctx *ctx, int device, uint32_t segment_ord, uint32_t max_doc,
                             uint8_t record_option, const uint8_t *idx, size_t idx_len,
                             const uint8_t *pos, size_t pos_len, const uint8_t *fieldnorm,
// ... 19 lines not shown
SegmentReader::~SegmentReader() {
  tq_segment_free(seg_);
  delete[] fast_handles_.load(std::memory_order_relaxed);
}

void SegmentReader::add_term(uint32_t term_id, const TermInfo &info) { terms_[term_id] = info; }
void SegmentReader::set_term_info_store(std::shared_ptr<const TermInfoStore> store) {
  store_ = std::move(store);
}
const TermInfo *SegmentReader::get_term_info(uint32_t term_id) const {
  std::lock_guard<std::mutex> lk(m_);
  auto it = terms_.find(term_id);
  if (it == terms_.end() && store_ && term_id < store_->num_terms())
    it = terms_.emplace(term_id, store_->get(term_id)).first;
  if (it == terms_.end() || it->second.doc_freq == 0) return nullptr;
  return &it->second;
}
tq_term_handle SegmentReader::term_handle(uint32_t term_id) {
  if (term_id == TQ_TERM_ALL) return TQ_TERM_ALL;
  if (term_id < kFastHandles) {
    std::atomic<tq_term_handle> *fast = fast_handles_.load(std::memory_order_acquire);
    if (fast) {
      const tq_term_handle h = fast[term_id].load(std::memory_order_acquire);
      if (h != kHandleUnknown) return h;
    }
  }
  {
    std::lock_guard<std::mutex> lk(m_);
    auto h = handles_.find(term_id);
    if (h != handles_.end()) return h->second;
  }
  const TermInfo *ti = get_term_info(term_id);
  tq_term_handle handle = TQ_TERM_ABSENT;
  if (ti) {
    const int rc = tq_term_prepare(seg_, ti->postings_start,
                                   (uint32_t)(ti->postings_end - ti->postings_start),
                                   ti->positions_start,
                                   (uint32_t)(ti->positions_end - ti->positions_start),
                                   ti->doc_freq, &handle);
    if (rc != TQ_OK) throw_tq(rc);
  }
  std::lock_guard<std::mutex> lk(m_);
  handles_[term_id] = handle;
  if (term_id < kFastHandles) {
    std::atomic<tq_term_handle> *fast = fast_handles_.load(std::memory_order_relaxed);
    if (!fast) {
      fast = new std::atomic<tq_term_handle>[kFastHandles];
      for (uint32_t i = 0; i < kFastHandles; ++i) fast[i].store(kHandleUnknown, std::memory_order_relaxed);
      fast_handles_.store(fast, std::memory_order_release);
    }
    fast[term_id].store(handle, std::memory_order_release);
  }
  return handle;
}

void SegmentReader::prepare_terms(const uint32_t *term_ids, size_t n) {
  std::vector<uint32_t> fresh;
  {
    std::atomic<tq_term_handle> *fast = fast_handles_.load(std::memory_order_acquire);
    std::unordered_map<uint32_t, char> seen;
    for (size_t i = 0; i < n; ++i) {
      const uint32_t t = term_ids[i];
      if (t == TQ_TERM_ALL) continue;
      if (t < kFastHandles && fast && fast[t].load(std::memory_order_acquire) != kHandleUnknown) continue;
      if (!seen.emplace(t, 1).second) continue;
      {
        std::lock_guard<std::mutex> lk(m_);
        if (handles_.count(t)) continue;
      }
      fresh.push_back(t);
    }
  }
  if (fresh.size() < 2) return;
  std::vector<tq_term_info> infos;
  std::vector<uint32_t> ids;
  for (uint32_t t : fresh) {
    const TermInfo *ti = get_term_info(t);
    if (!ti) continue;
    tq_term_info x{};
    x.postings_off = ti->postings_start;
    x.postings_len = (uint32_t)(ti->postings_end - ti->postings_start);
    x.positions_off = ti->positions_start;
    x.positions_len = (uint32_t)(ti->positions_end - ti->positions_start);
    x.doc_freq = ti->doc_freq;
    infos.push_back(x);
    ids.push_back(t);
  }
  if (infos.empty()) return;
  std::vector<tq_term_handle> hs(infos.size(), TQ_TERM_ABSENT);
  const int rc = tq_term_prepare_batch(seg_, infos.data(), (uint32_t)infos.size(), hs.data());
  if (rc != TQ_OK) throw_tq(rc);
  std::lock_guard<std::mutex> lk(m_);
  std::atomic<tq_term_handle> *fast = fast_handles_.load(std::memory_order_relaxed);
  if (!fast) {
    fast = new std::atomic<tq_term_handle>[kFastHandles];
    for (uint32_t i = 0; i < kFastHandles; ++i) fast[i].store(kHandleUnknown, std::memory_order_relaxed);
    fast_handles_.store(fast, std::memory_order_release);
  }
  for (size_t i = 0; i < ids.size(); ++i) {
    handles_[ids[i]] = hs[i];
    if (ids[i] < kFastHandles) fast[ids[i]].store(hs[i], std::memory_order_release);
  }
}

WeightTermSet::~WeightTermSet() {
  for (auto &p : prepared_)
    if (std::shared_ptr<SegmentReader> seg = p.first.lock()) (void)tq_term_set_release(seg->raw(), p.second);
}
tq_term_handle WeightTermSet::handle(const std::shared_ptr<SegmentReader> &seg) {
  std::lock_guard<std::mutex> lk(m_);
  for (auto &p : prepared_)
    if (p.first.lock() == seg) return p.second;
  seg->prepare_terms(term_ids_.data(), term_ids_.size());
  std::vector<tq_term_handle> hs;
  hs.reserve(term_ids_.size());
  for (uint32_t t : term_ids_) hs.push_back(seg->term_handle(t));
  tq_term_handle h = TQ_TERM_ABSENT;
  const int rc = tq_term_set_prepare(seg->raw(), hs.data(), (uint32_t)hs.size(), &h);
  if (rc != TQ_OK) throw_tq(rc);
  prepared_.emplace_back(seg, h);
  return h;
}
namespace {
tq_term_handle resolve_handle(const std::shared_ptr<SegmentReader> &seg, const Weight &w, uint32_t t) {
  if (t >= kTermSetBase && (size_t)(t - kTermSetBase) < w.sets.size()) return w.sets[t - kTermSetBase]->handle(seg);
  return seg->term_handle(t);
}
}

Searcher::Searcher(std::vector<std::shared_ptr<SegmentReader>> segments)
    : segments_(std::move(segments)) {}
Searcher::~Searcher() { delete[] fast_weights_.load(std::memory_order_relaxed); }

void Searcher::add_remote_statistics(
    uint64_t max_doc, uint64_t total_num_tokens,
    const std::vector<std::pair<uint32_t, uint32_t>> &term_doc_freqs) {
  remote_docs_ += max_doc;
  remote_tokens_ += total_num_tokens;
  for (auto &tf : term_doc_freqs) remote_doc_freq_[tf.first] += tf.second;
  shared_cache_.reset();
  if (std::atomic<uint32_t> *fw = fast_weights_.load(std::memory_order_acquire))
    for (uint32_t i = 0; i < kFastWeights; ++i) fw[i].store(0xFFFFFFFFu, std::memory_order_relaxed);
}

Score Searcher::term_weight_cached(uint32_t term, uint64_t nd) const {
  std::atomic<uint32_t> *fw = term < kFastWeights ? fast_weights_.load(std::memory_order_acquire) : nullptr;
  if (fw) {
    const uint32_t bits = fw[term].load(std::memory_order_relaxed);
    if (bits != 0xFFFFFFFFu) {
      Score w;
      std::memcpy(&w, &bits, sizeof w);
      return w;
    }
  }
  const Score w = idf(doc_freq(term), nd) * (1.0f + K1);
  if (term < kFastWeights) {
    if (!fw) {
      std::lock_guard<std::mutex> lk(cache_m_);
      fw = fast_weights_.load(std::memory_order_relaxed);
      if (!fw) {
        fw = new std::atomic<uint32_t>[kFastWeights];
        for (uint32_t i = 0; i < kFastWeights; ++i) fw[i].store(0xFFFFFFFFu, std::memory_order_relaxed);
        fast_weights_.store(fw, std::memory_order_release);
      }
    }
    uint32_t bits;
    std::memcpy(&bits, &w, sizeof bits);
    fw[term].store(bits, std::memory_order_relaxed);
  }
  return w;
}

Searcher::FlatContext Searcher::flat_context() const {
  FlatContext fc;
  fc.nd = total_num_docs();
  const uint64_t nt = total_num_tokens();
  if (fc.nd == 0)
    throw TantivyError(TantivyError::InvalidArgument, "no documents: BM25 statistics undefined");
  std::lock_guard<std::mutex> lk(cache_m_);
  if (!shared_cache_) {
    const Score avg = (Score)nt / (Score)fc.nd;
    shared_cache_ = std::make_shared<Bm25Weight>(Bm25Weight::from_idf(0.0f, avg));
  }
  fc.cache = shared_cache_;
  return fc;
// ... 220 lines not shown
            w.terms.push_back(kTermSetBase + (uint32_t)w.sets.size());
            w.sets.push_back(std::make_shared<WeightTermSet>(c.second.set_terms));
          } else {
            w.terms.push_back((uint32_t)TQ_TERM_ALL);
          }
          w.weights.push_back(bc);
          if (w.mode == TQ_MODE_BOOL) {
            w.occurs.push_back(oc);
            w.clause_of.push_back(clause);
            if (tree) {
              w.nested_occurs.push_back((uint8_t)TQ_MUST);
              w.atom_of.push_back(member);
            }
          }
        } else if (c.second.kind == Query::Term) {
          add(c.second.term, bc, Occur::Must);
        } else if (c.second.kind == Query::Phrase) {
          add_phrase(c.second, bc, Occur::Must);
        } else {
          for (auto &sub : c.second.clauses) {
            if (sub.second.kind == Query::Term)
              add(sub.second.term, bc * sub.second.boost, sub.first);
            else if (sub.second.kind == Query::Phrase)
              add_phrase(sub.second, bc * sub.second.boost, sub.first);
            else if (is_member_union(sub.second))
              for (auto &leaf : sub.second.clauses) add(leaf.second.term, bc * sub.second.boost * leaf.second.boost, sub.first, TQ_NESTED_ANY);
            else
              for (auto &leaf : sub.second.clauses) add(leaf.second.term, bc * sub.second.boost * leaf.second.boost, sub.first);
            ++member;
          }
          if (tree && c.second.minimum_number_should_match) {
            if (clause >= TQ_MAX_TERMS || c.second.minimum_number_should_match > 255)
              throw TantivyError(TantivyError::Unsupported, "nested minimum_number_should_match out of range");
            if (w.clause_min_should.empty()) w.clause_min_should.assign(TQ_MAX_TERMS, 0);
            w.clause_min_should[clause] = (uint8_t)c.second.minimum_number_should_match;
          }
        }
        ++clause;
      }
      if (w.terms.size() > TQ_MAX_TERMS)
        throw TantivyError(TantivyError::Unsupported, "more than 16 terms stay on the CPU");
      if (any_phrase) w.phrase_offsets.resize(w.terms.size(), 0u);
      w.min_should_match = (uint32_t)std::min<size_t>(msm, 0xFFFFu);
      return w;
    }
  }
  throw TantivyError(TantivyError::InvalidArgument, "unknown query kind");
}

namespace {
struct SegmentBatch {
  std::vector<tq_query> qs;
  std::vector<tq_term_handle> handles;
  SegmentBatch(const std::shared_ptr<SegmentReader> &seg_p, const std::vector<Weight> &weights, uint32_t k) {
    SegmentReader &seg = *seg_p;
    const size_t n = weights.size();
    qs.resize(n);
    size_t total_terms = 0;
    for (auto &w : weights) total_terms += w.terms.size();
    handles.reserve(total_terms);
    if (n > 1) {
      std::vector<uint32_t> all;
      all.reserve(total_terms);
      for (auto &w : weights)
        for (uint32_t t : w.terms)
          if (t < kTermSetBase) all.push_back(t);
      seg.prepare_terms(all.data(), all.size());
    }
    for (size_t i = 0; i < n; ++i) {
      const Weight &w = weights[i];
      const size_t at = handles.size();
      for (uint32_t t : w.terms) handles.push_back(resolve_handle(seg_p, w, t));
      tq_query &q = qs[i];
      q.n_terms = (uint32_t)w.terms.size();
      q.terms = handles.data() + at;
      q.weights = w.weights.data();
      q.tf_cache = w.bm25->cache;
      q.mode = w.mode;
      q.phrase_offsets = w.phrase_offsets.empty() ? nullptr : w.phrase_offsets.data();
      q.k = k;
      q.occurs = w.occurs.empty() ? nullptr : w.occurs.data();
      q.clause_of = w.clause_of.empty() ? nullptr : w.clause_of.data();
      q.min_should_match = w.min_should_match;
      q.nested_occurs = w.nested_occurs.empty() ? nullptr : w.nested_occurs.data();
      q.clause_min_should = w.clause_min_should.empty() ? nullptr : w.clause_min_should.data();
      q.atom_of = w.atom_of.empty() ? nullptr : w.atom_of.data();
    }
  }
};
}

uint32_t Searcher::bound_slack_ppm(const SegmentReader &seg) const {
  const double global = (double)total_num_tokens() / (double)total_num_docs();
  const double local = seg.max_doc() ? (double)seg.total_num_tokens() / (double)seg.max_doc() : global;
  double ppm = 0.0;
  if (global > 0.0 && local > 0.0 && global != local) {
    const double d = std::abs(global - local) / std::min(global, local);
    ppm = std::ceil(((1.0 + d) * (1.0 + d) - 1.0) * 1e6) + 2.0;
  }
  return (uint32_t)std::min(ppm, 1e9);
}

void Searcher::collect_segment_batch(size_t segment_ord, const std::vector<Weight> &weights,
                                     uint32_t k, std::vector<float> &scores,
                                     std::vector<uint32_t> &docs, std::vector<uint32_t> &counts) {
  SegmentReader &seg = *segments_[segment_ord];
  const size_t n = weights.size();
  SegmentBatch b(segments_[segment_ord], weights, k);
  scores.assign(n * k, 0.0f);
  docs.assign(n * k, TERMINATED);
  counts.assign(n, 0);
  const tq_search_opts opts{-1, bound_slack_ppm(seg)};
  const int rc = tq_search_batch_opts(seg.raw(), b.qs.data(), (uint32_t)n, k, scores.data(),
                                      docs.data(), counts.data(), &opts);
  if (rc != TQ_OK) throw_tq(rc);
}

std::vector<uint64_t> Searcher::count_batch(const std::vector<Weight> &weights) {
  std::vector<uint64_t> total(weights.size(), 0);
  std::vector<uint32_t> per(weights.size());
  for (auto &seg : segments_) {
    SegmentBatch b(seg, weights, 1);
    const int rc = tq_count_batch(seg->raw(), b.qs.data(), (uint32_t)weights.size(), per.data());
    if (rc != TQ_OK) throw_tq(rc);
    for (size_t i = 0; i < per.size(); ++i) total[i] += per[i];
  }
  return total;
}

std::vector<std::vector<DocAddress>> Searcher::docset_batch(const std::vector<Weight> &weights) {
  const size_t n = weights.size();
  std::vector<std::vector<DocAddress>> out(n);
  std::vector<uint64_t> starts(n + 1);
  std::vector<uint32_t> docs;
  for (auto &seg : segments_) {
    SegmentBatch b(seg, weights, 1);
    int rc = tq_docset_batch(seg->raw(), b.qs.data(), (uint32_t)n, docs.data(), docs.size(), starts.data());
    if (rc == TQ_ERR_INVALID && starts[n] > docs.size()) {
      docs.resize(starts[n]);
      rc = tq_docset_batch(seg->raw(), b.qs.data(), (uint32_t)n, docs.data(), docs.size(), starts.data());
    }
    if (rc != TQ_OK) throw_tq(rc);
    for (size_t q = 0; q < n; ++q) {
      out[q].reserve(out[q].size() + (size_t)(starts[q + 1] - starts[q]));
      for (uint64_t i = starts[q]; i < starts[q + 1]; ++i) out[q].push_back(DocAddress{seg->segment_ord(), docs[i]});
    }
  }
  return out;
}

std::vector<std::vector<std::pair<DocAddress, Score>>> Searcher::docset_scored_batch(const std::vector<Weight> &weights) {
  const size_t n = weights.size();
  std::vector<std::vector<std::pair<DocAddress, Score>>> out(n);
  std::vector<uint64_t> starts(n + 1);
  std::vector<uint32_t> docs;
  std::vector<float> scores;
  for (auto &seg : segments_) {
    SegmentBatch b(seg, weights, 1);
    int rc = tq_docset_scored_batch(seg->raw(), b.qs.data(), (uint32_t)n, docs.data(), scores.data(), docs.size(), starts.data());
    if (rc == TQ_ERR_INVALID && starts[n] > docs.size()) {
      docs.resize(starts[n]);
      scores.resize(starts[n]);
      rc = tq_docset_scored_batch(seg->raw(), b.qs.data(), (uint32_t)n, docs.data(), scores.data(), docs.size(), starts.data());
    }
    if (rc != TQ_OK) throw_tq(rc);
    for (size_t q = 0; q < n; ++q) {
      out[q].reserve(out[q].size() + (size_t)(starts[q + 1] - starts[q]));
      for (uint64_t i = starts[q]; i < starts[q + 1]; ++i)
        out[q].push_back({DocAddress{seg->segment_ord(), docs[i]}, scores[i]});
    }
  }
  return out;
}

void Searcher::collect_segment_batch_device(size_t segment_ord, const std::vector<Weight> &weights,
                                            uint32_t k, float *d_scores, uint32_t *d_docs,
                                            uint32_t *d_counts, void *hip_stream) {
  SegmentReader &seg = *segments_[segment_ord];
  SegmentBatch b(segments_[segment_ord], weights, k);
  const tq_search_opts opts{-1, bound_slack_ppm(seg)};
  const int rc = tq_search_batch_device_opts(seg.raw(), b.qs.data(), (uint32_t)weights.size(), k,
                                             d_scores, d_docs, d_counts, &opts, hip_stream);
  if (rc != TQ_OK) throw_tq(rc);
}

std::vector<Fruit> Searcher::search_batch(const std::vector<Weight> &weights,
                                          const TopDocs &collector) {
  const size_t n = weights.size(), S = segments_.size();
  const uint32_t k = (uint32_t)(collector.offset() + collector.limit());
  if (k > TQ_MAX_K)
    throw TantivyError(TantivyError::Unsupported, "offset+limit above the device heap size");
  std::vector<float> all_scores(S * n * k);
  std::vector<uint32_t> all_docs(S * n * k), all_counts(S * n);
  std::vector<float> sc;
  std::vector<uint32_t> dc, ct;
  for (size_t s = 0; s < S; ++s) {
    collect_segment_batch(s, weights, k, sc, dc, ct);
    std::memcpy(all_scores.data() + s * n * k, sc.data(), n * k * sizeof(float));
    std::memcpy(all_docs.data() + s * n * k, dc.data(), n * k * sizeof(uint32_t));
    std::memcpy(all_counts.data() + s * n, ct.data(), n * sizeof(uint32_t));
  }
  const uint32_t limit = (uint32_t)collector.limit(), offset = (uint32_t)collector.offset();
  std::vector<float> out_s(n * limit);
  std::vector<uint32_t> out_o(n * limit), out_d(n * limit), out_c(n);
  const int rc = tq_merge_topk(all_scores.data(), all_docs.data(), all_counts.data(), (uint32_t)S,
                               (uint32_t)n, k, offset, limit, out_s.data(), out_o.data(),
                               out_d.data(), out_c.data());
  if (rc != TQ_OK) throw_tq(rc);
  std::vector<Fruit> res(n);
  for (size_t q = 0; q < n; ++q) {
    res[q].reserve(out_c[q]);
    for (uint32_t i = 0; i < out_c[q]; ++i)
      res[q].push_back({out_s[q * limit + i],
                        DocAddress{segments_[out_o[q * limit + i]]->segment_ord(),
                                   out_d[q * limit + i]}});
  }
  return res;
}

Fruit Searcher::search(const Query &query, const TopDocs &collector) {
  const Weight w = weight(query);
  const size_t S = segments_.size();
  const uint32_t k = (uint32_t)(collector.offset() + collector.limit());
  if (k > TQ_MAX_K)
    throw TantivyError(TantivyError::Unsupported, "offset+limit above the device heap size");
  std::vector<float> all_scores(S * k);
  std::vector<uint32_t> all_docs(S * k), all_counts(S);
  std::vector<tq_term_handle> handles(w.terms.size());
  for (size_t s = 0; s < S; ++s) {
    SegmentReader &seg = *segments_[s];
    for (size_t i = 0; i < w.terms.size(); ++i) handles[i] = resolve_handle(segments_[s], w, w.terms[i]);
    tq_query q{};
    q.n_terms = (uint32_t)w.terms.size();
    q.terms = handles.data();
    q.weights = w.weights.data();
// ... 31 lines not shown
```

tantivy_amd/host/searcher.hpp:

```cpp
#pragma once
#include <atomic>
#include <memory>
#include <mutex>
#include <stdexcept>
#include <string>
#include <unordered_map>
#include <utility>
#include <vector>

#include "../../include/tantivy_amd.h"
#include "bm25.hpp"

namespace tantivy_amd {

struct TantivyError : std::runtime_error {
  enum Kind { InvalidArgument, SchemaError, SystemError, DataCorruption, Unsupported } kind;
  TantivyError(Kind k, const std::string &msg) : std::runtime_error(msg), kind(k) {}
};

struct TermInfo {
  uint32_t doc_freq = 0;
  uint64_t postings_start = 0, postings_end = 0;
  uint64_t positions_start = 0, positions_end = 0;
};

struct DocAddress {
  uint32_t segment_ord = 0;
  DocId doc_id = 0;
  bool operator==(const DocAddress &o) const {
    return segment_ord == o.segment_ord && doc_id == o.doc_id;
  }
};

class SegmentReader {
 public:
  SegmentReader(tq_ctx *ctx, int device, uint32_t segment_ord, uint32_t max_doc,
                uint8_t record_option, const uint8_t *idx, size_t idx_len, const uint8_t *pos,
                size_t pos_len, const uint8_t *fieldnorm, size_t fn_len);
  struct DeviceResident {};
  SegmentReader(DeviceResident, tq_ctx *ctx, int device, uint32_t segment_ord, uint32_t max_doc,
                uint8_t record_option, const uint8_t *d_idx, size_t idx_len, const uint8_t *d_pos,
                size_t pos_len, const uint8_t *d_fieldnorm, size_t fn_len, uint64_t total_num_tokens);
  ~SegmentReader();
  SegmentReader(const SegmentReader &) = delete;
  SegmentReader &operator=(const SegmentReader &) = delete;

  void add_term(uint32_t term_id, const TermInfo &info);
  void set_term_info_store(std::shared_ptr<const class TermInfoStore> store);
  const TermInfo *get_term_info(uint32_t term_id) const;
  tq_term_handle term_handle(uint32_t term_id);
  void prepare_terms(const uint32_t *term_ids, size_t n);
  uint32_t max_doc() const { return max_doc_; }
  uint32_t segment_ord() const { return segment_ord_; }
  uint64_t total_num_tokens() const { return total_num_tokens_; }
  uint8_t record_option() const { return record_option_; }
  tq_segment *raw() const { return seg_; }

 private:
  tq_segment *seg_ = nullptr;
  uint32_t segment_ord_, max_doc_;
  uint8_t record_option_;
  uint64_t total_num_tokens_ = 0;
  mutable std::mutex m_;
  mutable std::unordered_map<uint32_t, TermInfo> terms_;
  std::unordered_map<uint32_t, tq_term_handle> handles_;
  static constexpr uint32_t kFastHandles = 1u << 20;
  static constexpr tq_term_handle kHandleUnknown = 0xFFFFFFFEu;
  std::atomic<std::atomic<tq_term_handle> *> fast_handles_{nullptr};
  std::shared_ptr<const class TermInfoStore> store_;
};

enum class Occur { Should, Must, MustNot };

struct Query {
  enum Kind { Term, Boolean, Phrase, All, TermSet } kind;
  uint32_t term = 0;
  std::vector<uint32_t> set_terms;
  std::vector<std::pair<Occur, Query>> clauses;
  size_t minimum_number_should_match = 0;
  Score boost = 1.0f;
  std::vector<std::pair<uint32_t, uint32_t>> phrase_terms;

  static Query term_query(uint32_t term) {
    Query q;
    q.kind = Term;
    q.term = term;
    return q;
  }
  static Query all() {
    Query q;
    q.kind = All;
    return q;
  }
  static Query term_set(std::vector<uint32_t> term_ids) {
    Query q;
    q.kind = TermSet;
    q.set_terms = std::move(term_ids);
    return q;
  }
  static Query boolean(std::vector<std::pair<Occur, Query>> clauses) {
    Query q;
    q.kind = Boolean;
    q.clauses = std::move(clauses);
    return q;
// ... 142 lines not shown
  std::mutex m_;
  std::vector<std::pair<std::weak_ptr<SegmentReader>, tq_term_handle>> prepared_;
};
constexpr uint32_t kTermSetBase = 0xFFFFFF00u;

struct Weight {
  uint8_t mode = TQ_MODE_AND;
  std::vector<std::shared_ptr<WeightTermSet>> sets;
  InlineVec<uint32_t, 4> terms;
  InlineVec<Score, 4> weights;
  std::vector<uint32_t> phrase_offsets;
  std::vector<uint8_t> occurs;
  std::vector<uint8_t> clause_of;
  std::vector<uint8_t> nested_occurs;
  std::vector<uint8_t> atom_of;
  std::vector<uint8_t> clause_min_should;
  uint32_t min_should_match = 0;
  std::shared_ptr<Bm25Weight> bm25;
};

class Searcher {
 public:
  explicit Searcher(std::vector<std::shared_ptr<SegmentReader>> segments);
  ~Searcher();
  Searcher(const Searcher &) = delete;
  Searcher &operator=(const Searcher &) = delete;
  uint64_t total_num_docs() const;
  uint64_t total_num_tokens() const;
  uint64_t doc_freq(uint32_t term) const;
  size_t num_segments() const { return segments_.size(); }
  SegmentReader &segment_reader(size_t ord) { return *segments_[ord]; }

  void add_remote_statistics(uint64_t max_doc, uint64_t total_num_tokens,
                             const std::vector<std::pair<uint32_t, uint32_t>> &term_doc_freqs);

  Weight weight(const Query &query) const;
  Weight weight_flat(uint8_t mode, const uint32_t *terms, uint32_t n_terms) const;
  struct FlatContext {
    uint64_t nd = 0;
    std::shared_ptr<Bm25Weight> cache;
  };
  FlatContext flat_context() const;
  void weight_flat_into(const FlatContext &fc, uint8_t mode, const uint32_t *terms, uint32_t n_terms, Weight &w) const;
  Fruit search(const Query &query, const TopDocs &collector);
  std::vector<Fruit> search_batch(const std::vector<Weight> &weights, const TopDocs &collector);
  std::vector<uint64_t> count_batch(const std::vector<Weight> &weights);
  std::vector<std::vector<DocAddress>> docset_batch(const std::vector<Weight> &weights);
  std::vector<std::vector<std::pair<DocAddress, Score>>> docset_scored_batch(const std::vector<Weight> &weights);
  void collect_segment_batch(size_t segment_ord, const std::vector<Weight> &weights, uint32_t k,
                             std::vector<float> &scores, std::vector<uint32_t> &docs,
                             std::vector<uint32_t> &counts);
  void collect_segment_batch_device(size_t segment_ord, const std::vector<Weight> &weights,
                                    uint32_t k, float *d_scores, uint32_t *d_docs,
                                    uint32_t *d_counts, void *hip_stream);

 private:
  uint32_t bound_slack_ppm(const SegmentReader &seg) const;
  std::vector<std::shared_ptr<SegmentReader>> segments_;
  mutable std::mutex cache_m_;
  mutable std::shared_ptr<Bm25Weight> shared_cache_;
  static constexpr uint32_t kFastWeights = 1u << 20;
  mutable std::atomic<std::atomic<uint32_t> *> fast_weights_{nullptr};
  Score term_weight_cached(uint32_t term, uint64_t nd) const;
  uint64_t remote_docs_ = 0, remote_tokens_ = 0;
  std::unordered_map<uint32_t, uint64_t> remote_doc_freq_;
};

}
```

Baseline: 11.12 million queries/s.

## Inline warm tasks into ashare band ordering and add device-side prepared search path

Adds an ashare_inline_warm mode (default on) in which the warm-up tasks of the AND-share plan are no longer run as a separate kernel phase. Independent tasks are instead ordered into bands so they fill the resident grid alongside the warm tasks, and the two-phase launch collapses into one. This is meant to remove the phase barrier and the idle compute units during warm-up, at the risk of dependent tasks running with weaker pruning thresholds. Separately, it adds a device-resident prepared-search API that writes segment ords directly, reuses a cached SegmentBatch, skips re-preparing known term handles, and adds timing events for the merge.

```diff
diff --git a/include/tantivy_amd.h b/include/tantivy_amd.h
--- a/include/tantivy_amd.h
+++ b/include/tantivy_amd.h
@@ -110,6 +110,10 @@
                                 uint32_t out_stride, float *d_out_scores, uint32_t *d_out_docs,
                                 uint32_t *d_out_counts, const tq_search_opts *opts,
                                 void *hip_stream);
+int tq_search_batch_device_rows(tq_segment *seg, const tq_query *queries, uint32_t n_queries,
+                                uint32_t out_stride, float *d_out_scores, uint32_t *d_out_segment_ords,
+                                uint32_t *d_out_docs, uint32_t *d_out_counts, uint32_t segment_ord,
+                                const tq_search_opts *opts, void *hip_stream);
 
 typedef struct tq_ticket tq_ticket;
 int tq_submit(tq_segment *seg, const tq_query *query, const tq_search_opts *opts, float *out_scores,
diff --git a/include/tantivy_amd_host.h b/include/tantivy_amd_host.h
--- a/include/tantivy_amd_host.h
+++ b/include/tantivy_amd_host.h
@@ -59,6 +59,10 @@
 int tqh_collect_segment_prepared_device(tqh_searcher *s, uint32_t segment_ord, uint32_t k,
                                         float *d_scores, uint32_t *d_docs, uint32_t *d_counts,
                                         void *hip_stream);
+int tqh_search_prepared_device(tqh_searcher *s, uint32_t k, float *out_scores, uint32_t *out_segment_ords,
+                               uint32_t *out_docs, uint32_t *out_counts, float *d_slab_scores,
+                               uint32_t *d_slab_docs, uint32_t *d_slab_counts, void *hip_stream);
+int tqh_exchange_ms(tqh_searcher *s, float *ms);
 int tqh_bm25_for_terms(const uint64_t *term_doc_freqs, uint32_t n_terms, uint64_t total_num_docs,
                        uint64_t total_num_tokens, float boost, float *weight_out,
                        float *cache_out);
diff --git a/tantivy_amd/binding.py b/tantivy_amd/binding.py
--- a/tantivy_amd/binding.py
+++ b/tantivy_amd/binding.py
@@ -118,7 +118,7 @@
     "tq_init", "tq_shutdown", "tq_last_error", "tq_segment_upload", "tq_segment_upload_device",
     "tq_segment_free",
     "tq_term_prepare", "tq_term_prepare_batch", "tq_search_batch", "tq_search_batch_device", "tq_search_batch_opts",
-    "tq_search_batch_device_opts", "tq_merge_topk",
+    "tq_search_batch_device_opts", "tq_search_batch_device_rows", "tq_merge_topk",
     "tq_merge_topk_device", "tq_copy_to_host_async", "tq_decode_postings", "tq_decode_position_deltas",
     "tq_last_batch_stats", "tq_segment_get_stats", "tq_segment_reserve_columns", "tq_set_option", "tq_segment_set_alive_bitset", "tq_count_batch",
     "tq_last_batch_match_counts", "tq_last_batch_query_kernels", "tq_encoder_create", "tq_encoder_free", "tq_encode_postings",
@@ -127,7 +127,7 @@
     "tq_comm_info", "tq_allgather_topk",
     "tqh_last_error", "tqh_searcher_new", "tqh_searcher_free", "tqh_searcher_add_segment",
     "tqh_prepare_batch", "tqh_prepare_batch_next", "tqh_commit_next", "tqh_search_prepared", "tqh_collect_segment_prepared",
-    "tqh_collect_segment_prepared_device", "tqh_searcher_add_remote_stats",
+    "tqh_collect_segment_prepared_device", "tqh_search_prepared_device", "tqh_exchange_ms", "tqh_searcher_add_remote_stats",
     "tqh_bm25_for_terms", "tqh_segment_raw", "tqh_term_handle", "tqh_term_dictionary_values",
     "tqh_term_info_store_open", "tqh_term_info_store_free", "tqh_term_info_store_num_terms",
     "tqh_term_info_store_get", "tqh_term_info_store_write", "tqh_searcher_add_segment_with_store",
@@ -167,6 +167,8 @@
                                        u32p, C.POINTER(TqSearchOpts)]
     L.tq_search_batch_device_opts.argtypes = [vp, C.POINTER(TqQuery), C.c_uint32, C.c_uint32, vp,
                                               vp, vp, C.POINTER(TqSearchOpts), vp]
+    L.tq_search_batch_device_rows.argtypes = [vp, C.POINTER(TqQuery), C.c_uint32, C.c_uint32, vp, vp,
+                                              vp, vp, C.c_uint32, C.POINTER(TqSearchOpts), vp]
     L.tq_merge_topk.argtypes = [f32p, u32p, u32p, C.c_uint32, C.c_uint32, C.c_uint32, C.c_uint32,
                                 C.c_uint32, f32p, u32p, u32p, u32p]
     L.tq_copy_to_host_async.argtypes = [vp, C.c_int, vp, vp, C.c_size_t, vp]
@@ -228,6 +230,8 @@
     L.tq_wait.argtypes = [vp]
     L.tqh_collect_segment_prepared.argtypes = [vp, C.c_uint32, C.c_uint32, f32p, u32p, u32p]
     L.tqh_collect_segment_prepared_device.argtypes = [vp, C.c_uint32, C.c_uint32, vp, vp, vp, vp]
+    L.tqh_search_prepared_device.argtypes = [vp, C.c_uint32, vp, vp, vp, vp, vp, vp, vp, vp]
+    L.tqh_exchange_ms.argtypes = [vp, f32p]
     L.tqh_searcher_add_remote_stats.argtypes = [vp, C.c_uint64, C.c_uint64, u32p, u32p, C.c_uint32]
     L.tqh_bm25_for_terms.argtypes = [C.POINTER(C.c_uint64), C.c_uint32, C.c_uint64, C.c_uint64,
                                      C.c_float, f32p, f32p]
@@ -662,6 +666,17 @@
             self._s, int(segment_ord), int(k), d_scores.data_ptr(), d_docs.data_ptr(),
             d_counts.data_ptr(), C.c_void_p(stream) if stream else None), host=True)
 
+    def search_prepared_device(self, k, out, slabs=None, stream=None):
+        sl = [t.data_ptr() for t in slabs] if slabs is not None else [None, None, None]
+        _check(lib().tqh_search_prepared_device(
+            self._s, int(k), out[0].data_ptr(), out[1].data_ptr(), out[2].data_ptr(), out[3].data_ptr(),
+            sl[0], sl[1], sl[2], C.c_void_p(stream) if stream else None), host=True)
+
+    def exchange_ms(self):
+        ms = C.c_float(0.0)
+        _check(lib().tqh_exchange_ms(self._s, C.byref(ms)), host=True)
+        return float(ms.value)
+
     @property
     def ctx(self):
         return self._ctx
diff --git a/tantivy_amd/csrc/tq_api.cpp b/tantivy_amd/csrc/tq_api.cpp
--- a/tantivy_amd/csrc/tq_api.cpp
+++ b/tantivy_amd/csrc/tq_api.cpp
@@ -485,6 +485,8 @@
     s->opt.docset_trees = (int)value;
   else if (!strcmp(name, "docset_score_trees") && (value == 0 || value == 1))
     s->opt.docset_score_trees = (int)value;
+  else if (!strcmp(name, "ashare_inline_warm") && value >= 0 && value <= 2)
+    s->opt.ashare_inline_warm = (int)value;
   else if (!strcmp(name, "ashare_min_batch") && value >= 0 && value <= 0x7FFFFFFF)
     s->opt.ashare_min_batch = (int)value;
   else if (!strcmp(name, "xunion_min_queries") && value >= 1 && value <= 0x7FFFFFFF)
diff --git a/tantivy_amd/csrc/tq_common.hpp b/tantivy_amd/csrc/tq_common.hpp
--- a/tantivy_amd/csrc/tq_common.hpp
+++ b/tantivy_amd/csrc/tq_common.hpp
@@ -404,6 +404,30 @@
   }
 }
 
+template <int KPL>
+__device__ __forceinline__ void write_topk_rows(const TqkMergeParams &p, const TopK<KPL> &tk, uint32_t k, uint32_t out_q,
+                                                int lane) {
+  const uint64_t row = (uint64_t)out_q * p.out_stride;
+  uint32_t count = 0;
+#pragma unroll
+  for (int r = 0; r < KPL; ++r) {
+    const uint32_t rank = (uint32_t)r * 64u + (uint32_t)lane;
+    const bool real = rank < k && tk.v[r] != 0ull;
+    count += (uint32_t)__popcll(__ballot(real));
+    if (rank < p.out_stride) {
+      p.out_scores[row + rank] = real ? key_score(tk.v[r]) : 0.0f;
+      p.out_docs[row + rank] = real ? key_doc(tk.v[r]) : TQD_TERMINATED;
+      if (p.out_segment_ords) p.out_segment_ords[row + rank] = real ? p.segment_ord : 0xFFFFFFFFu;
+    }
+  }
+  for (uint32_t rank = (uint32_t)(KPL * 64) + (uint32_t)lane; rank < p.out_stride; rank += 64u) {
+    p.out_scores[row + rank] = 0.0f;
+    p.out_docs[row + rank] = TQD_TERMINATED;
+    if (p.out_segment_ords) p.out_segment_ords[row + rank] = 0xFFFFFFFFu;
+  }
+  if (lane == 0) p.out_counts[out_q] = count;
+}
+
 __device__ __forceinline__ uint32_t sortable(float x) {
   uint32_t fb = __float_as_uint(x);
   return fb ^ ((uint32_t)((int32_t)fb >> 31) | 0x80000000u);
diff --git a/tantivy_amd/csrc/tq_internal.hpp b/tantivy_amd/csrc/tq_internal.hpp
--- a/tantivy_amd/csrc/tq_internal.hpp
+++ b/tantivy_amd/csrc/tq_internal.hpp
@@ -163,6 +163,7 @@
   int docset_temp_lists = 0;
   int docset_trees = 0;
   int docset_score_trees = 0;
+  int ashare_inline_warm = 1;
   int ashare_min_batch = 16;
   int submit_window_us = 100;
   int record_query_kernels = 0;
@@ -522,6 +523,8 @@
     };
     std::vector<ARun> aruns;
     uint32_t a_warm_tasks = 0;
+    bool a_inline = false;
+    uint32_t a_dep_tasks = 0;
     bool over_budget = false;
     bool any_rdir = false;
   };
@@ -795,7 +798,7 @@
 void docset_tree_view(const tq_query &q, TreeView &v, bool scored = false);
 int build_group_chunks(Group &g, bool or_windows, PlanScratch &ps, bool boolean_group = false);
 int build_share_plan(tq_segment *s, Group &g, PlanScratch &ps);
-int build_ashare_plan(tq_segment *s, Group &g, PlanScratch &ps, bool boolean = false);
+int build_ashare_plan(tq_segment *s, Group &g, PlanScratch &ps, bool boolean = false, uint32_t resident = 0);
 int build_dense_plan(tq_segment *s, Group &g, PlanScratch &ps, uint32_t cus);
 int plan_bool_query(tq_segment *s, const tq_query &q, uint32_t qi, TqdQuery &dq, uint64_t &qbytes,
                     uint32_t &n_tiles, uint32_t &tile_cost, uint32_t &n_thr_rows, bool exhaustive);
@@ -807,7 +810,7 @@
 int fail_tree_tables(const tq_segment *s, uint32_t qi);
 int search_batch_impl(tq_segment *s, const tq_query *queries, uint32_t n_queries, uint32_t out_stride,
                       float *d_out_scores, uint32_t *d_out_docs, uint32_t *d_out_counts, void *hip_stream,
-                      const CallOpts &co);
+                      const CallOpts &co, uint32_t *d_out_segment_ords = nullptr, uint32_t segment_ord = 0);
 int search_batch_host(tq_segment *s, const tq_query *queries, uint32_t n_queries, uint32_t out_stride,
                       float *out_scores, uint32_t *out_docs, uint32_t *out_counts, const CallOpts &co);
 struct HostBatchSlot {
diff --git a/tantivy_amd/csrc/tq_launch.h b/tantivy_amd/csrc/tq_launch.h
--- a/tantivy_amd/csrc/tq_launch.h
+++ b/tantivy_amd/csrc/tq_launch.h
@@ -138,6 +138,8 @@
   uint32_t n_queries;
   uint32_t out_stride;
   uint32_t pre_slices;
+  uint32_t *out_segment_ords;
+  uint32_t segment_ord;
 };
 constexpr uint32_t TQK_MERGE_PRE_MIN = 96;
 inline __host__ __device__ uint32_t tqk_merge_slice_lists(uint32_t n_parts, uint32_t pre_slices) {
diff --git a/tantivy_amd/csrc/tq_misc.hip b/tantivy_amd/csrc/tq_misc.hip
--- a/tantivy_amd/csrc/tq_misc.hip
+++ b/tantivy_amd/csrc/tq_misc.hip
@@ -57,23 +57,7 @@
     flush_partial<KPL>(tk, const_cast<uint64_t *>(p.partials), part_start, lane);
     return;
   }
-  const uint32_t out_q = p.out_index ? p.out_index[q] : q;
-  uint32_t count = 0;
-#pragma unroll
-  for (int r = 0; r < KPL; ++r) {
-    const uint32_t rank = (uint32_t)r * 64u + (uint32_t)lane;
-    const bool real = rank < k && tk.v[r] != 0ull;
-    count += (uint32_t)__popcll(__ballot(real));
-    if (rank < p.out_stride) {
-      p.out_scores[(uint64_t)out_q * p.out_stride + rank] = real ? key_score(tk.v[r]) : 0.0f;
-      p.out_docs[(uint64_t)out_q * p.out_stride + rank] = real ? key_doc(tk.v[r]) : TQD_TERMINATED;
-    }
-  }
-  for (uint32_t rank = (uint32_t)(KPL * 64) + (uint32_t)lane; rank < p.out_stride; rank += 64u) {
-    p.out_scores[(uint64_t)out_q * p.out_stride + rank] = 0.0f;
-    p.out_docs[(uint64_t)out_q * p.out_stride + rank] = TQD_TERMINATED;
-  }
-  if (lane == 0) p.out_counts[out_q] = count;
+  write_topk_rows<KPL>(p, tk, k, p.out_index ? p.out_index[q] : q, lane);
 }
 
 __global__ __launch_bounds__(256) void zero_regions_kernel(TqkZeroParams p) {
diff --git a/tantivy_amd/csrc/tq_plan_share.cpp b/tantivy_amd/csrc/tq_plan_share.cpp
--- a/tantivy_amd/csrc/tq_plan_share.cpp
+++ b/tantivy_amd/csrc/tq_plan_share.cpp
@@ -208,7 +208,7 @@
   return TQ_OK;
 }
 
-int build_ashare_plan(tq_segment *s, Group &g, PlanScratch &ps, bool boolean) {
+int build_ashare_plan(tq_segment *s, Group &g, PlanScratch &ps, bool boolean, uint32_t resident) {
   PlanScratch::ASharePlan &A = ps.ap[boolean ? 1 : 0];
   static const uint32_t kTaskPairsEnv = tune_u32("TQ_AS_TASK_PAIRS", 0);
   static const uint32_t kTargetTasks = std::max<uint32_t>(1u, tune_u32("TQ_AS_TARGET_TASKS", 24576));
@@ -604,7 +604,24 @@
   }
   if (n_tasks > 0x7FFFFFFFull) return fail(TQ_ERR_UNSUPPORTED, "batch too large (tasks)");
   tasks.resize(n_tasks);
-  constexpr uint32_t kSl = 4098;
+  uint64_t band2_want = 0;
+  {
+    static const uint32_t kInlineEnv = tune_u32("TQ_AS_INLINE_WARM", 0xFFFFFFFFu);
+    const uint32_t mode = boolean ? 0u : kInlineEnv != 0xFFFFFFFFu ? kInlineEnv : (uint32_t)s->opt.ashare_inline_warm;
+    uint64_t n_warm = 0, n_indep = 0;
+    for (const PlanScratch::ASharePlan::ARun &R : runs) {
+      const uint64_t warm = (uint64_t)((R.nb_warm + kWarmBlocks - 1) / kWarmBlocks) * R.n_groups;
+      n_warm += warm;
+      if (!R.nb_warm) n_indep += (uint64_t)R.n_runs * R.n_groups;
+    }
+    const uint64_t grid = std::min<uint64_t>(n_tasks, resident);
+    band2_want = grid - std::min(grid, n_warm);
+    A.a_inline = n_warm != 0 && (mode == 2u || (mode == 1u && resident != 0 && n_indep >= band2_want));
+    static const bool kBand2All = tune_u32("TQ_AS_BAND2_ALL", 0) != 0;
+    if (kBand2All) band2_want = ~0ull;
+  }
+  const bool bands = A.a_inline;
+  constexpr uint32_t kSl = 4098, kBand3 = 2049;
   const uint32_t t_slabs = n_tasks >= 16384 ? std::min<uint32_t>(plan_threads(), (uint32_t)runs.size()) : 1u;
   std::vector<uint32_t> &hist = A.atask_hist;
   hist.assign((size_t)t_slabs * kSl, 0u);
@@ -622,7 +639,8 @@
     for (uint32_t j0 = 0; j0 < R.n_blocks;) {
       const bool warm = j0 < R.nb_warm;
       const uint32_t nb = warm ? std::min<uint32_t>(kWarmBlocks, R.nb_warm - j0) : std::min<uint32_t>(R.bpt, R.n_blocks - j0);
-      emit(j0, nb, warm ? 0u : 1u + std::min<uint32_t>(4095u, (uint32_t)((j0 * slice_mul) >> 32)));
+      const uint32_t slice = std::min<uint32_t>(4095u, (uint32_t)((j0 * slice_mul) >> 32));
+      emit(j0, nb, warm ? 0u : !bands ? 1u + slice : (R.nb_warm ? kBand3 : 1u) + (slice >> 1));
       j0 += nb;
     }
   };
@@ -639,13 +657,26 @@
   });
   {
     uint32_t run = 0;
-    for (uint32_t sl = 0; sl < kSl; ++sl)
+    auto place = [&](uint32_t sl) {
       for (uint32_t sb = 0; sb < t_slabs; ++sb) {
         const uint32_t n = hist[(size_t)sb * kSl + sl];
         hist[(size_t)sb * kSl + sl] = run;
         run += n;
-        if (sl == 0 && sb + 1 == t_slabs) A.a_warm_tasks = run;
-      }
+      }
+    };
+    place(0);
+    A.a_warm_tasks = A.a_dep_tasks = run;
+    if (!bands) {
+      for (uint32_t sl = 1; sl < kSl; ++sl) place(sl);
+    } else {
+      uint32_t c = 1;
+      while (c < kBand3 && run - A.a_warm_tasks < band2_want) place(c++);
+      A.a_dep_tasks = run;
+      for (uint32_t sl = 0; sl + 1u < kBand3; ++sl) {
+        if (1u + sl >= c) place(1u + sl);
+        place(kBand3 + sl);
+      }
+    }
   }
   parallel_slabs(t_slabs, [&](uint32_t sb) {
     uint32_t *h = hist.data() + (size_t)sb * kSl;
diff --git a/tantivy_amd/csrc/tq_search.cpp b/tantivy_amd/csrc/tq_search.cpp
--- a/tantivy_amd/csrc/tq_search.cpp
+++ b/tantivy_amd/csrc/tq_search.cpp
@@ -25,6 +25,8 @@
   uint32_t *out_docs, *out_counts;
   void *hip_stream;
   CallOpts co;
+  uint32_t *out_segment_ords;
+  uint32_t segment_ord;
   bool replan = false;
   hipStream_t st = nullptr;
   bool exhaustive = false, or_windows = false;
@@ -784,9 +786,15 @@
   return TQ_OK;
 }
 
+uint32_t ashare_resident(int cus) {
+  static const uint32_t kAGridMul = tune_u32("TQ_AS_GRID_MUL", 0);
+  return (uint32_t)std::max(1, cus) * (kAGridMul ? kAGridMul : tqk_ashare_waves_per_cu());
+}
+
 int plan_group_tasks(Batch &b) {
   PlanScratch &ps = *b.ps;
   (void)hipDeviceGetAttribute(&b.cus, hipDeviceAttributeMultiprocessorCount, b.s->device);
+  const bool alone = std::count_if(b.groups, b.groups + kNGroups, [](const Group &g) { return !g.queries.empty(); }) == 1;
   for (int gi = 0; gi < kNGroups; ++gi) {
     Group &g = b.groups[gi];
     if (g.queries.empty()) continue;
@@ -804,7 +812,7 @@
       continue;
     }
     const int rc = gi == kGUShare   ? build_share_plan(b.s, g, ps)
-                   : gi == kGAShare ? build_ashare_plan(b.s, g, ps, false)
+                   : gi == kGAShare ? build_ashare_plan(b.s, g, ps, false, alone ? ashare_resident(b.cus) : 0u)
                    : gi == kGBShare ? build_ashare_plan(b.s, g, ps, true)
                    : gi == kGXUnion ? build_dense_plan(b.s, g, ps, (uint32_t)std::max(1, b.cus))
                                     : build_group_chunks(g, b.or_windows && gi != kGBool, ps, gi == kGBool);
@@ -1071,7 +1079,7 @@
   static const uint32_t kBoundMode = tune_u32("TQ_AS_BOUND", 3);
   ap.bound_mode = kBoundMode;
   ap.n_queues = 1;
-  const uint32_t bounds[3] = {0u, b.ps->ap[ai].a_warm_tasks, g.n_chunks};
+  const uint32_t bounds[3] = {0u, b.ps->ap[ai].a_inline ? g.n_chunks : b.ps->ap[ai].a_warm_tasks, g.n_chunks};
   for (int ph = 0; ph < 2; ++ph) {
     ap.task_begin = bounds[ph];
     ap.n_tasks = bounds[ph + 1];
@@ -1242,6 +1250,8 @@
     m.out_scores = b.out_scores;
     m.out_docs = b.out_docs;
     m.out_counts = b.out_counts;
+    m.out_segment_ords = b.out_segment_ords;
+    m.segment_ord = b.segment_ord;
     m.n_queries = (uint32_t)g.queries.size();
     m.out_stride = b.out_stride;
     if (!kGroupTraits[gi].result_lists) {
@@ -1392,7 +1402,8 @@
 
 int search_batch_impl(tq_segment *s, const tq_query *queries, uint32_t n_queries,
                       uint32_t out_stride, float *d_out_scores, uint32_t *d_out_docs,
-                      uint32_t *d_out_counts, void *hip_stream, const CallOpts &co) {
+                      uint32_t *d_out_counts, void *hip_stream, const CallOpts &co, uint32_t *d_out_segment_ords,
+                      uint32_t segment_ord) {
   if (!s || (!queries && n_queries) || !d_out_scores || !d_out_docs || !d_out_counts)
     return fail(TQ_ERR_INVALID, "tq_search_batch: null argument");
   if (n_queries == 0) return TQ_OK;
@@ -1400,12 +1411,12 @@
   int rc = strip_all_clauses(s, queries, n_queries, strip);
   if (rc != TQ_OK) return rc;
   if (!strip.eff.empty()) queries = strip.eff.data();
-  Batch b{s, queries, n_queries, out_stride, d_out_scores, d_out_docs, d_out_counts, hip_stream, co};
+  Batch b{s, queries, n_queries, out_stride, d_out_scores, d_out_docs, d_out_counts, hip_stream, co, d_out_segment_ords, segment_ord};
   b.n_all_queries = strip.n_all_based;
   b.set_q = strip.n_set ? strip.set_q.data() : nullptr;
   rc = plan_batch(b);
   while (rc != TQ_OK && b.replan) {
-    b = Batch{s, queries, n_queries, out_stride, d_out_scores, d_out_docs, d_out_counts, hip_stream, b.co};
+    b = Batch{s, queries, n_queries, out_stride, d_out_scores, d_out_docs, d_out_counts, hip_stream, b.co, d_out_segment_ords, segment_ord};
     b.n_all_queries = strip.n_all_based;
     b.set_q = strip.n_set ? strip.set_q.data() : nullptr;
     rc = plan_batch(b);
@@ -1514,6 +1525,26 @@
   }
 }
 
+int tq_search_batch_device_rows(tq_segment *s, const tq_query *queries, uint32_t n_queries,
+                                uint32_t out_stride, float *d_out_scores, uint32_t *d_out_segment_ords,
+                                uint32_t *d_out_docs, uint32_t *d_out_counts, uint32_t segment_ord,
+                                const tq_search_opts *opts, void *hip_stream) {
+  if (!s) return fail(TQ_ERR_INVALID, "tq_search_batch: null segment");
+  if (!d_out_segment_ords) return fail(TQ_ERR_INVALID, "tq_search_batch_device_rows: null argument");
+  try {
+    TQ_SEGMENT_LOCK(s);
+    CallOpts co;
+    const int rc = resolve_opts(s, opts, co);
+    if (rc != TQ_OK) return rc;
+    return search_batch_impl(s, queries, n_queries, out_stride, d_out_scores, d_out_docs,
+                             d_out_counts, hip_stream, co, d_out_segment_ords, segment_ord);
+  } catch (const std::exception &e) {
+    return fail(TQ_ERR_HIP, "tq_search_batch_device_rows: %s", e.what());
+  } catch (...) {
+    return fail(TQ_ERR_HIP, "tq_search_batch_device_rows: unknown exception");
+  }
+}
+
 int tq_search_batch(tq_segment *s, const tq_query *queries, uint32_t n_queries,
                     uint32_t out_stride, float *out_scores, uint32_t *out_docs,
                     uint32_t *out_counts) {
diff --git a/tantivy_amd/csrc/tq_ushare.hip b/tantivy_amd/csrc/tq_ushare.hip
--- a/tantivy_amd/csrc/tq_ushare.hip
+++ b/tantivy_amd/csrc/tq_ushare.hip
@@ -771,44 +771,77 @@
   if (lane == 0 && n_scored) atomicAdd(sload(&p.sinks->match_counter), (unsigned long long)n_scored);
 }
 
+constexpr uint32_t kMergeWaves = 16, kMergeStageRow = 64;
 template <int KPL, typename QT>
-__global__ __launch_bounds__(64) void merge_lists_kernel(TqkMergeParams p, const uint32_t *list_count) {
+__global__ __launch_bounds__(64 * kMergeWaves) void merge_lists_kernel(TqkMergeParams p, const uint32_t *list_count) {
+  __shared__ uint32_t s_rows[3][kMergeWaves * kMergeStageRow];
+  __shared__ uint32_t s_out_q[kMergeWaves], s_count[kMergeWaves];
   const int lane = (int)__lane_id();
-  const uint32_t q = blockIdx.x;
-  if (q >= p.n_queries) return;
-  const QT *Q = uni_ptr(reinterpret_cast<const QT *>(p.queries) + q);
-  const uint32_t k = uni(Q->k);
-  const uint32_t n = uni(list_count[uni(Q->chunk_first)]);
-  const uint64_t *src = p.partials + (size_t)uni(Q->part_start);
-  TopK<KPL> tk;
-  tk.reset(k);
-  for (uint32_t i0 = 0; i0 < n; i0 += 256u) {
-    uint64_t keys[4];
-#pragma unroll
-    for (uint32_t u = 0; u < 4u; ++u) {
-      const uint32_t i = i0 + 64u * u + (uint32_t)lane;
-      keys[u] = i < n ? src[i] : 0ull;
-    }
-#pragma unroll
-    for (uint32_t u = 0; u < 4u; ++u) tk.offer(keys[u] != 0ull, keys[u], lane);
+  const uint32_t wave = uni(threadIdx.x >> 6);
+  const uint32_t q0 = blockIdx.x * kMergeWaves, q = q0 + wave;
+  const bool staged = p.out_stride <= kMergeStageRow;
+  if (q < p.n_queries) {
+    const QT *Q = uni_ptr(reinterpret_cast<const QT *>(p.queries) + q);
+    const uint32_t k = uni(Q->k);
+    const uint32_t n = uni(list_count[uni(Q->chunk_first)]);
+    const uint64_t *src = p.partials + (size_t)uni(Q->part_start);
+    TopK<KPL> tk;
+    tk.reset(k);
+    for (uint32_t i0 = 0; i0 < n; i0 += 256u) {
+      uint64_t keys[4];
+#pragma unroll
+      for (uint32_t u = 0; u < 4u; ++u) {
+        const uint32_t i = i0 + 64u * u + (uint32_t)lane;
+        keys[u] = i < n ? src[i] : 0ull;
+      }
+#pragma unroll
+      for (uint32_t u = 0; u < 4u; ++u) tk.offer(keys[u] != 0ull, keys[u], lane);
+    }
+    const uint32_t out_q = p.out_index ? p.out_index[q] : q;
+    if (!staged) {
+      write_topk_rows<KPL>(p, tk, k, out_q, lane);
+    } else {
+      const bool real = (uint32_t)lane < k && tk.v[0] != 0ull;
+      const uint32_t count = (uint32_t)__popcll(__ballot(real));
+      if ((uint32_t)lane < p.out_stride) {
+        const uint32_t at = wave * p.out_stride + (uint32_t)lane;
+        s_rows[0][at] = real ? __float_as_uint(key_score(tk.v[0])) : __float_as_uint(0.0f);
+        s_rows[1][at] = real ? key_doc(tk.v[0]) : TQD_TERMINATED;
+        s_rows[2][at] = real ? p.segment_ord : 0xFFFFFFFFu;
+      }
+      if (lane == 0) {
+        s_out_q[wave] = out_q;
+        s_count[wave] = count;
+      }
+    }
   }
-  const uint32_t out_q = p.out_index ? p.out_index[q] : q;
-  uint32_t count = 0;
-#pragma unroll
-  for (int r = 0; r < KPL; ++r) {
-    const uint32_t rank = (uint32_t)r * 64u + (uint32_t)lane;
-    const bool real = rank < k && tk.v[r] != 0ull;
-    count += (uint32_t)__popcll(__ballot(real));
-    if (rank < p.out_stride) {
-      p.out_scores[(uint64_t)out_q * p.out_stride + rank] = real ? key_score(tk.v[r]) : 0.0f;
-      p.out_docs[(uint64_t)out_q * p.out_stride + rank] = real ? key_doc(tk.v[r]) : TQD_TERMINATED;
-    }
+  if (!staged) return;
+  __syncthreads();
+  const uint32_t n_live = p.n_queries - q0 < kMergeWaves ? p.n_queries - q0 : kMergeWaves;
+  const uint32_t base = s_out_q[0];
+  const bool in_run = (uint32_t)lane >= n_live || s_out_q[(uint32_t)lane < n_live ? lane : 0] == base + (uint32_t)lane;
+  const bool contiguous = __ballot(in_run) == ~0ull;
+  uint32_t *o_scores = reinterpret_cast<uint32_t *>(p.out_scores);
+  if (contiguous) {
+    const uint32_t i = threadIdx.x;
+    if (i < n_live * p.out_stride) {
+      const uint64_t o = (uint64_t)base * p.out_stride + i;
+      o_scores[o] = s_rows[0][i];
+      p.out_docs[o] = s_rows[1][i];
+      if (p.out_segment_ords) p.out_segment_ords[o] = s_rows[2][i];
+    }
+    if (i < n_live) p.out_counts[base + i] = s_count[i];
+  } else if (q < p.n_queries) {
+    const uint32_t out_q = s_out_q[wave];
+    if ((uint32_t)lane < p.out_stride) {
+      const uint32_t at = wave * p.out_stride + (uint32_t)lane;
+      const uint64_t o = (uint64_t)out_q * p.out_stride + (uint32_t)lane;
+      o_scores[o] = s_rows[0][at];
+      p.out_docs[o] = s_rows[1][at];
+      if (p.out_segment_ords) p.out_segment_ords[o] = s_rows[2][at];
+    }
+    if (lane == 0) p.out_counts[out_q] = s_count[wave];
   }
-  for (uint32_t rank = (uint32_t)(KPL * 64) + (uint32_t)lane; rank < p.out_stride; rank += 64u) {
-    p.out_scores[(uint64_t)out_q * p.out_stride + rank] = 0.0f;
-    p.out_docs[(uint64_t)out_q * p.out_stride + rank] = TQD_TERMINATED;
-  }
-  if (lane == 0) p.out_counts[out_q] = count;
 }
 
 }
@@ -828,7 +861,7 @@
 hipError_t tqk_launch_merge_lists(const TqkMergeParams &m, const uint32_t *list_count, int kpl, bool compact,
                                   hipStream_t st) {
   if (m.n_queries == 0) return hipSuccess;
-  const dim3 grid(m.n_queries), block(64);
+  const dim3 grid((m.n_queries + kMergeWaves - 1u) / kMergeWaves), block(64u * kMergeWaves);
   if (compact) {
     switch (kpl) {
       case 1: merge_lists_kernel<1, TqdAQuery><<<grid, block, 0, st>>>(m, list_count); break;
diff --git a/tantivy_amd/distributed.py b/tantivy_amd/distributed.py
--- a/tantivy_amd/distributed.py
+++ b/tantivy_amd/distributed.py
@@ -126,6 +126,7 @@
         self._ev_at = 0
         self._trace = bool(os.environ.get("TQ_RUNNER_TRACE"))
         self.n = self.k = 0
+        self._native_args = None
         self._ex_events = []
         self._agree("local segments per rank", self.n_local)
 
@@ -187,6 +188,11 @@
         self._zero_copy = os.environ.get("TQ_RUNNER_D2H_COPY", "0") != "1"
         self.host = list(views(self._host_all))
         self.merged = tuple(self.host) if self._zero_copy else views(self._merged_all)
+        self._native_args = None
+        if W == 1 and not self.force_exchange and os.environ.get("TQ_RUNNER_ONE_CALL", "1") != "0":
+            slabs = [t.data_ptr() for t in self.local] if S > 1 else [None, None, None]
+            self._native_args = (self.dev._s, int(k)) + tuple(t.data_ptr() for t in self.merged) + tuple(slabs) + \
+                (C.c_void_p(self.stream),)
 
     def prepare_next(self, queries, k, marshalled):
         if (len(queries), k) != (self.n, self.k):
@@ -197,6 +203,16 @@
         return self.dev.commit_next()
 
     def enqueue(self):
+        if self._native_args is not None:
+            t0 = time.perf_counter() if self._trace else 0.0
+            B._check(B.lib().tqh_search_prepared_device(*self._native_args), host=True)
+            if not self._zero_copy:
+                B._check(B.lib().tq_copy_to_host_async(
+                    self.dev.ctx, int(self.device), self._host_all.data_ptr(), self._merged_all.data_ptr(),
+                    self._merged_all.numel() * 4, C.c_void_p(self.stream)))
+            if self._trace and time.perf_counter() - t0 > 0.003:
+                print("[runner] native step %.2f ms" % ((time.perf_counter() - t0) * 1e3), file=sys.stderr)
+            return
         torch = self.torch
         n, k, S, W = self.n, self.k, self.n_local, self.world
         sc, dc, ct = self.local
@@ -253,6 +269,9 @@
         return out
 
     def exchange_ms(self):
+        if self._native_args is not None:
+            self.stream_obj.synchronize()
+            return self.dev.exchange_ms()
         if not self._ex_events:
             return 0.0
         self.stream_obj.synchronize()
diff --git a/tantivy_amd/host/host_capi.cpp b/tantivy_amd/host/host_capi.cpp
--- a/tantivy_amd/host/host_capi.cpp
+++ b/tantivy_amd/host/host_capi.cpp
@@ -10,6 +10,8 @@
 #include <string>
 #include <thread>
 #include <vector>
+
+#include <hip/hip_runtime_api.h>
 
 #include "searcher.hpp"
 #include "term_info_store.hpp"
@@ -44,6 +46,16 @@
   std::unique_ptr<Searcher> searcher;
   std::vector<Weight> prepared;
   std::vector<Weight> prepared_next;
+  int device = 0;
+  bool one_device = true;
+  static constexpr uint32_t kExRing = 16;
+  hipEvent_t ex_ev[kExRing][2] = {};
+  uint32_t ex_at = 0, ex_n = 0;
+  ~tqh_searcher() {
+    for (auto &pair : ex_ev)
+      for (hipEvent_t e : pair)
+        if (e) (void)hipEventDestroy(e);
+  }
 };
 
 extern "C" {
@@ -128,6 +140,8 @@
       for (uint32_t i = 0; i < n_terms; ++i) by_df.emplace_back(terms[i].doc_freq, terms[i].postings_start);
       reserve_densest_columns(*seg, by_df);
     }
+    s->one_device = s->segments.empty() || (s->one_device && s->device == device);
+    s->device = device;
     s->segments.push_back(seg);
     s->searcher.reset(new Searcher(s->segments));
   });
@@ -146,6 +160,8 @@
                                                fieldnorm, fn_len);
     seg->set_term_info_store(st);
     reserve_densest_columns(*seg, *st);
+    s->one_device = s->segments.empty() || (s->one_device && s->device == device);
+    s->device = device;
     s->segments.push_back(seg);
     s->searcher.reset(new Searcher(s->segments));
   });
@@ -166,6 +182,8 @@
                                                total_num_tokens);
     seg->set_term_info_store(st);
     reserve_densest_columns(*seg, *st);
+    s->one_device = s->segments.empty() || (s->one_device && s->device == device);
+    s->device = device;
     s->segments.push_back(seg);
     s->searcher.reset(new Searcher(s->segments));
   });
@@ -460,6 +478,57 @@
   });
 }
 
+int tqh_search_prepared_device(tqh_searcher *s, uint32_t k, float *out_scores, uint32_t *out_segment_ords,
+                               uint32_t *out_docs, uint32_t *out_counts, float *d_slab_scores,
+                               uint32_t *d_slab_docs, uint32_t *d_slab_counts, void *hip_stream) {
+  return guard([&] {
+    if (!s || !s->searcher || s->segments.empty()) throw TantivyError(TantivyError::InvalidArgument, "no segments");
+    if (!out_scores || !out_segment_ords || !out_docs || !out_counts || !k)
+      throw TantivyError(TantivyError::InvalidArgument, "null argument");
+    const size_t S = s->segments.size(), n = s->prepared.size();
+    if (n == 0) return;
+    if (S == 1) {
+      s->searcher->collect_segment_batch_device(0, s->prepared, k, out_scores, out_docs, out_counts, hip_stream,
+                                                out_segment_ords);
+      return;
+    }
+    if (!d_slab_scores || !d_slab_docs || !d_slab_counts)
+      throw TantivyError(TantivyError::InvalidArgument, "several segments need the slabs");
+    if (!s->one_device) throw TantivyError(TantivyError::Unsupported, "tqh_search_prepared_device: the segments sit on several devices");
+    for (size_t sg = 0; sg < S; ++sg)
+      s->searcher->collect_segment_batch_device(sg, s->prepared, k, d_slab_scores + sg * n * k, d_slab_docs + sg * n * k,
+                                                d_slab_counts + sg * n, hip_stream);
+    auto hip = [](hipError_t e) {
+      if (e != hipSuccess) throw TantivyError(TantivyError::SystemError, hipGetErrorString(e));
+    };
+    hipEvent_t *ev = s->ex_ev[s->ex_at % tqh_searcher::kExRing];
+    for (int i = 0; i < 2; ++i)
+      if (!ev[i]) hip(hipEventCreate(&ev[i]));
+    hip(hipEventRecord(ev[0], (hipStream_t)hip_stream));
+    const int rc = tq_merge_topk_device(s->ctx, s->device, d_slab_scores, d_slab_docs, d_slab_counts, nullptr, (uint32_t)S,
+                                        (uint32_t)n, k, 0, k, out_scores, out_segment_ords, out_docs, out_counts, hip_stream);
+    if (rc != TQ_OK) throw TantivyError(TantivyError::SystemError, tq_last_error());
+    hip(hipEventRecord(ev[1], (hipStream_t)hip_stream));
+    ++s->ex_at;
+    s->ex_n = std::min(s->ex_n + 1u, tqh_searcher::kExRing);
+  });
+}
+int tqh_exchange_ms(tqh_searcher *s, float *ms) {
+  return guard([&] {
+    if (!s || !ms) throw TantivyError(TantivyError::InvalidArgument, "null argument");
+    double sum = 0.0;
+    for (uint32_t i = 0; i < s->ex_n; ++i) {
+      hipEvent_t *ev = s->ex_ev[(s->ex_at - 1u - i) % tqh_searcher::kExRing];
+      float one = 0.0f;
+      if (hipEventSynchronize(ev[1]) != hipSuccess || hipEventElapsedTime(&one, ev[0], ev[1]) != hipSuccess)
+        throw TantivyError(TantivyError::SystemError, "tqh_exchange_ms: the events of a merge launch cannot be read");
+      sum += one;
+    }
+    *ms = s->ex_n ? (float)(sum / s->ex_n) : 0.0f;
+    s->ex_n = 0;
+  });
+}
+
 int tqh_bm25_for_terms(const uint64_t *term_doc_freqs, uint32_t n_terms, uint64_t total_num_docs,
                        uint64_t total_num_tokens, float boost, float *weight_out,
                        float *cache_out ) {
diff --git a/tantivy_amd/host/searcher.cpp b/tantivy_amd/host/searcher.cpp
--- a/tantivy_amd/host/searcher.cpp
+++ b/tantivy_amd/host/searcher.cpp
@@ -95,6 +95,12 @@
     fast[term_id].store(handle, std::memory_order_release);
   }
   return handle;
+}
+
+bool SegmentReader::handle_known(uint32_t term_id) const {
+  if (term_id >= kFastHandles) return false;
+  std::atomic<tq_term_handle> *fast = fast_handles_.load(std::memory_order_acquire);
+  return fast && fast[term_id].load(std::memory_order_acquire) != kHandleUnknown;
 }
 
 void SegmentReader::prepare_terms(const uint32_t *term_ids, size_t n) {
@@ -170,10 +176,6 @@
   return seg->term_handle(t);
 }
 }
-
-Searcher::Searcher(std::vector<std::shared_ptr<SegmentReader>> segments)
-    : segments_(std::move(segments)) {}
-Searcher::~Searcher() { delete[] fast_weights_.load(std::memory_order_relaxed); }
 
 void Searcher::add_remote_statistics(
     uint64_t max_doc, uint64_t total_num_tokens,
@@ -500,20 +502,22 @@
 struct SegmentBatch {
   std::vector<tq_query> qs;
   std::vector<tq_term_handle> handles;
-  SegmentBatch(const std::shared_ptr<SegmentReader> &seg_p, const std::vector<Weight> &weights, uint32_t k) {
+  SegmentBatch() = default;
+  SegmentBatch(const std::shared_ptr<SegmentReader> &seg_p, const std::vector<Weight> &weights, uint32_t k) { fill(seg_p, weights, k); }
+  void fill(const std::shared_ptr<SegmentReader> &seg_p, const std::vector<Weight> &weights, uint32_t k) {
     SegmentReader &seg = *seg_p;
     const size_t n = weights.size();
     qs.resize(n);
     size_t total_terms = 0;
     for (auto &w : weights) total_terms += w.terms.size();
+    handles.clear();
     handles.reserve(total_terms);
     if (n > 1) {
-      std::vector<uint32_t> all;
-      all.reserve(total_terms);
+      std::vector<uint32_t> fresh;
       for (auto &w : weights)
         for (uint32_t t : w.terms)
-          if (t < kTermSetBase) all.push_back(t);
-      seg.prepare_terms(all.data(), all.size());
+          if (t < kTermSetBase && !seg.handle_known(t)) fresh.push_back(t);
+      if (!fresh.empty()) seg.prepare_terms(fresh.data(), fresh.size());
     }
     for (size_t i = 0; i < n; ++i) {
       const Weight &w = weights[i];
@@ -538,6 +542,15 @@
 };
 }
 
+struct Searcher::DeviceBatch {
+  std::mutex m;
+  SegmentBatch b;
+};
+
+Searcher::Searcher(std::vector<std::shared_ptr<SegmentReader>> segments)
+    : segments_(std::move(segments)), device_batch_(new DeviceBatch()) {}
+Searcher::~Searcher() { delete[] fast_weights_.load(std::memory_order_relaxed); }
+
 uint32_t Searcher::bound_slack_ppm(const SegmentReader &seg) const {
   const double global = (double)total_num_tokens() / (double)total_num_docs();
   const double local = seg.max_doc() ? (double)seg.total_num_tokens() / (double)seg.max_doc() : global;
@@ -623,12 +636,17 @@
 
 void Searcher::collect_segment_batch_device(size_t segment_ord, const std::vector<Weight> &weights,
                                             uint32_t k, float *d_scores, uint32_t *d_docs,
-                                            uint32_t *d_counts, void *hip_stream) {
+                                            uint32_t *d_counts, void *hip_stream, uint32_t *d_segment_ords) {
   SegmentReader &seg = *segments_[segment_ord];
-  SegmentBatch b(segments_[segment_ord], weights, k);
+  std::lock_guard<std::mutex> lk(device_batch_->m);
+  SegmentBatch &b = device_batch_->b;
+  b.fill(segments_[segment_ord], weights, k);
   const tq_search_opts opts{-1, bound_slack_ppm(seg)};
-  const int rc = tq_search_batch_device_opts(seg.raw(), b.qs.data(), (uint32_t)weights.size(), k,
-                                             d_scores, d_docs, d_counts, &opts, hip_stream);
+  const int rc = d_segment_ords
+                     ? tq_search_batch_device_rows(seg.raw(), b.qs.data(), (uint32_t)weights.size(), k, d_scores,
+                                                   d_segment_ords, d_docs, d_counts, (uint32_t)segment_ord, &opts, hip_stream)
+                     : tq_search_batch_device_opts(seg.raw(), b.qs.data(), (uint32_t)weights.size(), k,
+                                                   d_scores, d_docs, d_counts, &opts, hip_stream);
   if (rc != TQ_OK) throw_tq(rc);
 }
 
diff --git a/tantivy_amd/host/searcher.hpp b/tantivy_amd/host/searcher.hpp
--- a/tantivy_amd/host/searcher.hpp
+++ b/tantivy_amd/host/searcher.hpp
@@ -50,6 +50,7 @@
   const TermInfo *get_term_info(uint32_t term_id) const;
   tq_term_handle term_handle(uint32_t term_id);
   void prepare_terms(const uint32_t *term_ids, size_t n);
+  bool handle_known(uint32_t term_id) const;
   uint32_t max_doc() const { return max_doc_; }
   uint32_t segment_ord() const { return segment_ord_; }
   uint64_t total_num_tokens() const { return total_num_tokens_; }
@@ -298,11 +299,13 @@
                              std::vector<uint32_t> &counts);
   void collect_segment_batch_device(size_t segment_ord, const std::vector<Weight> &weights,
                                     uint32_t k, float *d_scores, uint32_t *d_docs,
-                                    uint32_t *d_counts, void *hip_stream);
+                                    uint32_t *d_counts, void *hip_stream, uint32_t *d_segment_ords = nullptr);
 
  private:
   uint32_t bound_slack_ppm(const SegmentReader &seg) const;
   std::vector<std::shared_ptr<SegmentReader>> segments_;
+  struct DeviceBatch;
+  std::unique_ptr<DeviceBatch> device_batch_;
   mutable std::mutex cache_m_;
   mutable std::shared_ptr<Bm25Weight> shared_cache_;
   static constexpr uint32_t kFastWeights = 1u << 20;
```

After: 11.95 million queries/s, median of 6. 1.07x the previous value.
